# bastienjacquet/CudaDepthMapIntegration

Hardware: AMD Instinct MI355X
Metric: Gvoxel-projections/s (higher is better)
Workload: dtype f64

## Files before the change

### cudadepthmapintegration_amd/build.py

```python
from __future__ import annotations

import os
import re
import shutil
import subprocess
from concurrent.futures import ThreadPoolExecutor

_HERE = os.path.dirname(os.path.abspath(__file__))
ROOT = os.path.dirname(_HERE)
CSRC = os.path.join(_HERE, "csrc")
OBJ_DIR = os.path.join(ROOT, "build", "obj")
LIB_PATH = os.path.join(CSRC, "libdmi_hip.so")

SOURCES = ["fusion_kernels.hip", "fusion_tile.hip", "fusion_classify.hip", "coloration_kernels.hip", "grid_post.hip", "isosurface.hip", "isosurface_components.hip", "isosurface_smooth.hip", "dmi_capi.hip", "dmi_multi.hip", "host/recon_host.cpp", "host/vti_reader.cpp", "host/vtp_reader.cpp", "host/recon_cli.cpp", "host/color_cli.cpp", "host/dmi_host_capi.cpp"]
HEADERS = ["fusion_kernels.h", "fusion_device.h", "fusion_tile_acc.inc", "isosurface_table.inc", os.path.join("host", "recon_host.h"),
           os.path.join("host", "vtk_xml_data.h"), os.path.join("host", "vti_reader.h"), os.path.join("host", "vtp_reader.h"),
           os.path.join("host", "recon_cli.h"), os.path.join("host", "color_cli.h"),
           os.path.join("..", "..", "include", "dmi.h"), os.path.join("..", "..", "include", "dmi_host.h")]
CLI_MAINS = ["recon_cli_main.cpp", "color_cli_main.cpp"]

COMMON_FLAGS = ["-O3", "-std=c++17", "-fPIC", "-ffp-contract=off", "-fno-fast-math", "-Wall", "-Wno-unused-function",
                "-Wno-inline-asm", "-Wno-pass-failed"]
HIP_FLAGS = ["--offload-arch=gfx950", "-mllvm", "-disable-promote-alloca-to-vector", "-Xoffload-linker", "--discard-all"]
OPTIONAL_LLVM_FLAGS = ["-amdgpu-use-amdgpu-trackers=1"]


def _probe_llvm_flag(flag: str) -> bool:
    import tempfile

    try:
        with tempfile.TemporaryDirectory() as tmp:
            src = os.path.join(tmp, "probe.hip")
            with open(src, "w") as fh:
                fh.write("__global__ void probe() {}\n")
            r = subprocess.run([hipcc_path(), "--offload-arch=gfx950", "--cuda-device-only", "-mllvm", flag, "-c", src, "-o",
                                os.path.join(tmp, "probe.o")], capture_output=True)
            return r.returncode == 0
    except (OSError, RuntimeError):
        return False


_FLAG_CACHE = os.path.join(ROOT, "build", "llvm_flag_probe.json")


def _optional_flags() -> list:
    import json

    try:
        parts = []
        hip = os.path.realpath(hipcc_path())
        for f in (hip, os.path.realpath(os.path.join(os.path.dirname(hip), "..", "lib", "llvm", "bin", "clang"))):
            if os.path.exists(f):
                st = os.stat(f)
                parts.append("%s:%d:%d" % (f, st.st_size, int(st.st_mtime)))
        version = ";".join(parts)
    except (OSError, RuntimeError):
        return []
    try:
        with open(_FLAG_CACHE) as fh:
            rec = json.load(fh)
        if rec.get("hipcc") == version and set(rec.get("flags", {})) == set(OPTIONAL_LLVM_FLAGS):
            return [x for f in OPTIONAL_LLVM_FLAGS if rec["flags"][f] for x in ("-mllvm", f)]
    except (OSError, ValueError):
        pass
    flags = {f: _probe_llvm_flag(f) for f in OPTIONAL_LLVM_FLAGS}
    try:
        os.makedirs(os.path.dirname(_FLAG_CACHE), exist_ok=True)
        with open(_FLAG_CACHE, "w") as fh:
            json.dump({"hipcc": version, "flags": flags}, fh)
    except OSError:
        pass
    return [x for f in OPTIONAL_LLVM_FLAGS if flags[f] for x in ("-mllvm", f)]
if os.environ.get("DMI_EXP"):
    _name, _, _defs = os.environ["DMI_EXP"].partition(":")
    COMMON_FLAGS = COMMON_FLAGS + _defs.split()
    OBJ_DIR = os.path.join(ROOT, "build", "obj_exp_" + _name)
    LIB_PATH = os.path.join(CSRC, "libdmi_hip_exp_" + _name + ".so")
if os.environ.get("DMI_TUNING"):
    COMMON_FLAGS = COMMON_FLAGS + ["-DDMI_TUNING"]
    OBJ_DIR = os.path.join(ROOT, "build", "obj_tuning")
    LIB_PATH = os.path.join(CSRC, "libdmi_hip_tuning.so")


def hipcc_path() -> str:
    for cand in (shutil.which("hipcc"), "/opt/rocm/bin/hipcc"):
        if cand and os.path.exists(cand):
            return cand
    raise RuntimeError("hipcc not found: the HIP library cannot be built (no CPU fallback exists)")


HIP_FLAGS = HIP_FLAGS + _optional_flags()


def _sources():
    return [s for s in SOURCES if os.path.exists(os.path.join(CSRC, s))]


def _headers():
    return [os.path.join(CSRC, h) for h in HEADERS if os.path.exists(os.path.join(CSRC, h))]


def _obj(src: str) -> str:
    return os.path.join(OBJ_DIR, src.replace("/", "_") + ".o")


def _stale(target: str, deps) -> bool:
    if not os.path.exists(target):
        return True
    t = os.path.getmtime(target)
    return any(os.path.getmtime(d) > t for d in deps)


LIB_OVERRIDE = os.environ.get("DMI_LIB_OVERRIDE")
if LIB_OVERRIDE:
    LIB_PATH = os.path.abspath(LIB_OVERRIDE)


def source_digest(files=None) -> str:
    import hashlib

    h = hashlib.sha256()
    h.update(" ".join(COMMON_FLAGS + HIP_FLAGS).encode())
    if files is None:
        files = [os.path.join(CSRC, s) for s in _sources()] + _headers() + [os.path.join(CSRC, "host", m) for m in CLI_MAINS]
    for f in files:
        h.update(os.path.relpath(f, CSRC).encode())
        with open(f, "rb") as fh:
            h.update(fh.read())
    return h.hexdigest()


def _digest_path() -> str:
    return LIB_PATH + ".digest"


def needs_build() -> bool:
    if LIB_OVERRIDE:
        return False
    if not os.path.exists(LIB_PATH):
        return True
    if os.path.exists(_digest_path()):
        with open(_digest_path()) as fh:
            return fh.read().strip() != source_digest()
    deps = [os.path.join(CSRC, s) for s in _sources()] + _headers()
    return _stale(LIB_PATH, deps)


ACC_BASES = {8: 64, 7: 72, 6: 80, 5: 96}


def audit_accumulator_registers(asm_text: str) -> tuple[int, list[str]]:
    import re

    bad: list[str] = []
    checked = 0
    for body in re.split(r"\n(?=_ZN3dmi\S*fuse_tile_kernel\S*:)", asm_text):
        m = re.match(r"(_ZN3dmi\S*fuse_tile_kernelI\w+):", body)
        if not m:
            continue
        name = m.group(1)
        tpl = re.search(r"fuse_tile_kernelI\w\wLi(\d+)ELi(\d)ELi(\d)ELi(\d)ELi(\d)ELb([01])", name)
        tk, minw = int(tpl.group(1)), int(tpl.group(4))
        base = ACC_BASES.get(minw, 128)
        code = body[: body.find("s_endpgm")]
        in_asm = False
        scc_from_asm = False
        for line in code.splitlines():
            if "#ASMSTART" in line:
# ... 203 lines not shown
```

### cudadepthmapintegration_amd/capi.py

```python
from __future__ import annotations

import ctypes
import os
import sys
from typing import NamedTuple

import numpy as np

from . import build as _build
from .scene import GridDesc, RayPotential, Views

DMI_OK = 0
DMI_F32, DMI_F64 = 0, 1
DMI_DEPTH_AUTO, DMI_DEPTH_F32, DMI_DEPTH_F64 = 0, 1, 2
DMI_COMPONENTS_MIN_TRIANGLES, DMI_COMPONENTS_LARGEST = 0, 1

VARIANT_EXACT_DIVISION = 1
VARIANT_GENERAL_K = 2
VARIANT_FORCE_GENERAL = 16
VARIANT_NO_BRICK_CLASSES = 256
VARIANT_KEEP_BEHIND_ADDS = 1024
VARIANT_NO_INTERIOR = 2048
VARIANT_XCD_RUNS = 8192
VARIANT_ZMAJOR_SLOTS = 16384
VARIANT_PERSISTENT_ALWAYS = 32768
VARIANT_PERSISTENT_NEVER = 65536
VARIANT_NO_WINDOWS = 262144
VARIANT_WINDOWS_ALWAYS = 524288
VARIANT_COST_ORDER = 1048576
VARIANT_NO_COST_ORDER = 2097152
VARIANT_BRICK_CLASSES_ALWAYS = 131072
VARIANT_FIXED_TILE_SHAPE = 4096
VARIANT_SPATIAL_ORDER = 512
VARIANT_TILE_SHAPE = {"tk16_w5_g8_1x1": 0, "tk8_w6_g8_2x2": 32, "tk16_w5_g8_2x2": 64, "tk8_w6": 96, "tk8_w7_g8": 128, "tk16_w5_g4": 160,
                      "tk16_w6_g2": 192, "tk8_w6_g8_1x1": 224}


class GridDescC(ctypes.Structure):
    _fields_ = [("cell_dims", ctypes.c_int32 * 3), ("origin", ctypes.c_double * 3),
                ("spacing", ctypes.c_double * 3), ("grid_matrix", ctypes.c_double * 16)]


class RayPotentialC(ctypes.Structure):
    _fields_ = [("thickness", ctypes.c_double), ("rho", ctypes.c_double), ("eta", ctypes.c_double),
                ("delta", ctypes.c_double)]


class OptionsC(ctypes.Structure):
    _fields_ = [("device", ctypes.c_int32), ("grid_dtype", ctypes.c_int32), ("depth_storage", ctypes.c_int32),
                ("count_hits", ctypes.c_int32), ("kernel_variant", ctypes.c_int32), ("z_first", ctypes.c_int32),
                ("stream", ctypes.c_void_p), ("external_grid", ctypes.c_void_p)]


class TimingsC(ctypes.Structure):
    _fields_ = [("last_fuse_kernel_ms", ctypes.c_double), ("total_fuse_kernel_ms", ctypes.c_double),
                ("fuse_launches", ctypes.c_uint64), ("last_upload_ms", ctypes.c_double),
                ("last_download_ms", ctypes.c_double), ("last_cell_to_point_ms", ctypes.c_double),
                ("last_fuse_main_kernel_ms", ctypes.c_double), ("total_fuse_main_kernel_ms", ctypes.c_double)]


class InfoC(ctypes.Structure):
    _fields_ = [("n_voxels", ctypes.c_int64), ("n_views", ctypes.c_int32), ("depth_width", ctypes.c_int32),
                ("depth_height", ctypes.c_int32), ("depth_storage_in_use", ctypes.c_int32),
                ("grid_dtype", ctypes.c_int32), ("k_mode", ctypes.c_int32), ("kernel_variant", ctypes.c_int32),
                ("tiled_kernel", ctypes.c_int32), ("device_bytes", ctypes.c_uint64), ("pixels_without_depth", ctypes.c_uint64)]


class MultiOptionsC(ctypes.Structure):
    _fields_ = [("grid_dtype", ctypes.c_int32), ("depth_storage", ctypes.c_int32), ("kernel_variant", ctypes.c_int32),
                ("partition", ctypes.c_int32), ("exchange", ctypes.c_int32), ("n_slabs", ctypes.c_int32)]


class MultiInfoC(ctypes.Structure):
    _fields_ = [("world", ctypes.c_int32), ("n_local", ctypes.c_int32), ("first_rank", ctypes.c_int32),
                ("rccl_ranks", ctypes.c_int32), ("rccl_version", ctypes.c_int32), ("partition", ctypes.c_int32),
                ("exchange", ctypes.c_int32), ("n_slabs", ctypes.c_int32), ("n_voxels", ctypes.c_int64),
                ("n_views_total", ctypes.c_int64), ("n_views_local", ctypes.c_int64)]


class MultiTimingsC(ctypes.Structure):
    _fields_ = [("last_step_ms", ctypes.c_double), ("last_fuse_kernel_ms", ctypes.c_double),
                ("total_step_ms", ctypes.c_double), ("steps", ctypes.c_uint64)]


DMI_PARTITION_VIEWS, DMI_PARTITION_Z_SLABS = 0, 1
DMI_EXCHANGE_ALL_REDUCE, DMI_EXCHANGE_REDUCE_SCATTER, DMI_EXCHANGE_PEER_COPY = 0, 1, 2
DMI_UNIQUE_ID_BYTES = 128

ABI_SYMBOLS = [
    "dmi_default_options", "dmi_create", "dmi_destroy", "dmi_last_error", "dmi_add_views", "dmi_add_views_f32",
    "dmi_clear_views", "dmi_reset_grid", "dmi_upload_grid", "dmi_fuse", "dmi_fuse_range", "dmi_fuse_slab", "dmi_fuse_range_download", "dmi_synchronize",
    "dmi_download_grid_f64", "dmi_download_grid_f32", "dmi_download_hits", "dmi_grid_device_pointer",
    "dmi_get_brick_class_histogram", "dmi_get_timings", "dmi_get_info", "dmi_alloc_pinned", "dmi_free_pinned", "dmi_pcie_probe", "dmi_fp64_probe", "dmi_abi_version", "dmi_device_count",
    "dmi_color_mesh", "dmi_color_last_error", "dmi_cell_to_point", "dmi_download_point_data_f64",
    "dmi_point_data_device_pointer", "dmi_color_create", "dmi_color_destroy", "dmi_color_add_views",
    "dmi_color_clear_views", "dmi_color_process", "dmi_color_get_kernel_ms", "dmi_get_mixed_reason_histogram", "dmi_get_window_pair_count", "dmi_get_view_paths", "dmi_get_upload_kernel_ms", "dmi_sizeof_info", "dmi_sizeof_timings",
    "dmi_color_set_scratch_budget", "dmi_color_set_vertex_reorder", "dmi_color_add_views_with_depth", "dmi_color_set_depth_test",
    "dmi_iso_active_cells",
    "dmi_extract_isosurface", "dmi_download_isosurface", "dmi_get_isosurface_kernel_ms",
    "dmi_extract_isosurface_normals", "dmi_download_isosurface_normals",
    "dmi_filter_isosurface_components", "dmi_download_isosurface_regions", "dmi_get_isosurface_filter_kernel_ms",
    "dmi_get_isosurface_filter_pass_ms", "dmi_get_isosurface_filter_cas_retries",
    "dmi_smooth_isosurface", "dmi_get_isosurface_smooth_kernel_ms", "dmi_get_isosurface_smooth_pass_ms",
    "dmi_multi_default_options", "dmi_multi_view_shard", "dmi_multi_z_slab", "dmi_multi_slab_ranges", "dmi_multi_peer_chunk", "dmi_multi_create",
    "dmi_multi_get_unique_id", "dmi_multi_create_rank", "dmi_multi_destroy", "dmi_multi_last_error", "dmi_multi_add_views",
    "dmi_multi_add_views_f32", "dmi_multi_add_local_views", "dmi_multi_add_local_views_f32", "dmi_multi_clear_views", "dmi_multi_fuse", "dmi_multi_synchronize",
    "dmi_multi_download_grid_f32", "dmi_multi_download_grid_f64", "dmi_multi_get_info", "dmi_multi_get_timings",
    "dmi_multi_local_context",
]

_lib = None


class DmiError(RuntimeError):
    def __init__(self, code: int, message: str):
        super().__init__(f"dmi error {code}: {message}")
        self.code = code


def library_path() -> str:
    return _build.LIB_PATH


def load() -> ctypes.CDLL:
    global _lib
    if _lib is not None:
        return _lib
    if "torch" not in sys.modules:
        try:
            import torch
        except Exception:
            pass
    path = _build.build()
    if not os.path.exists(path):
        raise RuntimeError(f"{path} is missing: the HIP extension is required, there is no CPU fallback")
    L = ctypes.CDLL(path)
    vp, i32, dbl = ctypes.c_void_p, ctypes.c_int32, ctypes.c_double
    dp = ctypes.POINTER(ctypes.c_double)
    L.dmi_default_options.argtypes = [ctypes.POINTER(OptionsC)]
    L.dmi_default_options.restype = None
    L.dmi_create.argtypes = [ctypes.POINTER(GridDescC), ctypes.POINTER(RayPotentialC), ctypes.POINTER(OptionsC),
                             ctypes.POINTER(vp)]
    L.dmi_destroy.argtypes = [vp]
    L.dmi_destroy.restype = None
    L.dmi_last_error.argtypes = [vp]
    L.dmi_last_error.restype = ctypes.c_char_p
    L.dmi_add_views.argtypes = [vp, dp, dp, dbl, dp, dp, i32, i32, i32]
    L.dmi_add_views_f32.argtypes = [vp, ctypes.POINTER(ctypes.c_float), dp, dp, i32, i32, i32]
    L.dmi_clear_views.argtypes = [vp]
    L.dmi_reset_grid.argtypes = [vp]
    L.dmi_upload_grid.argtypes = [vp, dp]
    L.dmi_fuse.argtypes = [vp]
    L.dmi_fuse_range.argtypes = [vp, i32, i32]
    L.dmi_fuse_slab.argtypes = [vp, i32, i32]
    if hasattr(L, "dmi_fuse_range_download"):
        L.dmi_fuse_range_download.argtypes = [vp, i32, i32, vp, i32, i32]
    L.dmi_synchronize.argtypes = [vp]
    L.dmi_download_grid_f64.argtypes = [vp, dp]
    L.dmi_download_grid_f32.argtypes = [vp, ctypes.POINTER(ctypes.c_float)]
    L.dmi_download_hits.argtypes = [vp, ctypes.POINTER(ctypes.c_uint32), ctypes.POINTER(ctypes.c_uint64)]
    L.dmi_grid_device_pointer.argtypes = [vp, ctypes.POINTER(vp)]
    L.dmi_cell_to_point.argtypes = [vp]
    L.dmi_download_point_data_f64.argtypes = [vp, dp]
    L.dmi_point_data_device_pointer.argtypes = [vp, ctypes.POINTER(vp)]
    if hasattr(L, "dmi_iso_active_cells"):
        L.dmi_iso_active_cells.argtypes = [vp, ctypes.c_double, ctypes.POINTER(ctypes.c_uint64), ctypes.POINTER(ctypes.c_int64),
                                           ctypes.c_uint64]
    if hasattr(L, "dmi_extract_isosurface"):
        L.dmi_extract_isosurface.argtypes = [vp, ctypes.c_double, ctypes.POINTER(ctypes.c_uint64), ctypes.POINTER(ctypes.c_uint64)]
        L.dmi_download_isosurface.argtypes = [vp, dp, ctypes.POINTER(ctypes.c_int64)]
        L.dmi_get_isosurface_kernel_ms.argtypes = [vp, dp]
    if hasattr(L, "dmi_extract_isosurface_normals"):
        L.dmi_extract_isosurface_normals.argtypes = [vp, ctypes.c_double, ctypes.POINTER(ctypes.c_uint64), ctypes.POINTER(ctypes.c_uint64)]
        L.dmi_download_isosurface_normals.argtypes = [vp, ctypes.POINTER(ctypes.c_float)]
    if hasattr(L, "dmi_filter_isosurface_components"):
        u64p = ctypes.POINTER(ctypes.c_uint64)
        L.dmi_filter_isosurface_components.argtypes = [vp, ctypes.c_int, ctypes.c_uint64, u64p, u64p, u64p, u64p]
        L.dmi_download_isosurface_regions.argtypes = [vp, ctypes.POINTER(ctypes.c_int64), ctypes.POINTER(ctypes.c_int64)]
        L.dmi_get_isosurface_filter_kernel_ms.argtypes = [vp, dp]
        L.dmi_get_isosurface_filter_pass_ms.argtypes = [vp, dp]
        L.dmi_get_isosurface_filter_cas_retries.argtypes = [vp, u64p]
    if hasattr(L, "dmi_smooth_isosurface"):
        L.dmi_smooth_isosurface.argtypes = [vp, i32, dbl, dbl]
        L.dmi_get_isosurface_smooth_kernel_ms.argtypes = [vp, dp]
        L.dmi_get_isosurface_smooth_pass_ms.argtypes = [vp, dp]
    L.dmi_get_brick_class_histogram.argtypes = [vp, ctypes.POINTER(ctypes.c_uint64)]
    L.dmi_get_mixed_reason_histogram.argtypes = [vp, ctypes.POINTER(ctypes.c_uint64)]
    if hasattr(L, "dmi_get_window_pair_count"):
        L.dmi_get_window_pair_count.argtypes = [vp, ctypes.POINTER(ctypes.c_uint64)]
    if hasattr(L, "dmi_get_view_paths"):
        L.dmi_get_view_paths.argtypes = [vp, ctypes.POINTER(ctypes.c_uint64)]
    if hasattr(L, "dmi_get_upload_kernel_ms"):
        L.dmi_get_upload_kernel_ms.argtypes = [vp, dp, dp]
    for name in ("dmi_sizeof_info", "dmi_sizeof_timings"):
        if hasattr(L, name):
            getattr(L, name).restype = ctypes.c_size_t
    L.dmi_get_timings.argtypes = [vp, ctypes.POINTER(TimingsC)]
    L.dmi_get_info.argtypes = [vp, ctypes.POINTER(InfoC)]
    L.dmi_alloc_pinned.argtypes = [ctypes.c_size_t, ctypes.POINTER(vp)]
    L.dmi_free_pinned.argtypes = [vp]
    L.dmi_pcie_probe.argtypes = [i32, ctypes.c_size_t, dp, dp]
    L.dmi_fp64_probe.argtypes = [i32, ctypes.c_double, dp]
    u8p = ctypes.POINTER(ctypes.c_uint8)
    L.dmi_color_mesh.argtypes = [dp, ctypes.c_int64, u8p, dp, dp, i32, i32, i32, i32, u8p, u8p, ctypes.POINTER(ctypes.c_int32)]
    L.dmi_color_create.argtypes = [i32, ctypes.POINTER(vp)]
    L.dmi_color_destroy.argtypes = [vp]
    L.dmi_color_destroy.restype = None
    L.dmi_color_add_views.argtypes = [vp, u8p, dp, dp, i32, i32, i32]
    L.dmi_color_clear_views.argtypes = [vp]
    L.dmi_color_process.argtypes = [vp, dp, ctypes.c_int64, u8p, u8p, ctypes.POINTER(ctypes.c_int32)]
    L.dmi_color_get_kernel_ms.argtypes = [vp, dp]
    L.dmi_color_set_scratch_budget.argtypes = [vp, ctypes.c_uint64]
    L.dmi_color_set_vertex_reorder.argtypes = [vp, i32]
    L.dmi_color_add_views_with_depth.argtypes = [vp, u8p, dp, dp, dp, i32, i32, i32]
    L.dmi_color_set_depth_test.argtypes = [vp, i32, ctypes.c_double]
    L.dmi_color_last_error.argtypes = []
    L.dmi_color_last_error.restype = ctypes.c_char_p
    i64, i64p, i32p = ctypes.c_int64, ctypes.POINTER(ctypes.c_int64), ctypes.POINTER(ctypes.c_int32)
    L.dmi_multi_default_options.argtypes = [ctypes.POINTER(MultiOptionsC)]
    L.dmi_multi_default_options.restype = None
    L.dmi_multi_view_shard.argtypes = [i64, i32, i32, i64p, i64p]
    L.dmi_multi_z_slab.argtypes = [i32, i32, i32, i32p, i32p]
    L.dmi_multi_slab_ranges.argtypes = [i32, i32, i32p, i32p, i32]
    if hasattr(L, "dmi_multi_peer_chunk"):
        L.dmi_multi_peer_chunk.argtypes = [i64, i32, i32, i64p, i64p]
    L.dmi_multi_create.argtypes = [ctypes.POINTER(GridDescC), ctypes.POINTER(RayPotentialC), ctypes.POINTER(MultiOptionsC),
                                   i32p, i32, ctypes.POINTER(vp)]
    L.dmi_multi_get_unique_id.argtypes = [u8p]
    L.dmi_multi_create_rank.argtypes = [ctypes.POINTER(GridDescC), ctypes.POINTER(RayPotentialC), ctypes.POINTER(MultiOptionsC),
                                        i32, i32, i32, u8p, ctypes.POINTER(vp)]
    L.dmi_multi_destroy.argtypes = [vp]
    L.dmi_multi_destroy.restype = None
    L.dmi_multi_last_error.argtypes = [vp]
    L.dmi_multi_last_error.restype = ctypes.c_char_p
    L.dmi_multi_add_views.argtypes = [vp, dp, dp, dbl, dp, dp, i32, i32, i32]
    L.dmi_multi_add_views_f32.argtypes = [vp, ctypes.POINTER(ctypes.c_float), dp, dp, i32, i32, i32]
    L.dmi_multi_add_local_views.argtypes = [vp, i32, dp, dp, dbl, dp, dp, i32, i32, i32]
    L.dmi_multi_add_local_views_f32.argtypes = [vp, i32, ctypes.POINTER(ctypes.c_float), dp, dp, i32, i32, i32]
    L.dmi_multi_clear_views.argtypes = [vp]
    L.dmi_multi_fuse.argtypes = [vp]
    L.dmi_multi_synchronize.argtypes = [vp]
    L.dmi_multi_download_grid_f32.argtypes = [vp, ctypes.POINTER(ctypes.c_float), i64p, i64p]
    L.dmi_multi_download_grid_f64.argtypes = [vp, dp, i64p, i64p]
    L.dmi_multi_get_info.argtypes = [vp, ctypes.POINTER(MultiInfoC)]
    L.dmi_multi_get_timings.argtypes = [vp, ctypes.POINTER(MultiTimingsC)]
    L.dmi_multi_local_context.argtypes = [vp, i32, ctypes.POINTER(vp)]
    from . import build as _b
    for name in ABI_SYMBOLS:
        if _b.LIB_OVERRIDE and not hasattr(L, name):
            continue
        fn = getattr(L, name)
        if fn.restype is ctypes.c_int:
            fn.restype = ctypes.c_int
    _lib = L
    return L


def pinned_empty(shape, dtype) -> np.ndarray:
    L = load()
    n = int(np.prod(shape)) * np.dtype(dtype).itemsize
    p = ctypes.c_void_p()
    rc = L.dmi_alloc_pinned(n, ctypes.byref(p))
    if rc != DMI_OK:
        raise DmiError(rc, "dmi_alloc_pinned failed")
    buf = (ctypes.c_char * n).from_address(p.value)
    return np.frombuffer(buf, dtype=dtype).reshape(shape)


def pcie_probe(device: int = 0, n_bytes: int = 256 << 20) -> tuple[float, float]:
    L = load()
    a, b = ctypes.c_double(), ctypes.c_double()
    rc = L.dmi_pcie_probe(int(device), int(n_bytes), ctypes.byref(a), ctypes.byref(b))
    if rc != DMI_OK:
        raise DmiError(rc, L.dmi_last_error(None).decode())
    return float(a.value), float(b.value)


def fp64_probe(device: int = 0, milliseconds: float = 20.0) -> float:
    L = load()
    a = ctypes.c_double()
    rc = L.dmi_fp64_probe(int(device), float(milliseconds), ctypes.byref(a))
    if rc != DMI_OK:
        raise DmiError(rc, L.dmi_last_error(None).decode())
    return float(a.value)


def device_count() -> int:
    return int(load().dmi_device_count())


def _dp(a):
    return a.ctypes.data_as(ctypes.POINTER(ctypes.c_double))


class FusionContext:

    def __init__(self, grid: GridDesc, ray: RayPotential, *, device: int = 0, grid_dtype: str = "f64",
                 depth_storage: str = "auto", count_hits: bool = False, kernel_variant: int = 0,
                 stream: int | None = None, external_grid: int | None = None, z_first: int = 0):
        self._lib = load()
        self._h = ctypes.c_void_p()
        g = _grid_c(grid)
        r = RayPotentialC(float(ray.thickness), float(ray.rho), float(ray.eta), float(ray.delta))
        o = OptionsC()
        self._lib.dmi_default_options(ctypes.byref(o))
        o.device = device
        o.grid_dtype = {"f32": DMI_F32, "f64": DMI_F64}[grid_dtype]
        o.depth_storage = {"auto": DMI_DEPTH_AUTO, "f32": DMI_DEPTH_F32, "f64": DMI_DEPTH_F64}[depth_storage]
        o.count_hits = 1 if count_hits else 0
        o.kernel_variant = int(kernel_variant)
        o.z_first = int(z_first)
        o.stream = stream
        o.external_grid = external_grid
        self.grid = grid
        self.grid_dtype = grid_dtype
        self.n_voxels = grid.n_voxels
        self._mesh_counts = None
        rc = self._lib.dmi_create(ctypes.byref(g), ctypes.byref(r), ctypes.byref(o), ctypes.byref(self._h))
        if rc != DMI_OK:
            self._h = ctypes.c_void_p()
            raise DmiError(rc, self._lib.dmi_last_error(None).decode())

    def _check(self, rc: int):
        if rc != DMI_OK:
            raise DmiError(rc, self._lib.dmi_last_error(self._h).decode())

    def close(self):
        if getattr(self, "_h", None) is not None and self._h:
            self._lib.dmi_destroy(self._h)
            self._h = ctypes.c_void_p()

    def __enter__(self):
        return self

    def __exit__(self, *exc):
        self.close()

    def __del__(self):
        try:
            self.close()
# ... 84 lines not shown

    def cell_to_point(self):
        self._check(self._lib.dmi_cell_to_point(self._h))

    def download_point_data(self) -> np.ndarray:
        nx, ny, nz = (int(c) for c in self.grid.cell_dims)
        out = np.empty((nz + 1) * (ny + 1) * (nx + 1), dtype=np.float64)
        self._check(self._lib.dmi_download_point_data_f64(self._h, _dp(out)))
        return out.reshape(nz + 1, ny + 1, nx + 1)

    def iso_active_cells(self, iso: float, ids: bool = True):
        n = ctypes.c_uint64(0)
        self._check(self._lib.dmi_iso_active_cells(self._h, float(iso), ctypes.byref(n), None, 0))
        if not ids:
            return int(n.value), None
        out = np.empty(int(n.value), dtype=np.int64)
        if n.value:
            self._check(self._lib.dmi_iso_active_cells(self._h, float(iso), ctypes.byref(n),
                                                       out.ctypes.data_as(ctypes.POINTER(ctypes.c_int64)), out.size))
        return int(n.value), out

    def extract_isosurface(self, iso: float):
        nv, nt = ctypes.c_uint64(0), ctypes.c_uint64(0)
        self._mesh_counts = None
        self._check(self._lib.dmi_extract_isosurface(self._h, float(iso), ctypes.byref(nv), ctypes.byref(nt)))
        verts = np.empty((max(int(nv.value), 1), 3), dtype=np.float64)
        tris = np.empty((max(int(nt.value), 1), 3), dtype=np.int64)
        self._mesh_counts = (int(nv.value), int(nt.value), 0)
        self._check(self._lib.dmi_download_isosurface(self._h, _dp(verts), tris.ctypes.data_as(ctypes.POINTER(ctypes.c_int64))))
        return verts[:int(nv.value)], tris[:int(nt.value)]

    def extract_isosurface_with_normals(self, iso: float):
        nv, nt = ctypes.c_uint64(0), ctypes.c_uint64(0)
        self._mesh_counts = None
        self._check(self._lib.dmi_extract_isosurface_normals(self._h, float(iso), ctypes.byref(nv), ctypes.byref(nt)))
        verts = np.empty((max(int(nv.value), 1), 3), dtype=np.float64)
        tris = np.empty((max(int(nt.value), 1), 3), dtype=np.int64)
        normals = np.empty((max(int(nv.value), 1), 3), dtype=np.float32)
        self._mesh_counts = (int(nv.value), int(nt.value), 0)
        self._check(self._lib.dmi_download_isosurface(self._h, _dp(verts), tris.ctypes.data_as(ctypes.POINTER(ctypes.c_int64))))
        self._check(self._lib.dmi_download_isosurface_normals(self._h, normals.ctypes.data_as(ctypes.POINTER(ctypes.c_float))))
        return verts[:int(nv.value)], tris[:int(nt.value)], normals[:int(nv.value)]

    def filter_isosurface_components(self, mode: str = "min_triangles", min_triangles: int = 0):
        m = {"min_triangles": DMI_COMPONENTS_MIN_TRIANGLES, "largest": DMI_COMPONENTS_LARGEST}[mode]
        out = [ctypes.c_uint64(0) for _ in range(4)]
        self._check(self._lib.dmi_filter_isosurface_components(self._h, m, int(min_triangles), *[ctypes.byref(x) for x in out]))
        self._mesh_counts = (int(out[0].value), int(out[1].value), int(out[3].value))
        return tuple(int(x.value) for x in out)

    def _current_mesh_counts(self):
        c = self._mesh_counts
        if c is None:
            raise DmiError(1, "no mesh: extract_isosurface has not succeeded")
        return c

    def download_isosurface(self):
        nv, nt, _ = self._current_mesh_counts()
        verts = np.empty((max(nv, 1), 3), dtype=np.float64)
        tris = np.empty((max(nt, 1), 3), dtype=np.int64)
        self._check(self._lib.dmi_download_isosurface(self._h, _dp(verts), tris.ctypes.data_as(ctypes.POINTER(ctypes.c_int64))))
        return verts[:nv], tris[:nt]

    def download_isosurface_normals(self):
        nv, _, _ = self._current_mesh_counts()
        normals = np.empty((max(nv, 1), 3), dtype=np.float32)
        self._check(self._lib.dmi_download_isosurface_normals(self._h, normals.ctypes.data_as(ctypes.POINTER(ctypes.c_float))))
        return normals[:nv]

    def download_isosurface_regions(self):
        nv, _, nk = self._current_mesh_counts()
        rid = np.empty(max(nv, 1), dtype=np.int64)
        rsz = np.empty(max(nk, 1), dtype=np.int64)
        i64p = ctypes.POINTER(ctypes.c_int64)
        self._check(self._lib.dmi_download_isosurface_regions(self._h, rid.ctypes.data_as(i64p), rsz.ctypes.data_as(i64p)))
        return rid[:nv], rsz[:nk]

    def isosurface_filter_kernel_ms(self) -> float:
        a = ctypes.c_double(0)
        self._check(self._lib.dmi_get_isosurface_filter_kernel_ms(self._h, ctypes.byref(a)))
        return float(a.value)

    def isosurface_filter_cas_retries(self) -> int:
        a = ctypes.c_uint64(0)
        self._check(self._lib.dmi_get_isosurface_filter_cas_retries(self._h, ctypes.byref(a)))
        return int(a.value)

    def isosurface_filter_pass_ms(self) -> dict:
        a = (ctypes.c_double * 4)()
        self._check(self._lib.dmi_get_isosurface_filter_pass_ms(self._h, a))
        return dict(zip(("labels", "sizes", "scans", "compaction"), (float(x) for x in a)))

    def smooth_isosurface(self, iterations: int, lam: float = 0.5, mu: float = -0.53) -> None:
        self._check(self._lib.dmi_smooth_isosurface(self._h, int(iterations), float(lam), float(mu)))

    def isosurface_smooth_kernel_ms(self) -> float:
        a = ctypes.c_double(0)
        self._check(self._lib.dmi_get_isosurface_smooth_kernel_ms(self._h, ctypes.byref(a)))
        return float(a.value)

    def isosurface_smooth_pass_ms(self) -> dict:
        a = (ctypes.c_double * 3)()
        self._check(self._lib.dmi_get_isosurface_smooth_pass_ms(self._h, a))
        return dict(zip(("adjacency", "steps", "normals"), (float(x) for x in a)))

    def isosurface_kernel_ms(self) -> float:
        a = ctypes.c_double(0)
        self._check(self._lib.dmi_get_isosurface_kernel_ms(self._h, ctypes.byref(a)))
        return float(a.value)

    def brick_class_histogram(self) -> dict:
        h = (ctypes.c_uint64 * 4)()
        self._check(self._lib.dmi_get_brick_class_histogram(self._h, h))
        return {"mixed": int(h[0]), "free": int(h[1]), "behind": int(h[2]), "skip": int(h[3])}

    def mixed_reason_histogram(self) -> dict:
        h = (ctypes.c_uint64 * 8)()
        self._check(self._lib.dmi_get_mixed_reason_histogram(self._h, h))
        names = ["unspecified", "degenerate", "camera_plane", "image_border", "nan_depth", "sentinel_and_depth", "near_surface",
                 "free_or_no_depth"]
        return {n: int(h[i]) for i, n in enumerate(names)}

    def window_pair_count(self) -> int:
        n = ctypes.c_uint64(0)
        if not hasattr(self._lib, "dmi_get_window_pair_count"):
            return 0
        self._check(self._lib.dmi_get_window_pair_count(self._h, ctypes.byref(n)))
        return int(n.value)

    def upload_kernel_ms(self) -> tuple:
        if not hasattr(self._lib, "dmi_get_upload_kernel_ms"):
            return (0.0, 0.0)
        a, b = ctypes.c_double(0), ctypes.c_double(0)
        self._check(self._lib.dmi_get_upload_kernel_ms(self._h, ctypes.byref(a), ctypes.byref(b)))
        return (float(a.value), float(b.value))

    def timings(self) -> TimingsC:
        t = TimingsC()
        self._check(self._lib.dmi_get_timings(self._h, ctypes.byref(t)))
        return t

    def info(self) -> InfoC:
        i = InfoC()
        self._check(self._lib.dmi_get_info(self._h, ctypes.byref(i)))
        return i

    def view_paths(self) -> dict:
        names = ("general_kernel", "tiled_general_k", "tiled_fp64_selection", "tiled_tier1", "tiled_tier1_per_lane_margin", "with_window_record")
        if not hasattr(self._lib, "dmi_get_view_paths"):
            return {}
        a = (ctypes.c_uint64 * 6)()
        self._check(self._lib.dmi_get_view_paths(self._h, a))
        return {k: int(v) for k, v in zip(names, a)}


def _grid_c(grid: GridDesc) -> GridDescC:
    g = GridDescC()
    for i in range(3):
        g.cell_dims[i] = int(grid.cell_dims[i])
        g.origin[i] = float(grid.origin[i])
        g.spacing[i] = float(grid.spacing[i])
    gm = np.ascontiguousarray(grid.grid_matrix, dtype=np.float64).reshape(16)
    for i in range(16):
        g.grid_matrix[i] = gm[i]
    return g


def multi_view_shard(n: int, rank: int, world: int) -> tuple[int, int]:
    a, b = ctypes.c_int64(), ctypes.c_int64()
    if load().dmi_multi_view_shard(int(n), int(rank), int(world), ctypes.byref(a), ctypes.byref(b)) != DMI_OK:
        raise ValueError("rank/world out of range")
    return int(a.value), int(a.value + b.value)


def multi_z_slab(nz: int, rank: int, world: int) -> tuple[int, int]:
    a, b = ctypes.c_int32(), ctypes.c_int32()
    if load().dmi_multi_z_slab(int(nz), int(rank), int(world), ctypes.byref(a), ctypes.byref(b)) != DMI_OK:
        raise ValueError("rank/world out of range")
    return int(a.value), int(a.value + b.value)


def multi_peer_chunk(n: int, world: int, c: int) -> tuple[int, int]:
    a, b = ctypes.c_int64(), ctypes.c_int64()
    rc = load().dmi_multi_peer_chunk(int(n), int(world), int(c), ctypes.byref(a), ctypes.byref(b))
    if rc != DMI_OK:
        raise DmiError(rc, "dmi_multi_peer_chunk: invalid argument")
    return int(a.value), int(b.value)


def multi_slab_ranges(nz: int, n_slabs: int) -> list[tuple[int, int]]:
    a, b = (ctypes.c_int32 * 64)(), (ctypes.c_int32 * 64)()
    n = load().dmi_multi_slab_ranges(int(nz), int(n_slabs), a, b, 64)
    return [(int(a[i]), int(b[i])) for i in range(n)]


def multi_unique_id() -> bytes:
    L = load()
    buf = (ctypes.c_uint8 * DMI_UNIQUE_ID_BYTES)()
    rc = L.dmi_multi_get_unique_id(buf)
    if rc != DMI_OK:
        raise DmiError(rc, L.dmi_multi_last_error(None).decode())
    return bytes(buf)


class MultiContext:

    def __init__(self, grid: GridDesc, ray: RayPotential, *, devices=None, rank: int | None = None, world: int | None = None,
                 unique_id: bytes | None = None, device: int = 0, grid_dtype: str = "f32", depth_storage: str = "auto",
                 kernel_variant: int = 0, partition: str = "views", exchange: str = "all_reduce", n_slabs: int = 0):
        self._lib = load()
        self._h = ctypes.c_void_p()
        o = MultiOptionsC()
        self._lib.dmi_multi_default_options(ctypes.byref(o))
        o.grid_dtype = {"f32": DMI_F32, "f64": DMI_F64}[grid_dtype]
        o.depth_storage = {"auto": DMI_DEPTH_AUTO, "f32": DMI_DEPTH_F32, "f64": DMI_DEPTH_F64}[depth_storage]
        o.kernel_variant = int(kernel_variant)
        o.partition = {"views": DMI_PARTITION_VIEWS, "z_slabs": DMI_PARTITION_Z_SLABS}[partition]
        o.exchange = {"all_reduce": DMI_EXCHANGE_ALL_REDUCE, "reduce_scatter": DMI_EXCHANGE_REDUCE_SCATTER,
                      "peer_copy": DMI_EXCHANGE_PEER_COPY}[exchange]
        o.n_slabs = int(n_slabs)
        g = _grid_c(grid)
        r = RayPotentialC(float(ray.thickness), float(ray.rho), float(ray.eta), float(ray.delta))
        self.grid = grid
        self.grid_dtype = grid_dtype
        self.n_voxels = grid.n_voxels
        if devices is not None:
            d = (ctypes.c_int32 * len(devices))(*[int(x) for x in devices])
            rc = self._lib.dmi_multi_create(ctypes.byref(g), ctypes.byref(r), ctypes.byref(o), d, len(devices), ctypes.byref(self._h))
        else:
            if rank is None or world is None:
                raise ValueError("MultiContext needs devices=[...] or rank= and world=")
            idbuf = None
            if unique_id is not None:
                if len(unique_id) != DMI_UNIQUE_ID_BYTES:
                    raise ValueError("unique_id must be 128 bytes")
                idbuf = (ctypes.c_uint8 * DMI_UNIQUE_ID_BYTES).from_buffer_copy(unique_id)
            rc = self._lib.dmi_multi_create_rank(ctypes.byref(g), ctypes.byref(r), ctypes.byref(o), int(device), int(rank),
                                                 int(world), idbuf, ctypes.byref(self._h))
        if rc != DMI_OK:
            self._h = ctypes.c_void_p()
            raise DmiError(rc, self._lib.dmi_multi_last_error(None).decode())

    def _check(self, rc: int):
        if rc != DMI_OK:
            raise DmiError(rc, self._lib.dmi_multi_last_error(self._h).decode())

    def close(self):
        if getattr(self, "_h", None) is not None and self._h:
            self._lib.dmi_multi_destroy(self._h)
            self._h = ctypes.c_void_p()

    def __enter__(self):
        return self

    def __exit__(self, *exc):
        self.close()

    def __del__(self):
        try:
            self.close()
        except Exception:
            pass

    def add_views(self, views: Views, threshold: float | None = None, local_index: int | None = None):
        n, H, W = views.depth.shape
        K4 = np.ascontiguousarray(views.K4, dtype=np.float64).reshape(n, 16)
        RT4 = np.ascontiguousarray(views.RT4, dtype=np.float64).reshape(n, 16)
        L = self._lib
        if views.depth.dtype == np.float32:
            d = np.ascontiguousarray(views.depth)
            dptr = d.ctypes.data_as(ctypes.POINTER(ctypes.c_float))
            if local_index is None:
                self._check(L.dmi_multi_add_views_f32(self._h, dptr, _dp(K4), _dp(RT4), n, W, H))
            else:
                self._check(L.dmi_multi_add_local_views_f32(self._h, int(local_index), dptr, _dp(K4), _dp(RT4), n, W, H))
            return
        d = np.ascontiguousarray(views.depth, dtype=np.float64)
        bc = None
        if views.best_cost is not None and threshold is not None:
            bc = np.ascontiguousarray(views.best_cost, dtype=np.float64)
        thr = float(threshold) if threshold is not None else 0.0
        if local_index is None:
            self._check(L.dmi_multi_add_views(self._h, _dp(d), _dp(bc) if bc is not None else None, thr, _dp(K4), _dp(RT4), n, W, H))
        else:
            self._check(L.dmi_multi_add_local_views(self._h, int(local_index), _dp(d), _dp(bc) if bc is not None else None, thr,
                                                    _dp(K4), _dp(RT4), n, W, H))

    def clear_views(self):
        self._check(self._lib.dmi_multi_clear_views(self._h))

    def fuse(self):
        self._check(self._lib.dmi_multi_fuse(self._h))

    def synchronize(self):
        self._check(self._lib.dmi_multi_synchronize(self._h))

    def download_grid(self, dtype=np.float32, out: np.ndarray | None = None):
        nx, ny, nz = (int(c) for c in self.grid.cell_dims)
        if out is None:
            out = np.zeros(self.n_voxels, dtype=dtype)
        a, b = ctypes.c_int64(), ctypes.c_int64()
        if np.dtype(dtype) == np.float64:
            self._check(self._lib.dmi_multi_download_grid_f64(self._h, _dp(out), ctypes.byref(a), ctypes.byref(b)))
        else:
            self._check(self._lib.dmi_multi_download_grid_f32(self._h, out.ctypes.data_as(ctypes.POINTER(ctypes.c_float)),
                                                              ctypes.byref(a), ctypes.byref(b)))
# ... 560 lines not shown
```

### cudadepthmapintegration_amd/csrc/dmi_capi.hip

```cpp
#include "../../include/dmi.h"
#include "fusion_kernels.h"

#include <chrono>
#include <cmath>
#include <cstdio>
#include <cstdlib>
#include <cstring>
#include <exception>
#include <limits>
#include <new>
#include <string>
#include <vector>

using dmi::FuseArgs;
using dmi::FuseConfig;
using dmi::MapRec;
using dmi::TileArgs;
using dmi::TileMapRec;

namespace {

thread_local std::string g_create_error;

struct Batch {
// ... 331 lines not shown
    if (e == hipSuccess) e = hipStreamSynchronize(ctx->upload_stream);
    if (e == hipSuccess && ctx->up_start && ctx->up_stop) {
      float ms = 0.f;
      if (hipEventElapsedTime(&ms, ctx->up_start, ctx->up_stop) == hipSuccess) {
        const size_t last_cnt = (size_t)n - ((size_t)n - 1) / chunk * chunk;
        ctx->last_upload_kernel_ms = (double)ms * (double)n / (double)last_cnt;
        ctx->total_upload_kernel_ms += ctx->last_upload_kernel_ms;
      } else {
        (void)hipGetLastError();
      }
    }
    *lossy_out = counters[0];
    b.holes = counters[1];
    b.mingled_strips = counters[2];
    if (e != hipSuccess) rc = fail(ctx, DMI_ERR_DEVICE, std::string("depth upload: ") + hipGetErrorString(e));
  }
  if (rc != DMI_OK) {
    (void)hipFree(b.d_depth);
    (void)hipFree(b.d_pyramid);
    ctx->device_bytes -= npix * n * esz + pyr_bytes;
    return rc;
  }
  *out = b;
  return DMI_OK;
}


constexpr int kMaxColumn = 32;

void voxel_world(const dmi_grid_desc &g, int i, int j, int k, double w[3]) {
  const double p[3] = {g.origin[0] + (i + 0.5) * g.spacing[0], g.origin[1] + (j + 0.5) * g.spacing[1],
                       g.origin[2] + (k + 0.5) * g.spacing[2]};
  for (int r = 0; r < 3; ++r)
    w[r] = ((g.grid_matrix[4 * r] * p[0] + g.grid_matrix[4 * r + 1] * p[1]) + g.grid_matrix[4 * r + 2] * p[2]) +
           g.grid_matrix[4 * r + 3];
}

bool grid_axis_aligned(const dmi_grid_desc &g) {
  const double *m = g.grid_matrix;
  return m[1] == 0 && m[2] == 0 && m[4] == 0 && m[6] == 0 && m[8] == 0 && m[9] == 0;
}

float float_not_below(double x) {
  float f = (float)x;
  if ((double)f < x) f = std::nextafterf(f, std::numeric_limits<float>::infinity());
  return f;
}

void make_centred_rows(const dmi_context *ctx, const MapRec &r, const double P[4], const double Q[4], const double S[4],
                       double Sx, double Sy, const double M[3], double zabs, double zscale, bool general, bool aligned, TileMapRec *out,
                       dmi::WinRec *win, dmi::FootRec *foot) {
  TileMapRec &t = *out;
  std::memset(foot, 0, sizeof(*foot));
  std::memset(win, 0, sizeof(*win));
  win->e_abs = std::numeric_limits<float>::infinity();
  win->c1 = dmi::kWinC1;
  t.t1_ok = 0;
  t.t1_e1 = std::numeric_limits<float>::infinity();
  t.t1_c1 = 0.5f - 0x1p-20f;
  const double cxc = (double)(ctx->W / 2), cyc = (double)(ctx->H / 2);
  t.t1_cidx = (int32_t)((int64_t)ctx->W * (ctx->H / 2) + ctx->W / 2);
  if (general) return;
  double Pc[4], Qc[4];
  for (int c = 0; c < 4; ++c) {
    Pc[c] = P[c] - cxc * S[c];
    Qc[c] = Q[c] - cyc * S[c];
  }
  t.cpx = Pc[0]; t.cpy = Pc[1]; t.cpz = Pc[2]; t.cp0 = Pc[3];
  t.cqx = Qc[0]; t.cqy = Qc[1]; t.cqz = Qc[2]; t.cq0 = Qc[3];
  const double *g = ctx->grid.grid_matrix;
  const double sz = ctx->grid.spacing[2];
  t.cdhx = (Pc[0] * (g[2] * sz) + Pc[1] * (g[6] * sz)) + Pc[2] * (g[10] * sz);
  t.cdhy = (Qc[0] * (g[2] * sz) + Qc[1] * (g[6] * sz)) + Qc[2] * (g[10] * sz);
  const double rot = aligned ? 1.0 : 2.0;
  const double Sxc = Sx + cxc * M[2], Syc = Sy + cyc * M[2];
  const double cerr = rot * std::max(Sxc, Syc) * 0x1p-44;
  t.cerrk = cerr + 0x1p-22 * zabs * (1.0 + 0x1p-20);
  t.t1_dhx = (float)t.cdhx;
  t.t1_dhy = (float)t.cdhy;
  const double dcz = t.dhz;
  t.t1_dcz = (float)dcz;
  t.t1_dthr = (float)(dcz * (double)t.t1_c1);
  if (!(cerr < 0x1p-12 * zscale)) return;
  double czmin = std::numeric_limits<double>::infinity(), Scx = 0.0, Scy = 0.0;
  for (int c = 0; c < 8; ++c) {
    double w[3];
    voxel_world(ctx->grid, (c & 1) ? ctx->grid.cell_dims[0] - 1 : 0, (c & 2) ? ctx->grid.cell_dims[1] - 1 : 0,
                ctx->opt.z_first + ((c & 4) ? ctx->grid.cell_dims[2] - 1 : 0), w);
    czmin = std::min(czmin, ((r.rt[8] * w[0] + r.rt[9] * w[1]) + r.rt[10] * w[2]) + r.rt[11]);
    Scx = std::max(Scx, std::fabs(((Pc[0] * w[0] + Pc[1] * w[1]) + Pc[2] * w[2]) + Pc[3]));
    Scy = std::max(Scy, std::fabs(((Qc[0] * w[0] + Qc[1] * w[1]) + Qc[2] * w[2]) + Qc[3]));
  }
  czmin -= rot * 16.0 * 0x1p-52 * M[2];
  const double Sc = (std::max(Scx, Scy) + cerr) * (1.0 + 0x1p-20);
  const double D = kMaxColumn * std::max(std::fabs(t.cdhx), std::fabs(t.cdhy));
  const double Dz = kMaxColumn * std::fabs(dcz);
  const double nl = rot * 32.0 * 0x1p-53 * M[2];
  if (!std::isfinite(czmin)) return;
  const bool per_lane = !(czmin > 0.0) || !(Sc / czmin + 1.0 < 0x1p22);
  const double pmax = per_lane ? 0.0 : Sc / czmin + 1.0;
  const bool index_exact = ((int64_t)ctx->H + 2 * dmi::kValidMargin + 8) * ((int64_t)ctx->W + 2 * dmi::kValidMargin) + ctx->H +
                               2 * dmi::kValidMargin < (int64_t(1) << 24);
  double e1 = cerr + 3.0 * 0x1p-24 * Dz * pmax + 0x1p-22 * Dz + nl * (pmax + 2.0) + 0x1p-53 * std::max(Sx, Sy);
  e1 *= 1.0 + 0x1p-10;
  t.t1_erel = 0x1p-22f * (1.0f + 0x1p-10f);
  t.t1_hspan = float_not_below(D * (1.0 + 0x1p-20));
  if (!(pmax < 0x1p22) || !index_exact || !(e1 > 0x1p-100) || !(Sc < 0x1p60) || !std::isfinite(e1)) return;
  t.t1_e1 = float_not_below(e1);
  t.t1_ok = 1;
  {
    const double *sp = ctx->grid.spacing;
    double d[3][2], c[3];
    for (int ax = 0; ax < 3; ++ax) {
      const double wxs = g[ax] * sp[ax], wys = g[4 + ax] * sp[ax], wzs = g[8 + ax] * sp[ax];
      d[ax][0] = (Pc[0] * wxs + Pc[1] * wys) + Pc[2] * wzs;
      d[ax][1] = (Qc[0] * wxs + Qc[1] * wys) + Qc[2] * wzs;
      c[ax] = (S[0] * wxs + S[1] * wys) + S[2] * wzs;
    }
    const double xmax = (double)(std::max(ctx->W, ctx->H) / 2 + dmi::kValidMargin + 1);
    const double nl2 = 2.0 * nl;
    const double pwin = (dmi::kWindowRows - 0.5) * dmi::kWinCzRatio + 3.0;
    const double steps[3] = {7.0, 7.0, (double)(kMaxColumn - 1)};
    double e_step = 0.0;
    for (int xy = 0; xy < 2; ++xy) {
      double e = 0.0;
      for (int ax = 0; ax < 3; ++ax) e += steps[ax] * (std::fabs(d[ax][xy]) + xmax * std::fabs(c[ax]));
      e_step = std::max(e_step, e * 0x1p-23);
    }
    double ew = (cerr + xmax * nl2) + e_step + pwin * nl2 + 0x1p-53 * std::max(Sx, Sy);
    ew *= 1.0 + 0x1p-10;
    bool ok = std::isfinite(ew) && ew > 0x1p-100 && ew < 0x1p60;
    for (int ax = 0; ax < 3; ++ax) ok = ok && std::fabs(d[ax][0]) < 0x1p60 && std::fabs(d[ax][1]) < 0x1p60 && std::fabs(c[ax]) < 0x1p60;
    if (ok) {
      for (int xy = 0; xy < 2; ++xy) {
        win->di[xy] = (float)d[0][xy];
        win->dj[xy] = (float)d[1][xy];
        win->dk[xy] = (float)d[2][xy];
      }
      win->ci[0] = (float)c[0]; win->ci[1] = (float)(c[0] * (double)dmi::kWinC1);
      win->cj[0] = (float)c[1]; win->cj[1] = (float)(c[1] * (double)dmi::kWinC1);
      win->ck[0] = (float)c[2]; win->ck[1] = (float)(c[2] * (double)dmi::kWinC1);
      win->e_abs = float_not_below(ew);
      for (int cnr = 0; cnr < 8; ++cnr) {
        const double ni = (cnr & 1) ? 7.0 : 0.0, nj = (cnr & 2) ? 7.0 : 0.0;
        for (int v = 0; v < 2; ++v) {
          const double nk = (cnr & 4) ? (v ? 15.0 : 7.0) : 0.0;
          float *dst = v ? foot->s16[cnr] : foot->s8[cnr];
          dst[0] = (float)((ni * d[0][0] + nj * d[1][0]) + nk * d[2][0]);
          dst[1] = (float)((ni * d[0][1] + nj * d[1][1]) + nk * d[2][1]);
          dst[2] = (float)((ni * c[0] + nj * c[1]) + nk * c[2]);
        }
      }
      foot->ferr = float_not_below(cerr + xmax * nl2);
    }
  }
  if (per_lane) {
    const double B = (3.0 * 0x1p-24 * Dz + nl) * (1.0 + 0x1p-10) * (1.0 + 0x1p-10);
    if (!(B < 0x1p60) || !(B >= 0.0)) {
      t.t1_ok = 0;
      t.t1_e1 = std::numeric_limits<float>::infinity();
      return;
    }
    t.t1_b = float_not_below(B);
    t.t1_ok = 2;
  }
}

TileMapRec make_tile_rec(const dmi_context *ctx, const MapRec &r, dmi::WinRec *win, dmi::FootRec *foot, double *zscale_out) {
  TileMapRec t;
  std::memset(&t, 0, sizeof(t));
  const double *rt = r.rt, *k = r.k;
  t.rz0 = rt[8];
  t.rz1 = rt[9];
  t.rz3 = rt[11];
  const bool general = classify_k(r.k, r.rt) == dmi::K_GENERAL;
  double P[4], Q[4], S[4];
  for (int c = 0; c < 4; ++c) {
    if (general) {
      P[c] = (k[0] * rt[c] + k[1] * rt[4 + c]) + k[2] * rt[8 + c];
      Q[c] = (k[4] * rt[c] + k[5] * rt[4 + c]) + k[6] * rt[8 + c];
      S[c] = (k[8] * rt[c] + k[9] * rt[4 + c]) + k[10] * rt[8 + c];
    } else {
      P[c] = k[0] * rt[c] + k[1] * rt[4 + c] + k[2] * rt[8 + c];
      Q[c] = k[5] * rt[4 + c] + k[6] * rt[8 + c];
      S[c] = rt[8 + c];
    }
  }
  if (general) {
    P[3] += k[3];
    Q[3] += k[7];
    S[3] += k[11];
  }
  t.px = P[0]; t.py = P[1]; t.pz = P[2]; t.p0 = P[3];
  t.qx = Q[0]; t.qy = Q[1]; t.qz = Q[2]; t.q0 = Q[3];
  t.sx = S[0]; t.sy = S[1]; t.sz = S[2]; t.s0 = S[3];
  const double *g = ctx->grid.grid_matrix;
  const double sz = ctx->grid.spacing[2];
  t.dhx = (P[0] * (g[2] * sz) + P[1] * (g[6] * sz)) + P[2] * (g[10] * sz);
  t.dhy = (Q[0] * (g[2] * sz) + Q[1] * (g[6] * sz)) + Q[2] * (g[10] * sz);
  t.dhz = (S[0] * (g[2] * sz) + S[1] * (g[6] * sz)) + S[2] * (g[10] * sz);
  double wm[3];
  const bool aligned = grid_axis_aligned(ctx->grid);
  if (aligned) {
    double lo[3], hi[3];
    voxel_world(ctx->grid, 0, 0, ctx->opt.z_first, lo);
    voxel_world(ctx->grid, ctx->grid.cell_dims[0] - 1, ctx->grid.cell_dims[1] - 1,
                ctx->opt.z_first + ctx->grid.cell_dims[2] - 1 + kMaxColumn, hi);
    for (int a = 0; a < 3; ++a) wm[a] = std::max(std::fabs(lo[a]), std::fabs(hi[a]));
  } else {
    double gm[3];
    for (int a = 0; a < 3; ++a)
      gm[a] = std::fabs(ctx->grid.origin[a]) +
              (ctx->grid.cell_dims[a] + 1.0 + (a == 2 ? ctx->opt.z_first + kMaxColumn : 0)) * std::fabs(ctx->grid.spacing[a]);
    for (int a = 0; a < 3; ++a)
      wm[a] = std::fabs(g[4 * a]) * gm[0] + std::fabs(g[4 * a + 1]) * gm[1] + std::fabs(g[4 * a + 2]) * gm[2] + std::fabs(g[4 * a + 3]);
  }
  double M[3];
  for (int row = 0; row < 3; ++row)
    M[row] = std::fabs(rt[4 * row]) * wm[0] + std::fabs(rt[4 * row + 1]) * wm[1] + std::fabs(rt[4 * row + 2]) * wm[2] +
             std::fabs(rt[4 * row + 3]);
  const double Sx = std::fabs(k[0]) * M[0] + std::fabs(k[1]) * M[1] + std::fabs(k[2]) * M[2] + (general ? std::fabs(k[3]) : 0.0);
  const double Sy = (general ? std::fabs(k[4]) * M[0] : 0.0) + std::fabs(k[5]) * M[1] + std::fabs(k[6]) * M[2] +
                    (general ? std::fabs(k[7]) : 0.0);
  const double Sz = general ? std::fabs(k[8]) * M[0] + std::fabs(k[9]) * M[1] + std::fabs(k[10]) * M[2] + std::fabs(k[11]) : M[2];
  t.err = std::max(Sx, Sy) * 0x1p-44;
  t.errz = general ? Sz * 0x1p-44 : 0.0;
  t.cz_err = aligned ? 0.0 : M[2] * 0x1p-47;
  double zabs = Sz, czlo = std::numeric_limits<double>::infinity(), czhi = -czlo;
  if (!general) {
    zabs = 0.0;
    for (int c = 0; c < 8; ++c) {
      double w[3];
      voxel_world(ctx->grid, (c & 1) ? ctx->grid.cell_dims[0] - 1 : 0, (c & 2) ? ctx->grid.cell_dims[1] - 1 : 0,
                  ctx->opt.z_first + ((c & 4) ? ctx->grid.cell_dims[2] - 1 + kMaxColumn : 0), w);
      const double cz = ((rt[8] * w[0] + rt[9] * w[1]) + rt[10] * w[2]) + rt[11];
      zabs = std::max(zabs, std::fabs(cz));
      czlo = std::min(czlo, cz);
      czhi = std::max(czhi, cz);
    }
    zabs = zabs * (1.0 + 0x1p-20) + (aligned ? 1.0 : 2.0) * 32.0 * 0x1p-52 * M[2];
    if (!std::isfinite(zabs)) zabs = Sz;
  }
  double zscale = 1.0;
  if (!general && std::isfinite(czlo) && std::isfinite(czhi)) zscale = std::max(1.0, std::max(czlo, czhi / 16.0));
  t.errk = (t.err + 65536.0 * t.errz) + 0x1p-22 * zabs * (1.0 + 0x1p-20);
  t.depth = r.depth;
  make_centred_rows(ctx, r, P, Q, S, Sx, Sy, M, zabs, zscale, general, aligned, &t, win, foot);
  if (zscale_out) *zscale_out = zscale;
  return t;
}

bool tile_eligible(const dmi_context *ctx) {
  if (ctx->opt.kernel_variant & dmi::VAR_FORCE_GENERAL) return false;
  if (!ctx->finite_bounded) return false;
  if (!(ctx->ray.thickness >= 0) || !(ctx->ray.delta >= 0)) return false;
  if ((int64_t)ctx->W * ctx->H * (int64_t)(ctx->depth_f64 ? 8 : 4) >= (int64_t(1) << 31)) return false;
  return true;
}

int add_views_impl(dmi_context *ctx, const double *depth64, const float *depth32, const double *best_cost,
                   double threshold, const double *K4, const double *RT4, int32_t n, int32_t width, int32_t height) {
  if (!ctx) return DMI_ERR_INVALID_ARGUMENT;
  if ((!depth64 && !depth32) || !K4 || !RT4) return fail(ctx, DMI_ERR_INVALID_ARGUMENT, "dmi_add_views: null pointer");
  if (n <= 0) return fail(ctx, DMI_ERR_INVALID_ARGUMENT, "dmi_add_views: n must be positive");
  if (width < 1 || height < 1 || width > 32768 || height > 32768)
    return fail(ctx, DMI_ERR_INVALID_ARGUMENT, "dmi_add_views: depth-map dimensions must be in [1, 32768]");
  if (!ctx->batches.empty() && (width != ctx->W || height != ctx->H))
    return fail(ctx, DMI_ERR_INVALID_ARGUMENT, "dmi_add_views: every view of a context must share width and height");
  DMI_HIP(ctx, hipSetDevice(ctx->opt.device));
  const auto t0 = std::chrono::steady_clock::now();
  if (ctx->batches.empty()) {
    ctx->W = width;
    ctx->H = height;
    ctx->depth_f64 = ctx->opt.depth_storage == DMI_DEPTH_F64;
    ctx->k_mode = ctx->finite_bounded ? (int)dmi::K_PINHOLE : (int)dmi::K_GENERAL;
    ctx->max_tile_err = 0.0;
    ctx->pyramid = dmi::make_pyramid_desc(width, height);
  }
  const size_t npix = (size_t)width * height;

  Batch b;
  unsigned long long lossy = 0;
  int rc = upload_batch(ctx, depth64, depth32, best_cost, threshold, n, &b, &lossy);
  if (rc != DMI_OK) return rc;
  if (lossy != 0 && !ctx->depth_f64 && ctx->opt.depth_storage == DMI_DEPTH_AUTO) {
    (void)hipFree(b.d_depth);
    (void)hipFree(b.d_pyramid);
    ctx->device_bytes -= npix * n * 4 + b.aux_bytes;
    rc = promote_to_f64(ctx);
    if (rc != DMI_OK) return rc;
    rc = upload_batch(ctx, depth64, depth32, best_cost, threshold, n, &b, &lossy);
    if (rc != DMI_OK) return rc;
  }
  ctx->batches.push_back(b);
  const size_t esz = depth_elem(ctx);
  for (int32_t m = 0; m < n; ++m) {
    MapRec r;
    std::memset(&r, 0, sizeof(r));
    std::memcpy(r.rt, RT4 + 16 * (size_t)m, 12 * sizeof(double));
    std::memcpy(r.k, K4 + 16 * (size_t)m, 12 * sizeof(double));
    r.depth = static_cast<const char *>(b.d_depth) + (size_t)m * npix * esz;
    r.pyramid = b.d_pyramid + (size_t)m * ctx->pyramid.total_tiles;
    ctx->h_maps.push_back(r);
    bool finite = true;
    for (int q = 0; q < 12; ++q) finite = finite && bounded(r.k[q]) && bounded(r.rt[q]);
    const int km = classify_k(r.k, r.rt);
    if (km < ctx->k_mode) ctx->k_mode = km;
    dmi::WinRec wrec;
    dmi::FootRec frec;
    double zscale = 1.0;
    TileMapRec t = make_tile_rec(ctx, r, &wrec, &frec, &zscale);
    t.valid = reinterpret_cast<const uint8_t *>(b.d_pyramid) + b.valid_offset + (size_t)m * (size_t)dmi::valid_map_bytes(ctx->W, ctx->H);
    t.vm_c0 = ((float)(ctx->H / 2 + dmi::kValidMargin) - 3.5f) * 0.125f;
    t.vm_w8 = (float)(8 * (ctx->W + 2 * dmi::kValidMargin) - 8);
    t.vm_base = 8 * (ctx->W / 2 + dmi::kValidMargin) + ctx->H / 2 + dmi::kValidMargin;
    t.vm_bytes = (int32_t)std::min<int64_t>(dmi::valid_map_bytes(ctx->W, ctx->H), 0x7fffffff);
    t.vbits = reinterpret_cast<const uint32_t *>(reinterpret_cast<const uint8_t *>(b.d_pyramid) + b.bits_offset +
                                                 (size_t)m * (size_t)dmi::valid_bits_bytes(ctx->W, ctx->H));
    t.vb_bytes = (int32_t)std::min<int64_t>(dmi::valid_bits_bytes(ctx->W, ctx->H), 0x7fffffff);
    t.vb_rowskip = (dmi::valid_bits_tiles_x(ctx->W) - 1) * 128;
    t.vb_mx = 0x4B400000 + dmi::kValidMargin + ctx->W / 2;
    t.vb_my = 0x4B400000 + dmi::kValidMargin + ctx->H / 2;
    ctx->h_tile_maps.push_back(t);
    wrec.vbits = t.vbits;
    ctx->h_win_recs.push_back(wrec);
    ctx->h_foot_recs.push_back(frec);
    if (!(t.err <= ctx->max_tile_err)) ctx->max_tile_err = t.err;
    ctx->view_k_mode.push_back((uint8_t)km);
    ctx->view_tile_ok.push_back(finite && t.err < 0x1p-12 * zscale && 65536.0 * t.errz < 0x1p-14 && t.cerrk < 0x1p-11 * zscale ? 1 : 0);
  }
  ctx->maps_dirty = true;
  ctx->timings.last_upload_ms =
      std::chrono::duration<double, std::milli>(std::chrono::steady_clock::now() - t0).count();
  return DMI_OK;
}

constexpr int64_t kConvertChunk = int64_t(32) << 20;

int ensure_convert_stage(dmi_context *ctx) {
  if (ctx->d_convert) return DMI_OK;
  const int64_t elems = std::min<int64_t>(kConvertChunk, ctx->n_voxels);
  DMI_HIP(ctx, hipMalloc(&ctx->d_convert, (size_t)elems * 8));
  ctx->device_bytes += (uint64_t)elems * 8;
  return DMI_OK;
}

template <typename HostT>
int upload_converted(dmi_context *ctx, const HostT *src) {
  int rc = ensure_convert_stage(ctx);
  if (rc != DMI_OK) return rc;
  const size_t gsz = grid_elem(ctx);
  for (int64_t i0 = 0; i0 < ctx->n_voxels; i0 += kConvertChunk) {
    const int64_t n = std::min<int64_t>(kConvertChunk, ctx->n_voxels - i0);
    DMI_HIP(ctx, hipMemcpyAsync(ctx->d_convert, src + i0, (size_t)n * sizeof(HostT), hipMemcpyHostToDevice, ctx->stream));
    DMI_HIP(ctx, dmi::launch_convert_grid(ctx->d_convert, sizeof(HostT) == 8 ? 1 : 0, static_cast<char *>(ctx->d_grid) + (size_t)i0 * gsz, n,
                                          ctx->stream));
  }
  DMI_HIP(ctx, hipStreamSynchronize(ctx->stream));
  return DMI_OK;
}

template <typename HostT>
int download_converted(dmi_context *ctx, HostT *dst) {
  int rc = ensure_convert_stage(ctx);
  if (rc != DMI_OK) return rc;
  const size_t gsz = grid_elem(ctx);
  for (int64_t i0 = 0; i0 < ctx->n_voxels; i0 += kConvertChunk) {
    const int64_t n = std::min<int64_t>(kConvertChunk, ctx->n_voxels - i0);
    DMI_HIP(ctx, dmi::launch_convert_grid(static_cast<const char *>(ctx->d_grid) + (size_t)i0 * gsz, gsz == 8 ? 1 : 0, ctx->d_convert, n,
                                          ctx->stream));
    DMI_HIP(ctx, hipMemcpyAsync(dst + i0, ctx->d_convert, (size_t)n * sizeof(HostT), hipMemcpyDeviceToHost, ctx->stream));
  }
  DMI_HIP(ctx, hipStreamSynchronize(ctx->stream));
  return DMI_OK;
}

int flush_zero_fill(dmi_context *ctx) {
  if (ctx->zero_fill_pending) {
    DMI_HIP(ctx, hipMemsetAsync(ctx->d_grid, 0, ctx->n_voxels * grid_elem(ctx), ctx->stream));
    ctx->zero_fill_pending = false;
  }
  return DMI_OK;
}

int sync_maps(dmi_context *ctx) {
  const size_t n = ctx->h_maps.size();
  if (ctx->d_maps_capacity < n) {
    if (ctx->d_maps) (void)hipFree(ctx->d_maps);
    ctx->d_maps = nullptr;
    size_t cap = std::max<size_t>(64, n * 2);
    DMI_HIP(ctx, hipMalloc(&ctx->d_maps, cap * sizeof(MapRec)));
    if (ctx->d_tile_maps) (void)hipFree(ctx->d_tile_maps);
    ctx->d_tile_maps = nullptr;
    DMI_HIP(ctx, hipMalloc(&ctx->d_tile_maps, cap * sizeof(TileMapRec)));
    if (ctx->d_win_recs) (void)hipFree(ctx->d_win_recs);
    ctx->d_win_recs = nullptr;
    DMI_HIP(ctx, hipMalloc(&ctx->d_win_recs, cap * sizeof(dmi::WinRec)));
    if (ctx->d_foot_recs) (void)hipFree(ctx->d_foot_recs);
    ctx->d_foot_recs = nullptr;
    DMI_HIP(ctx, hipMalloc(&ctx->d_foot_recs, cap * sizeof(dmi::FootRec)));
    ctx->device_bytes += (cap - ctx->d_maps_capacity) * (sizeof(MapRec) + sizeof(TileMapRec) + sizeof(dmi::WinRec) + sizeof(dmi::FootRec));
    ctx->d_maps_capacity = cap;
    ctx->maps_dirty = true;
// ... 442 lines not shown
  a.delta = ctx->ray.delta;
  a.rho_pos = ctx->ray.rho * 1.0;
  a.rho_neg = ctx->ray.rho * -1.0;
  a.rho_zero = ctx->ray.rho * 0.0;
  a.slope = ctx->ray.rho / ctx->ray.thickness;
  a.free_space = -ctx->ray.eta * ctx->ray.rho;
  a.maps = ctx->d_maps;
  a.grid = ctx->d_grid;
  a.voxel_hits = ctx->d_voxel_hits;
  a.map_hits = ctx->d_map_hits;

  FuseConfig cfg;
  cfg.depth_is_f64 = ctx->depth_f64 ? 1 : 0;
  cfg.grid_is_f64 = ctx->opt.grid_dtype == DMI_F64 ? 1 : 0;
  cfg.k_mode = run_k_mode;
  cfg.count_hits = ctx->opt.count_hits ? 1 : 0;
  cfg.variant = ctx->opt.kernel_variant;

  cfg.use_tile = tiled ? 1 : 0;
  cfg.general_k = tiled && general_k ? 1 : 0;
  bool tall_by_holes = false, many_borders = false;
  {
    unsigned long long mingled = 0, strips = 0, without = 0;
    for (const Batch &bt : ctx->batches) {
      mingled += bt.mingled_strips;
      without += bt.holes;
      strips += (unsigned long long)bt.n * (unsigned long long)ctx->W * (unsigned long long)(ctx->H / 8);
    }
    const bool scattered = without <= 6 * mingled;
    cfg.holes = scattered && mingled * 160 > strips ? 1 : 0;
    tall_by_holes = scattered && mingled * 80 > strips;
    many_borders = mingled * 25 > strips;
    tall_by_holes = tall_by_holes || many_borders;
  }
  bool mostly_empty = false;
  if (!cfg.holes) {
    unsigned long long without = 0, pixels = 0;
    for (const Batch &bt : ctx->batches) {
      without += bt.holes;
      pixels += (unsigned long long)bt.n * (unsigned long long)ctx->W * (unsigned long long)ctx->H;
    }
    mostly_empty = without * 4 >= pixels && pixels > 0;
  }
  if (cfg.use_tile && !(cfg.variant & (dmi::VAR_TILE_SHAPE_MASK | dmi::VAR_FIXED_TILE_SHAPE))) {
    const int64_t bricks16 = (int64_t)((a.nx + 15) / 16) * ((a.ny + 15) / 16) * ((a.nz + 15) / 16);
    if (bricks16 <= 32768 && !(tall_by_holes && bricks16 >= 4096) && !(mostly_empty && bricks16 >= 13824))
      cfg.variant |= 7 << dmi::VAR_TILE_SHAPE_SHIFT;
  }

  TileArgs t;
  std::memset(&t, 0, sizeof(t));
  if (cfg.use_tile) {
    const dmi::TileShape sh = dmi::tile_shape(cfg.variant, ctx->depth_f64, !grid_axis_aligned(ctx->grid), cfg.general_k != 0);
    t.nx = a.nx; t.ny = a.ny; t.nz = a.nz; t.W = a.W; t.H = a.H;
    t.first_map = first; t.n_maps = count; t.init_from_grid = a.init_from_grid;
    t.kpad = (a.nz + sh.tk - 1) / sh.tk * sh.tk;
    t.bricks_x = (a.nx + 8 * sh.wx - 1) / (8 * sh.wx);
    t.bricks_y = (a.ny + 8 * sh.wy - 1) / (8 * sh.wy);
    t.bricks_z = t.kpad / sh.tk;
    t.super_x = (t.bricks_x + 3) / 4;
    t.super_y = (t.bricks_y + 3) / 4;
    t.super_z = (t.bricks_z + 1) / 2;
    if (!whole_grid) {
      t.sbz_first = z_first / (2 * sh.tk);
      t.super_z = (z_first + z_count + 2 * sh.tk - 1) / (2 * sh.tk) - t.sbz_first;
    }
    if (t.bricks_x > 2047 || t.bricks_y > 2047 || t.bricks_z > 1023)
      return fail(ctx, DMI_ERR_INVALID_ARGUMENT, "dmi_fuse: more bricks along an axis than the tiled kernel's order entries hold");
    t.slot_base = t.sbz_first * t.super_x * t.super_y * 32;
    t.slot_count = t.super_x * t.super_y * t.super_z * 32;
    rc = slot_permutation(ctx, t.super_x, t.super_y, t.super_z, (cfg.variant & dmi::VAR_ZMAJOR_SLOTS) != 0, &t.sb_perm);
    if (rc != DMI_OK) return rc;
    t.xcd_run_wg = 32 * std::max(1, t.super_x * t.super_y);
    if (((int64_t)t.super_x * t.super_y * t.super_z * 32 + 16 * (int64_t)t.xcd_run_wg + 64) > (int64_t)0x7fffffff)
      return fail(ctx, DMI_ERR_INVALID_ARGUMENT, "dmi_fuse: grid too large for one launch");
    t.depth_bytes = (int32_t)((int64_t)a.W * a.H * (ctx->depth_f64 ? 8 : 4));
    t.kz0 = a.kz0;
#ifdef DMI_TUNING
    if (std::getenv("DMI_DEBUG_NO_DEPTH_LOADS")) t.depth_bytes = 0;
#endif
    t.ox = a.ox; t.oy = a.oy; t.oz = a.oz; t.sx = a.sx; t.sy = a.sy; t.sz = a.sz;
    std::memcpy(t.g, a.g, sizeof(t.g));
    t.thick = a.thick; t.delta = a.delta; t.rho_pos = a.rho_pos; t.rho_neg = a.rho_neg;
    t.slope = a.slope; t.free_space = a.free_space;
    t.tile_maps = ctx->d_tile_maps;
    t.grid = a.grid; t.voxel_hits = a.voxel_hits; t.map_hits = a.map_hits;
    t.rotated = grid_axis_aligned(ctx->grid) ? 0 : 1;
    t.flags = ((cfg.variant & dmi::VAR_NO_INTERIOR) ? dmi::TILE_FLAG_NO_INTERIOR : 0) |
              ((cfg.variant & dmi::VAR_XCD_RUNS) ? dmi::TILE_FLAG_XCD_RUNS : 0);
    t.maps = ctx->d_maps;
    const size_t table_doubles = std::max<size_t>((size_t)n_views, 4) * (size_t)t.kpad;
    const size_t need = table_doubles + (size_t)dmi::kFreeSumsMax + 1;
    if (ctx->cz_table_capacity < need) {
      if (ctx->d_cz_table) {
        DMI_HIP(ctx, hipStreamSynchronize(ctx->stream));
        (void)hipFree(ctx->d_cz_table);
        ctx->device_bytes -= ctx->cz_table_capacity * 8;
        ctx->d_cz_table = nullptr;
        ctx->cz_table_capacity = 0;
      }
      const size_t grown = need * 2;
      DMI_HIP(ctx, hipMalloc(&ctx->d_cz_table, grown * 8));
      ctx->cz_table_capacity = grown;
      ctx->device_bytes += grown * 8;
    }
    t.cz_table = ctx->d_cz_table;
    if (!ctx->d_queue_heads) DMI_HIP(ctx, hipMalloc(&ctx->d_queue_heads, 128 * sizeof(int32_t)));
    t.queue_heads = ctx->d_queue_heads;
    if (!a.init_from_grid && !ctx->opt.count_hits && count <= dmi::kFreeSumsMax) t.free_sums = ctx->d_cz_table + table_doubles;
    t.wbricks_x = (a.nx + 7) / 8;
    t.wbricks_y = (a.ny + 7) / 8;
    if (!(cfg.variant & (dmi::VAR_NO_BRICK_CLASSES | dmi::VAR_BRICK_CLASSES_ALWAYS)) &&
        (int64_t)t.wbricks_x * t.wbricks_y * (int64_t)t.bricks_z <= dmi::kNoClassesMaxBricks && count < dmi::kNoClassesMaxViews)
      cfg.variant |= dmi::VAR_NO_BRICK_CLASSES;
    t.class_pitch = 64;
    while (t.class_pitch < n_views) t.class_pitch *= 2;
    if (cfg.variant & dmi::VAR_NO_BRICK_CLASSES) {
      if (ctx->zero_row_capacity < (size_t)t.class_pitch) {
        if (ctx->d_zero_row) {
          DMI_HIP(ctx, hipStreamSynchronize(ctx->stream));
          (void)hipFree(ctx->d_zero_row);
          ctx->d_zero_row = nullptr;
        }
        DMI_HIP(ctx, hipMalloc(&ctx->d_zero_row, (size_t)t.class_pitch));
        DMI_HIP(ctx, hipMemsetAsync(ctx->d_zero_row, dmi::BRICK_MIXED, (size_t)t.class_pitch, ctx->stream));
        ctx->zero_row_capacity = (size_t)t.class_pitch;
      }
      t.classes = ctx->d_zero_row;
      t.class_pitch = 0;
    } else {
      const size_t fine_bytes = ((size_t)t.wbricks_x * t.wbricks_y * t.bricks_z * (size_t)t.class_pitch + 255) / 256 * 256;
      const size_t coarse_end = (fine_bytes + (size_t)dmi::coarse_class_bytes(t, sh.tk) + 255) / 256 * 256;
      bool any_tier1 = false;
      for (int32_t m = first; m < first + count && !any_tier1; ++m) any_tier1 = std::isfinite(ctx->h_win_recs[(size_t)m].e_abs);
      const bool zero_free = (!a.init_from_grid || ctx->grid_free_of_negative_zero) && !ctx->opt.count_hits && !(cfg.variant & dmi::VAR_KEEP_BEHIND_ADDS);
      const bool windows = DMI_TIER1 != 0 && !cfg.general_k && !cfg.count_hits && !(cfg.variant & (dmi::VAR_NO_WINDOWS | dmi::VAR_NO_INTERIOR)) &&
                           (cfg.holes || many_borders || (cfg.variant & dmi::VAR_WINDOWS_ALWAYS)) && any_tier1 && zero_free && !ctx->depth_f64;
      const size_t cbytes = coarse_end + (windows ? fine_bytes * sizeof(dmi::WinPair) : 0);
      ctx->coarse_offset = fine_bytes;
      if (ctx->classes_capacity < cbytes) {
        if (ctx->d_classes) {
          DMI_HIP(ctx, hipStreamSynchronize(ctx->stream));
          (void)hipFree(ctx->d_classes);
          ctx->device_bytes -= ctx->classes_capacity;
          ctx->d_classes = nullptr;
          ctx->classes_capacity = 0;
        }
        DMI_HIP(ctx, hipMalloc(&ctx->d_classes, cbytes));
        DMI_HIP(ctx, hipMemsetAsync(ctx->d_classes, dmi::BRICK_SKIP, cbytes, ctx->stream));
        ctx->classes_capacity = cbytes;
        ctx->device_bytes += cbytes;
      }
      t.classes = ctx->d_classes;
      if (windows) {
        t.win_origin = reinterpret_cast<dmi::WinPair *>(ctx->d_classes + coarse_end);
        t.win_delta = (int64_t)reinterpret_cast<intptr_t>(t.win_origin) - 16 * (int64_t)reinterpret_cast<intptr_t>(t.classes);
        t.win_recs = ctx->d_win_recs;
        t.foot_recs = ctx->d_foot_recs;
        t.vb_bytes = (int32_t)std::min<int64_t>(dmi::valid_bits_bytes(ctx->W, ctx->H), 0x7fffffff);
        t.vb_rowskip = (dmi::valid_bits_tiles_x(ctx->W) - 1) * 128;
        t.win_cx = dmi::kValidMargin + ctx->W / 2;
        t.win_cy = dmi::kValidMargin + ctx->H / 2;
      }
      if (!(cfg.variant & dmi::VAR_SPATIAL_ORDER)) {
        const size_t n_slots = (size_t)t.super_x * t.super_y * t.super_z * 32;
        if (ctx->order_capacity < n_slots) {
          if (ctx->d_order) {
            DMI_HIP(ctx, hipStreamSynchronize(ctx->stream));
            (void)hipFree(ctx->d_order);
            (void)hipFree(ctx->d_order_level);
            ctx->device_bytes -= ctx->order_capacity * 5 + 4;
            ctx->d_order = nullptr;
            ctx->d_order_level = nullptr;
            ctx->order_capacity = 0;
          }
          DMI_HIP(ctx, hipMalloc(&ctx->d_order, (n_slots + 1) * sizeof(int32_t)));
          DMI_HIP(ctx, hipMalloc(&ctx->d_order_level, dmi::order_scratch_bytes(n_slots)));
          ctx->order_capacity = n_slots;
          ctx->device_bytes += n_slots * 5 + 4;
        }
        t.order = ctx->d_order + 1;
        t.n_order = ctx->d_order;
        t.order_levels = reinterpret_cast<const int32_t *>(ctx->d_order_level + (n_slots + 15) / 16 * 16);
        t.xcd_run_wg = 32 * (4 / (sh.wx * sh.wy));
        const bool cost_order = sh.wx * sh.wy == 1 && !(cfg.variant & dmi::VAR_NO_COST_ORDER) &&
                                ((cfg.variant & dmi::VAR_COST_ORDER) || n_slots <= (size_t)dmi::kCostOrderMaxSlots);
        if (cost_order) {
          t.flags |= dmi::TILE_FLAG_COST_ORDER | dmi::TILE_FLAG_XCD_RUNS;
          t.xcd_run_wg = 16;
        }
      }
    }
    if ((!a.init_from_grid || ctx->grid_free_of_negative_zero) && !ctx->opt.count_hits && !(cfg.variant & dmi::VAR_KEEP_BEHIND_ADDS))
      t.behind_mask = 0x0101010101010101ull;
#ifdef DMI_TUNING
    if (std::getenv("DMI_DEBUG_WG_TIMES")) {
      const size_t per_round = 8 * (size_t)t.xcd_run_wg;
      const size_t blocks = ((size_t)t.super_x * t.super_y * t.super_z * 32 + 32 + per_round - 1) / per_round * per_round;
      if (ctx->wg_times_blocks < blocks) {
        if (ctx->d_wg_times) {
          DMI_HIP(ctx, hipStreamSynchronize(ctx->stream));
          (void)hipFree(ctx->d_wg_times);
        }
        DMI_HIP(ctx, hipMalloc(&ctx->d_wg_times, blocks * 3 * sizeof(unsigned long long)));
        ctx->wg_times_blocks = blocks;
      }
      DMI_HIP(ctx, hipMemsetAsync(ctx->d_wg_times, 0, blocks * 3 * sizeof(unsigned long long), ctx->stream));
      t.wg_times = ctx->d_wg_times;
      t.wg_times_n = (int64_t)blocks;
    }
    if (const char *e = std::getenv("DMI_DEBUG_PAIRS")) {
      if (!std::strcmp(e, "nowin")) t.flags |= dmi::TILE_FLAG_DBG_SKIP_WINDOW_PAIRS;
      if (!std::strcmp(e, "onlywin")) t.flags |= dmi::TILE_FLAG_DBG_ONLY_WINDOW_PAIRS;
      if (!std::strcmp(e, "nowinloads")) t.flags |= dmi::TILE_FLAG_DBG_NO_WINDOW_LOADS;
    }
    if (const char *e = std::getenv("DMI_XCD_RUN_WG")) {
      t.xcd_run_wg = std::max(1, std::atoi(e));
      if (((int64_t)t.super_x * t.super_y * t.super_z * 32 + 8 * (int64_t)t.xcd_run_wg) > (int64_t)0x7fffffff)
        return fail(ctx, DMI_ERR_INVALID_ARGUMENT, "dmi_fuse: DMI_XCD_RUN_WG makes the launch too large");
    }
#endif
    if (!ctx->d_fuse_args) DMI_HIP(ctx, hipMalloc(&ctx->d_fuse_args, sizeof(FuseArgs)));
    DMI_HIP(ctx, hipMemcpyAsync(ctx->d_fuse_args, &a, sizeof(FuseArgs), hipMemcpyHostToDevice, ctx->stream));
    t.full = ctx->d_fuse_args;
  }

  EventPair ev;
  if (!ctx->pool.empty()) {
    ev = ctx->pool.back();
    ctx->pool.pop_back();
  } else {
    DMI_HIP(ctx, hipEventCreate(&ev.start));
    DMI_HIP(ctx, hipEventCreate(&ev.stop));
    DMI_HIP(ctx, hipEventCreate(&ev.mid));
  }
  ev.has_mid = cfg.use_tile != 0 && !(cfg.variant & dmi::VAR_NO_BRICK_CLASSES);
  DMI_HIP(ctx, hipEventRecord(ev.start, ctx->stream));
  hipError_t e = cfg.use_tile ? dmi::launch_fuse_tiled(t, ctx->d_maps, cfg, ctx->pyramid, ctx->d_order_level,
                                                         ctx->d_classes ? ctx->d_classes + ctx->coarse_offset : nullptr,
                                                         ev.has_mid ? ev.mid : nullptr, ctx->stream) : dmi::launch_fuse(a, cfg, ctx->stream);
  if (e != hipSuccess) {
    ctx->pool.push_back(ev);
    (void)hipGetLastError();
    return fail(ctx, DMI_ERR_DEVICE, std::string("fusion kernel launch: ") + hipGetErrorString(e));
  }
  ctx->last_fuse_tiled = cfg.use_tile != 0;
  ctx->last_fuse_classes = cfg.use_tile != 0 && !(cfg.variant & dmi::VAR_NO_BRICK_CLASSES);
  ctx->last_class_bricks = (int64_t)t.wbricks_x * t.wbricks_y * t.bricks_z;
  ctx->last_bricks_z = t.bricks_z;
  ctx->last_tk = t.bricks_z > 0 ? t.kpad / t.bricks_z : 0;
  ctx->last_win_origin = t.win_origin;
  ctx->last_class_pitch = t.class_pitch;
  ctx->last_first = first;
  ctx->last_count = count;
  DMI_HIP(ctx, hipEventRecord(ev.stop, ctx->stream));
  ctx->pending.push_back(ev);
  for (int32_t z = z_first; z < z_first + z_count; ++z) ctx->layer_is_zero[(size_t)z] = 0;
  ctx->zero_fill_pending = false;
  ctx->points_valid = false;
  if (ctx->pending.size() >= 256) return drain_events(ctx);
  return DMI_OK;
}

}

int dmi_fuse(dmi_context *ctx) {
  return guarded(ctx, "dmi_fuse", [&]() -> int {
  if (!ctx) return DMI_ERR_INVALID_ARGUMENT;
  return dmi_fuse_range(ctx, 0, (int32_t)ctx->h_maps.size());
  });
}

int dmi_synchronize(dmi_context *ctx) {
  return guarded(ctx, "dmi_synchronize", [&]() -> int {
  if (!ctx) return DMI_ERR_INVALID_ARGUMENT;
  DMI_HIP(ctx, hipSetDevice(ctx->opt.device));
  DMI_HIP(ctx, hipStreamSynchronize(ctx->stream));
  return drain_events(ctx);
  });
}

int dmi_download_grid_f64(dmi_context *ctx, double *out) {
  return guarded(ctx, "dmi_download_grid_f64", [&]() -> int {
  if (!ctx || !out) return fail(ctx, DMI_ERR_INVALID_ARGUMENT, "dmi_download_grid_f64: null argument");
  DMI_HIP(ctx, hipSetDevice(ctx->opt.device));
  { int rc_ = flush_zero_fill(ctx); if (rc_ != DMI_OK) return rc_; }
  const auto t0 = std::chrono::steady_clock::now();
  if (ctx->opt.grid_dtype == DMI_F64) {
    DMI_HIP(ctx, hipMemcpyAsync(out, ctx->d_grid, ctx->n_voxels * 8, hipMemcpyDeviceToHost, ctx->stream));
    DMI_HIP(ctx, hipStreamSynchronize(ctx->stream));
  } else {
    int rc_ = download_converted<double>(ctx, out);
    if (rc_ != DMI_OK) return rc_;
  }
  ctx->timings.last_download_ms =
      std::chrono::duration<double, std::milli>(std::chrono::steady_clock::now() - t0).count();
  return drain_events(ctx);
  });
}

int dmi_download_grid_f32(dmi_context *ctx, float *out) {
  return guarded(ctx, "dmi_download_grid_f32", [&]() -> int {
  if (!ctx || !out) return fail(ctx, DMI_ERR_INVALID_ARGUMENT, "dmi_download_grid_f32: null argument");
  DMI_HIP(ctx, hipSetDevice(ctx->opt.device));
  { int rc_ = flush_zero_fill(ctx); if (rc_ != DMI_OK) return rc_; }
  const auto t0 = std::chrono::steady_clock::now();
  if (ctx->opt.grid_dtype == DMI_F32) {
    DMI_HIP(ctx, hipMemcpyAsync(out, ctx->d_grid, ctx->n_voxels * 4, hipMemcpyDeviceToHost, ctx->stream));
    DMI_HIP(ctx, hipStreamSynchronize(ctx->stream));
  } else {
    int rc_ = download_converted<float>(ctx, out);
// ... 913 lines not shown
```

### cudadepthmapintegration_amd/csrc/fusion_classify.hip

```cpp
#include <algorithm>
#include <cstring>

#include <stdlib.h>

#include "fusion_kernels.h"
#include "fusion_device.h"

namespace dmi {

namespace {

template <typename T>
__device__ __forceinline__ T cload(const T *p) {
  return *reinterpret_cast<const T __attribute__((address_space(4))) *>(reinterpret_cast<uintptr_t>(p));
}

__device__ __forceinline__ float float_below(double d) {
  float f = (float)d;
  if ((double)f > d) f = nextafterf(f, -__builtin_inff());
  return f;
}
__device__ __forceinline__ float float_above(double d) {
  float f = (float)d;
  if ((double)f < d) f = nextafterf(f, __builtin_inff());
  return f;
}

struct TileAcc {
  float dmin = __builtin_inff(), dmax = -__builtin_inff();
  uint32_t flags = 0;
  __device__ __forceinline__ void add_value(double d) {
    if (d != d) {
      flags |= TILE_HAS_NAN;
    } else if (d == -1.0) {
      flags |= TILE_HAS_SENTINEL;
    } else {
      flags |= TILE_HAS_VALID;
      dmin = fminf(dmin, float_below(d));
      dmax = fmaxf(dmax, float_above(d));
    }
  }
  __device__ __forceinline__ void add_tile(const DepthTile &t) {
    flags |= t.flags;
    dmin = fminf(dmin, t.dmin);
    dmax = fmaxf(dmax, t.dmax);
  }
  __device__ __forceinline__ DepthTile tile() const { return DepthTile{dmin, dmax, flags, 0u}; }
  __device__ __forceinline__ DepthTile base_tile() const {
    return DepthTile{dmin, dmax, flags | ((flags & TILE_HAS_SENTINEL) ? 0u : (uint32_t)TILE_PART_HOLE_FREE) |
                                     ((flags & TILE_HAS_VALID) ? 0u : (uint32_t)TILE_PART_NO_VALID), 0u};
  }
};

template <typename InT, typename OutT>
__global__ __launch_bounds__(512) void upload_views_kernel(const InT *__restrict__ in, const double *__restrict__ best_cost, double thr,
                                                           OutT *__restrict__ out, int W, int H, PyramidDesc P,
                                                           DepthTile *__restrict__ pyr, uint8_t *__restrict__ valid,
                                                           uint32_t *__restrict__ bits, unsigned long long *__restrict__ counters) {
  __shared__ unsigned long long masks[8][8];
  __shared__ float part_min[8][64], part_max[8][64];
  __shared__ uint32_t part_flags[8][64];
  __shared__ unsigned int block_counts[2];
  const int lane = threadIdx.x & 63, w = threadIdx.x >> 6;
  const int64_t m = blockIdx.z;
  const int Wp = W + 2 * kValidMargin;
  const int tiles_x = valid_bits_tiles_x(W), tiles_y = valid_bits_tiles_y(H);
  const int tile_rows = (H + 2 * kValidMargin + 7) / 8;
  const int Y = blockIdx.y * 8 + w, y = Y - kValidMargin;
  const bool row_inside = y >= 0 && y < H;
  const int64_t npix = (int64_t)W * H;
  const InT *src = in + m * npix + (int64_t)(H - 1 - y) * W;
  const double *cost = best_cost ? best_cost + m * npix + (int64_t)(H - 1 - y) * W : nullptr;
  OutT *dst = out + m * npix + (int64_t)y * W;
  if (threadIdx.x < 2) block_counts[threadIdx.x] = 0;
  unsigned int lossy = 0;
  InT held[8];
  double held_cost[8];
#pragma unroll
  for (int k = 0; k < 8; ++k) held[k] = (InT)0, held_cost[k] = 0.0;
  if (row_inside) {
#pragma unroll
    for (int k = 0; k < 8; ++k) {
      const int x = min(max(blockIdx.x * 512 + 64 * k + lane - kValidMargin, 0), W - 1);
      held[k] = src[x];
      if (cost != nullptr) held_cost[k] = cost[x];
    }
  }
#pragma unroll
  for (int k = 0; k < 8; ++k) {
    const int X = blockIdx.x * 512 + 64 * k + lane, x = X - kValidMargin;
    const bool inside = row_inside && x >= 0 && x < W;
    bool has = false;
    TileAcc acc;
    if (inside) {
      double d = (double)held[k];
      if (cost != nullptr && held_cost[k] > thr) d = -1.0;
      const OutT o = (OutT)d;
      if (sizeof(OutT) == 4 && sizeof(InT) == 8) {
        const double back = (double)o;
        lossy += (__double_as_longlong(back) != __double_as_longlong(d)) && !(d != d);
      }
      dst[x] = o;
      has = !(o == (OutT)-1);
      acc.add_value((double)o);
    }
    const unsigned long long mask = __builtin_amdgcn_ballot_w64(has);
    if (lane == 0) masks[w][k] = mask;
    const int tx = X >> 5;
    if ((lane & 31) == 0 && tx < tiles_x && Y < tiles_y * 32)
      bits[m * (valid_bits_bytes(W, H) / 4) + ((int64_t)(Y >> 5) * tiles_x + tx) * 32 + (Y & 31)] = (uint32_t)(mask >> (lane & 32));
    float dmin = acc.dmin, dmax = acc.dmax;
    uint32_t flags = acc.flags;
#pragma unroll
    for (int off = 1; off < 8; off <<= 1) {
      dmin = fminf(dmin, __shfl_xor(dmin, off, 64));
      dmax = fmaxf(dmax, __shfl_xor(dmax, off, 64));
      flags |= (uint32_t)__shfl_xor((int)flags, off, 64);
    }
    if ((lane & 7) == 0) {
      part_min[w][k * 8 + (lane >> 3)] = dmin;
      part_max[w][k * 8 + (lane >> 3)] = dmax;
      part_flags[w][k * 8 + (lane >> 3)] = flags;
    }
  }
  if (sizeof(OutT) == 4 && sizeof(InT) == 8) {
    for (int off = 32; off > 0; off >>= 1) lossy += __shfl_xor((int)lossy, off, 64);
    if (lane == 0 && lossy != 0) atomicAdd(counters, (unsigned long long)lossy);
  }
  __syncthreads();
  const int t = threadIdx.x;
  if (t < 64) {
    const int ptx = blockIdx.x * 64 + t - kValidMargin / 8, pty = (int)blockIdx.y - kValidMargin / 8;
    if (ptx >= 0 && ptx < P.width[0] && pty >= 0 && pty < P.height[0]) {
      TileAcc a;
#pragma unroll
      for (int r = 0; r < 8; ++r) {
        a.dmin = fminf(a.dmin, part_min[r][t]);
        a.dmax = fmaxf(a.dmax, part_max[r][t]);
        a.flags |= part_flags[r][t];
      }
      pyr[m * P.total_tiles + P.offset[0] + pty * P.width[0] + ptx] = a.base_tile();
    }
  }
  {
    const int X = blockIdx.x * 512 + t, x = X - kValidMargin;
    unsigned long long bytes = 0;
    int have = 0;
#pragma unroll
    for (int r = 0; r < 8; ++r) {
      const bool has = (masks[r][t >> 6] >> (t & 63)) & 1ull;
      bytes |= (unsigned long long)(has ? kValidByte : 0) << (8 * r);
      have += has ? 1 : 0;
    }
    if (X < Wp && (int)blockIdx.y < tile_rows) *reinterpret_cast<unsigned long long *>(valid + m * valid_map_bytes(W, H) + ((int64_t)blockIdx.y * Wp + X) * 8) = bytes;
    const int y0 = (int)blockIdx.y * 8 - kValidMargin;
    const int rows_inside = max(0, min(H, y0 + 8) - max(0, y0));
    const bool col_inside = x >= 0 && x < W;
    const int holes = col_inside ? rows_inside - have : 0;
    const bool mingled = col_inside && rows_inside == 8 && holes > 0 && holes < 8;
    int hsum = holes;
    for (int off = 32; off > 0; off >>= 1) hsum += __shfl_xor(hsum, off, 64);
    const int msum = __builtin_popcountll(__builtin_amdgcn_ballot_w64(mingled));
    if (lane == 0) {
      if (hsum) atomicAdd(&block_counts[0], (unsigned int)hsum);
      if (msum) atomicAdd(&block_counts[1], (unsigned int)msum);
    }
  }
  __syncthreads();
  if (t < 2 && block_counts[t] != 0) atomicAdd(counters + 1 + t, (unsigned long long)block_counts[t]);
}

__global__ __launch_bounds__(1024) void pyramid_levels_kernel(PyramidDesc P, DepthTile *pyr) {
  DepthTile *view = pyr + (int64_t)blockIdx.x * P.total_tiles;
  for (int level = 1; level < P.n_levels; ++level) {
    const int w = P.width[level], tiles = w * P.height[level];
    const DepthTile *child = view + P.offset[level - 1];
    const int cw = P.width[level - 1], ch = P.height[level - 1];
    for (int t = threadIdx.x; t < tiles; t += blockDim.x) {
      const int ty = t / w, tx = t - ty * w;
      TileAcc acc;
      for (int y = 2 * ty; y < 2 * ty + 2 && y < ch; ++y)
        for (int x = 2 * tx; x < 2 * tx + 2 && x < cw; ++x) acc.add_tile(child[y * cw + x]);
      view[P.offset[level] + t] = acc.tile();
    }
    __syncthreads();
  }
}

template <int kQueryTiles>
__device__ __forceinline__ int query_level(const PyramidDesc &P, int extent) {
  int li = 0;
  while (li + 1 < P.n_levels && ((extent - 1) >> (kPyramidMinLevel + li)) + 2 > kQueryTiles) ++li;
  return li;
}

template <int kQueryTiles>
__device__ __forceinline__ TileAcc pyramid_query(const DepthTile *__restrict__ pyr, const PyramidDesc &P, int x0, int x1,
                                                 int y0, int y1) {
  const int li = query_level<kQueryTiles>(P, max(x1 - x0, y1 - y0) + 1);
  const int L = kPyramidMinLevel + li;
  TileAcc acc;
  const int tx0 = x0 >> L, tx1 = x1 >> L, ty0 = y0 >> L, ty1 = y1 >> L;
  for (int ty = ty0; ty <= ty1; ++ty)
    for (int tx = tx0; tx <= tx1; ++tx) acc.add_tile(pyr[P.offset[li] + ty * P.width[li] + tx]);
  return acc;
}

struct BoxFootprint {
  uint8_t cls;
  bool query;
  bool partial;
  bool in_margin;
  int x0, x1, y0, y1;
  int rx0, rx1, ry0, ry1;
  double czmin, czmax;
};

template <bool ROT, bool GK>
__device__ __forceinline__ BoxFootprint box_footprint_k(const TileArgs &a, const MapRec *__restrict__ mr,
                                                      const TileMapRec *__restrict__ tr, int i0, int i1, int j0, int j1, int k0,
                                                      int k1) {
  BoxFootprint fp;
  fp.query = false;
  fp.partial = false;
  fp.in_margin = false;
  fp.x0 = fp.x1 = fp.y0 = fp.y1 = 0;
  fp.rx0 = fp.rx1 = fp.ry0 = fp.ry1 = 0;
  double czmin = __builtin_inf(), czmax = -__builtin_inf();
  double umin = __builtin_inf(), umax = -__builtin_inf(), vmin = __builtin_inf(), vmax = -__builtin_inf();
  constexpr bool genk = GK;
  double hzmin = __builtin_inf(), hzmax = -__builtin_inf();
  bool bad = false;
  const double r23 = mr->rt[11];
  if constexpr (ROT) {
#pragma unroll
    for (int c = 0; c < 8; ++c) {
      const int i = (c & 1) ? i1 : i0, j = (c & 2) ? j1 : j0, k = (c & 4) ? k1 : k0;
      const double gx = a.ox + (i + 0.5) * a.sx;
      const double gy = a.oy + (j + 0.5) * a.sy;
      const double gz = a.oz + ((k + a.kz0) + 0.5) * a.sz;
      const double wx = row4(a.g + 0, gx, gy, gz), wy = row4(a.g + 4, gx, gy, gz), wz = row4(a.g + 8, gx, gy, gz);
      const double cz = row4(mr->rt + 8, wx, wy, wz);
      const double hx = __builtin_fma(tr->px, wx, __builtin_fma(tr->py, wy, __builtin_fma(tr->pz, wz, tr->p0)));
      const double hy = __builtin_fma(tr->qx, wx, __builtin_fma(tr->qy, wy, __builtin_fma(tr->qz, wz, tr->q0)));
      const double hz = genk ? __builtin_fma(tr->sx, wx, __builtin_fma(tr->sy, wy, __builtin_fma(tr->sz, wz, tr->s0))) : cz;
      double r = __builtin_amdgcn_rcp(hz);
      r = __builtin_fma(r, __builtin_fma(-hz, r, 1.0), r);
      const double u = hx * r, v = hy * r;
      bad = bad || !(cz == cz);
      if (genk) {
        bad = bad || !(hz == hz);
        hzmin = fmin(hzmin, hz);
        hzmax = fmax(hzmax, hz);
      }
      czmin = fmin(czmin, cz);
      czmax = fmax(czmax, cz);
      umin = fmin(umin, u);
      umax = fmax(umax, u);
      vmin = fmin(vmin, v);
      vmax = fmax(vmax, v);
    }
    czmin -= 2.0 * tr->cz_err;
    czmax += 2.0 * tr->cz_err;
  } else {
  double wxs[2], wys[2], wzs[2];
  for (int c = 0; c < 2; ++c) {
    const int i = c ? i1 : i0, j = c ? j1 : j0, k = c ? k1 : k0;
    const double gx = a.ox + (i + 0.5) * a.sx;
    const double gy = a.oy + (j + 0.5) * a.sy;
    const double gz = a.oz + ((k + a.kz0) + 0.5) * a.sz;
    wxs[c] = row4(a.g + 0, gx, gy, gz);
    wys[c] = row4(a.g + 4, gx, gy, gz);
    wzs[c] = row4(a.g + 8, gx, gy, gz);
  }
  const double r20 = mr->rt[8], r21 = mr->rt[9], r22 = mr->rt[10];
  const double zx[2] = {r20 * wxs[0], r20 * wxs[1]}, zy[2] = {r21 * wys[0], r21 * wys[1]}, zz[2] = {r22 * wzs[0], r22 * wzs[1]};
  const double ux[2] = {tr->px * wxs[0], tr->px * wxs[1]};
  const double uy[2] = {__builtin_fma(tr->py, wys[0], tr->p0), __builtin_fma(tr->py, wys[1], tr->p0)};
  const double uz[2] = {tr->pz * wzs[0], tr->pz * wzs[1]};
  const double vx[2] = {tr->qx * wxs[0], tr->qx * wxs[1]};
  const double vy[2] = {__builtin_fma(tr->qy, wys[0], tr->q0), __builtin_fma(tr->qy, wys[1], tr->q0)};
  const double vz[2] = {tr->qz * wzs[0], tr->qz * wzs[1]};
  double sxw[2] = {0.0, 0.0}, syw[2] = {0.0, 0.0}, szw[2] = {0.0, 0.0};
  if (genk) {
    sxw[0] = tr->sx * wxs[0], sxw[1] = tr->sx * wxs[1];
    syw[0] = __builtin_fma(tr->sy, wys[0], tr->s0), syw[1] = __builtin_fma(tr->sy, wys[1], tr->s0);
    szw[0] = tr->sz * wzs[0], szw[1] = tr->sz * wzs[1];
  }
#pragma unroll
  for (int c = 0; c < 8; ++c) {
    const int cx = c & 1, cy = (c >> 1) & 1, ck = c >> 2;
    const double cz = ((zx[cx] + zy[cy]) + zz[ck]) + r23;
    const double hx = (ux[cx] + uy[cy]) + uz[ck];
    const double hy = (vx[cx] + vy[cy]) + vz[ck];
    const double hz = genk ? (sxw[cx] + syw[cy]) + szw[ck] : cz;
    double r = __builtin_amdgcn_rcp(hz);
    r = __builtin_fma(r, __builtin_fma(-hz, r, 1.0), r);
    const double u = hx * r, v = hy * r;
    bad = bad || !(cz == cz);
    if (genk) {
      bad = bad || !(hz == hz);
      hzmin = fmin(hzmin, hz);
      hzmax = fmax(hzmax, hz);
    }
    czmin = fmin(czmin, cz);
    czmax = fmax(czmax, cz);
    umin = fmin(umin, u);
    umax = fmax(umax, u);
    vmin = fmin(vmin, v);
    vmax = fmax(vmax, v);
  }
  }
  uint8_t cls = BRICK_MIXED | (MIXED_DEGENERATE << 2);
  const double errz2 = 2.0 * tr->errz;
  const double err = genk ? tr->err + 65536.0 * tr->errz : tr->err;
  const double dmin = genk ? hzmin - errz2 : czmin, dmax = genk ? hzmax + errz2 : czmax;
  const double ulimit = genk ? 65536.0 : 0x1p30;
  if (!bad) {
    cls = BRICK_MIXED | (MIXED_CAMERA_PLANE << 2);
    if (dmax < 0.0) {
      cls = BRICK_SKIP;
    } else if (dmin > 4.0 * err && dmin > 0.0 && umin == umin && umax == umax && vmin == vmin && vmax == vmax &&
               fabs(umin) < ulimit && fabs(umax) < ulimit && fabs(vmin) < ulimit && fabs(vmax) < ulimit) {
      double rmin = __builtin_amdgcn_rcp(dmin);
      rmin = __builtin_fma(rmin, __builtin_fma(-dmin, rmin, 1.0), rmin);
      const double e = 2.0 * err * rmin * (1.0 + 0x1p-30) + 0x1p-20;
      const int x0 = (int)ceil(umin - 0.5 - e), x1 = (int)floor(umax + 0.5 + e);
      const int y0 = (int)ceil(vmin - 0.5 - e), y1 = (int)floor(vmax + 0.5 + e);
      cls = BRICK_MIXED | (MIXED_IMAGE_BORDER << 2);
      fp.rx0 = x0;
      fp.rx1 = x1;
      fp.ry0 = y0;
      fp.ry1 = y1;
      if (x1 < 0 || y1 < 0 || x0 >= a.W || y0 >= a.H) {
        cls = BRICK_SKIP;
      } else if (x0 >= 0 && y0 >= 0 && x1 < a.W && y1 < a.H) {
        fp.query = true;
        fp.x0 = x0;
        fp.x1 = x1;
        fp.y0 = y0;
        fp.y1 = y1;
      } else {
        fp.partial = true;
        fp.in_margin = x0 >= -kValidMargin && y0 >= -kValidMargin && x1 < a.W + kValidMargin && y1 < a.H + kValidMargin;
        fp.x0 = max(x0, 0);
        fp.x1 = min(x1, a.W - 1);
        fp.y0 = max(y0, 0);
        fp.y1 = min(y1, a.H - 1);
      }
    }
  }
  fp.cls = cls;
  fp.czmin = czmin;
  fp.czmax = czmax;
  return fp;
}

template <bool ROT, bool GK>
__device__ __forceinline__ BoxFootprint box_footprint(const TileArgs &a, const MapRec *__restrict__ mr,
                                                      const TileMapRec *__restrict__ tr, int i0, int i1, int j0, int j1, int k0,
                                                      int k1) {
  if constexpr (GK) {
    if (tr->errz != 0.0) return box_footprint_k<ROT, true>(a, mr, tr, i0, i1, j0, j1, k0, k1);
  }
  return box_footprint_k<ROT, false>(a, mr, tr, i0, i1, j0, j1, k0, k1);
}

__device__ __forceinline__ uint8_t class_from_bounds(const TileArgs &a, const TileAcc &d, double czmin, double czmax) {
  if (d.flags & TILE_HAS_NAN) return BRICK_MIXED | (MIXED_NAN_DEPTH << 2);
  if (!(d.flags & TILE_HAS_VALID)) return BRICK_SKIP;
  const bool holes = (d.flags & TILE_HAS_SENTINEL) != 0;
  if ((czmax - (double)d.dmin) < -a.delta) {
    if (!holes) return BRICK_FREE;
    const bool free_column_exact = a.behind_mask != 0 || __builtin_signbit(a.free_space);
    return free_column_exact ? (uint8_t)(BRICK_MIXED | (MIXED_FREE_OR_NODEPTH << 2)) : (uint8_t)(BRICK_MIXED | (MIXED_SENTINEL_AND_DEPTH << 2));
  }
  if ((czmin - (double)d.dmax) > a.delta) {
    if (!holes) return BRICK_BEHIND;
    return a.behind_mask ? (uint8_t)BRICK_SKIP : (uint8_t)(BRICK_MIXED | (MIXED_SENTINEL_AND_DEPTH << 2));
  }
  return BRICK_MIXED | ((holes ? MIXED_SENTINEL_AND_DEPTH : MIXED_NEAR_SURFACE) << 2);
}

template <bool GK>
__device__ __forceinline__ uint8_t border_class(const TileArgs &a, const BoxFootprint &fp, const TileAcc &d) {
  const uint8_t c = class_from_bounds(a, d, fp.czmin, fp.czmax);
  if (c == BRICK_SKIP || (c == BRICK_BEHIND && a.behind_mask)) return BRICK_SKIP;
  const bool map_serves = DMI_TIER1 != 0 && !GK && fp.in_margin && a.behind_mask != 0;
  if (map_serves && (c == BRICK_FREE || c == (uint8_t)(BRICK_MIXED | (MIXED_FREE_OR_NODEPTH << 2))))
    return BRICK_MIXED | (MIXED_FREE_OR_NODEPTH << 2);
  return BRICK_MIXED | (MIXED_IMAGE_BORDER << 2);
}

template <int kQueryTiles, bool ROT, bool GK>
__device__ __forceinline__ uint8_t classify_box(const TileArgs &a, const MapRec *__restrict__ mr,
                                                const TileMapRec *__restrict__ tr, const PyramidDesc &P, int i0, int i1,
                                                int j0, int j1, int k0, int k1) {
  const BoxFootprint fp = box_footprint<ROT, GK>(a, mr, tr, i0, i1, j0, j1, k0, k1);
  if (fp.partial) return border_class<GK>(a, fp, pyramid_query<kQueryTiles>(mr->pyramid, P, fp.x0, fp.x1, fp.y0, fp.y1));
  if (!fp.query) return fp.cls;
  return class_from_bounds(a, pyramid_query<kQueryTiles>(mr->pyramid, P, fp.x0, fp.x1, fp.y0, fp.y1), fp.czmin, fp.czmax);
}

constexpr int kCostLevels = 64;

template <bool ROT, bool GK>
__global__ __launch_bounds__(256) void classify_coarse_kernel(const TileArgs a, const MapRec *__restrict__ maps,
                                                              const PyramidDesc P, int tk, uint8_t *__restrict__ classes,
                                                              uint8_t *__restrict__ coarse) {
  fill_launch_tables(a, maps, ((int64_t)blockIdx.y * gridDim.x + blockIdx.x) * 256 + threadIdx.y * 64 + threadIdx.x,
                     (int64_t)gridDim.x * gridDim.y * 256);
  if ((a.flags & TILE_FLAG_COST_ORDER) && blockIdx.x == 0 && blockIdx.y == 0 && threadIdx.y == 0)
    for (int q = threadIdx.x; q < 2 * kCostLevels; q += 64) const_cast<int32_t *>(a.order_levels)[q] = 0;
  const int bz_first = 2 * a.sbz_first;
  const int bz_count = min(2 * a.super_z, a.bricks_z - bz_first);
  const int per_z = 32 / tk;
  const int cx_n = (a.wbricks_x + 3) / 4, cy_n = (a.wbricks_y + 3) / 4, cz_n = (bz_count + per_z - 1) / per_z;
  const int local = blockIdx.x * 4 + threadIdx.y;
  const int mm = blockIdx.y * 64 + threadIdx.x;
  if (local >= cx_n * cy_n * cz_n || mm >= a.n_maps) return;
  const int m = a.first_map + mm;
  const int cbx = local % cx_n;
  const int ct = local / cx_n;
  const int cby = ct % cy_n, cbz = ct / cy_n + bz_first / per_z;
  const int bz0 = cbz * per_z;
  const BoxFootprint fp = box_footprint<ROT, GK>(a, maps + m, a.tile_maps + m, cbx * 32, cbx * 32 + 31, cby * 32, cby * 32 + 31,
                                                 bz0 * tk, bz0 * tk + 31);
  uint8_t cls = fp.cls;
  bool speckled = false;
  if (fp.query) {
    const TileAcc d = pyramid_query<5>(maps[m].pyramid, P, fp.x0, fp.x1, fp.y0, fp.y1);
    cls = class_from_bounds(a, d, fp.czmin, fp.czmax);
    speckled = !(d.flags & (TILE_PART_HOLE_FREE | TILE_PART_NO_VALID));
  } else if (fp.partial) {
    cls = border_class<GK>(a, fp, pyramid_query<5>(maps[m].pyramid, P, fp.x0, fp.x1, fp.y0, fp.y1));
  }
  const bool inherit_mixed = cls == (uint8_t)(BRICK_MIXED | (MIXED_FREE_OR_NODEPTH << 2)) && speckled;
  coarse[(int64_t)((cbz * cy_n + cby) * cx_n + cbx) * a.class_pitch + m] = inherit_mixed ? (uint8_t)(cls | COARSE_CHILDREN_WRITTEN) : cls;
  if ((cls & 3) == BRICK_MIXED && !inherit_mixed) return;
  for (int dz = 0; dz < per_z; ++dz) {
    const int bz = bz0 + dz;
    if (bz >= bz_first + bz_count) break;
    for (int dy = 0; dy < 4; ++dy) {
      const int by = cby * 4 + dy;
      if (by >= a.wbricks_y) break;
      for (int dx = 0; dx < 4; ++dx) {
        const int bx = cbx * 4 + dx;
        if (bx >= a.wbricks_x) break;
        classes[(int64_t)((bz * a.wbricks_y + by) * a.wbricks_x + bx) * a.class_pitch + m] = cls;
      }
    }
  }
}

constexpr int kWindow = 16;

template <int kQueryTiles, int kChildren, bool ROT, bool GK>
__global__ __launch_bounds__(256) void classify_kernel(const TileArgs a, const MapRec *__restrict__ maps,
                                                       const PyramidDesc P, int tk, uint8_t *__restrict__ classes,
                                                       const uint8_t *__restrict__ coarse, int group_views) {
  constexpr int children = kChildren;
  constexpr int views_per_wave = 64 / children;
  constexpr int per_z = children / 16;
  __shared__ float2 window_mm[4 * views_per_wave][kWindow * kWindow];
  __shared__ uint8_t window_fl[4 * views_per_wave][kWindow * kWindow];
  const int bz_first = 2 * a.sbz_first;
  const int bz_count = min(2 * a.super_z, a.bricks_z - bz_first);
  const int cx_n = (a.wbricks_x + 3) / 4, cy_n = (a.wbricks_y + 3) / 4;
  const int lane = threadIdx.x & 63, wave = __builtin_amdgcn_readfirstlane(threadIdx.x >> 6);
  const int local = blockIdx.x;
  const int cbx = local % cx_n;
  const int ct = local / cx_n;
  const int cby = ct % cy_n, cbz = ct / cy_n + bz_first / per_z;
  const int chunk0 = blockIdx.y * group_views;
  const uint8_t *__restrict__ crow = coarse + (int64_t)((cbz * cy_n + cby) * cx_n + cbx) * a.class_pitch + a.first_map + chunk0;
  const unsigned long long unproven = __builtin_amdgcn_ballot_w64(
      lane < group_views && chunk0 + lane < a.n_maps && (crow[lane] & (3 | COARSE_CHILDREN_WRITTEN)) == BRICK_MIXED);
  if (unproven == 0) return;
  unsigned long long items = views_per_wave == 1 ? unproven & (0x1111111111111111ull << wave)
                                                 : (unproven | (unproven >> 1)) & (0x0101010101010101ull << (2 * wave));
  const int child = lane % children;
  const int bx = cbx * 4 + (child & 3), by = cby * 4 + ((child >> 2) & 3), bz = cbz * per_z + (child >> 4);
  const bool in_grid = bx < a.wbricks_x && by < a.wbricks_y && bz < bz_first + bz_count;
  uint8_t *__restrict__ out = classes + (int64_t)((bz * a.wbricks_y + by) * a.wbricks_x + bx) * a.class_pitch;
  while (items) {
    const int first = __builtin_ctzll(items);
    items &= items - 1;
    const int rel = first + lane / children;
    const int mm = chunk0 + rel;
    const int m = a.first_map + min(mm, a.n_maps - 1);
    const bool mine = in_grid && ((unproven >> rel) & 1ull);
    const MapRec *__restrict__ mr = maps + m;
    BoxFootprint fp;
    fp.query = false;
    fp.partial = false;
    fp.in_margin = false;
    fp.cls = BRICK_SKIP;
    MapRec mr_u;
    TileMapRec tr_u;
    if constexpr (views_per_wave == 1) {
      const int mu = __builtin_amdgcn_readfirstlane(m);
      const MapRec *src = maps + mu;
      const TileMapRec *tsrc = a.tile_maps + mu;
#pragma unroll
      for (int q = 8; q < 12; ++q) mr_u.rt[q] = cload(&src->rt[q]);
      mr_u.pyramid = cload(&src->pyramid);
      tr_u.px = cload(&tsrc->px); tr_u.py = cload(&tsrc->py); tr_u.pz = cload(&tsrc->pz); tr_u.p0 = cload(&tsrc->p0);
      tr_u.qx = cload(&tsrc->qx); tr_u.qy = cload(&tsrc->qy); tr_u.qz = cload(&tsrc->qz); tr_u.q0 = cload(&tsrc->q0);
      tr_u.err = cload(&tsrc->err);
      tr_u.cz_err = cload(&tsrc->cz_err);
      tr_u.errz = cload(&tsrc->errz);
      if constexpr (GK) {
        tr_u.sx = cload(&tsrc->sx); tr_u.sy = cload(&tsrc->sy); tr_u.sz = cload(&tsrc->sz); tr_u.s0 = cload(&tsrc->s0);
      }
      mr = &mr_u;
      if (mine) {
        fp = box_footprint<ROT, GK>(a, &mr_u, &tr_u, bx * 8, bx * 8 + 7, by * 8, by * 8 + 7, bz * tk, bz * tk + tk - 1);
      }
    } else {
      if (mine) fp = box_footprint<ROT, GK>(a, mr, a.tile_maps + m, bx * 8, bx * 8 + 7, by * 8, by * 8 + 7, bz * tk, bz * tk + tk - 1);
    }
    const bool query = mine && (fp.query || fp.partial);
    uint8_t cls = fp.cls;
    const int li = query ? query_level<kQueryTiles>(P, max(fp.x1 - fp.x0, fp.y1 - fp.y0) + 1) : 0x7fff;
    bool from_window = false;
    {
      float2 *__restrict__ win_mm = window_mm[wave * views_per_wave + lane / children];
      uint8_t *__restrict__ win_fl = window_fl[wave * views_per_wave + lane / children];
      int li_w = li;
      for (int off = children >> 1; off > 0; off >>= 1) li_w = min(li_w, __shfl_xor(li_w, off, 64));
      if (li_w != 0x7fff) {
        const int L = kPyramidMinLevel + li_w;
        const bool at_level = query && li == li_w;
        int tx0 = at_level ? fp.x0 >> L : 0x7fffffff, ty0 = at_level ? fp.y0 >> L : 0x7fffffff;
        int tx1 = at_level ? fp.x1 >> L : -1, ty1 = at_level ? fp.y1 >> L : -1;
        int wx0 = tx0, wy0 = ty0, wx1 = tx1, wy1 = ty1;
        for (int off = children >> 1; off > 0; off >>= 1) {
          wx0 = min(wx0, __shfl_xor(wx0, off, 64));
          wy0 = min(wy0, __shfl_xor(wy0, off, 64));
          wx1 = max(wx1, __shfl_xor(wx1, off, 64));
          wy1 = max(wy1, __shfl_xor(wy1, off, 64));
        }
        if (wx1 - wx0 < kWindow && wy1 - wy0 < kWindow) {
          const DepthTile *__restrict__ level = mr->pyramid + P.offset[li_w];
          const int pitch = P.width[li_w];
          const int ww = wx1 - wx0 + 1, wh = wy1 - wy0 + 1;
          const int tx = child & 15;
          for (int ty = child >> 4; ty < wh; ty += children / 16)
            if (tx < ww) {
              const DepthTile t = level[(wy0 + ty) * pitch + wx0 + tx];
              win_mm[ty * kWindow + tx] = make_float2(t.dmin, t.dmax);
              win_fl[ty * kWindow + tx] = (uint8_t)t.flags;
            }
          __builtin_amdgcn_fence(__ATOMIC_RELEASE, "wavefront");
          __builtin_amdgcn_wave_barrier();
          __builtin_amdgcn_fence(__ATOMIC_ACQUIRE, "wavefront");
          if (at_level) {
            TileAcc d;
            for (int ty = ty0; ty <= ty1; ++ty)
              for (int tx = tx0; tx <= tx1; ++tx) {
                const int w = (ty - wy0) * kWindow + (tx - wx0);
                const float2 mm = win_mm[w];
                d.add_tile(DepthTile{mm.x, mm.y, (uint32_t)win_fl[w], 0u});
              }
            cls = fp.partial ? border_class<GK>(a, fp, d) : class_from_bounds(a, d, fp.czmin, fp.czmax);
            from_window = true;
          }
          __builtin_amdgcn_fence(__ATOMIC_RELEASE, "wavefront");
          __builtin_amdgcn_wave_barrier();
        }
      }
    }
    if (query && !from_window) {
      const TileAcc d = pyramid_query<kQueryTiles>(mr->pyramid, P, fp.x0, fp.x1, fp.y0, fp.y1);
      cls = fp.partial ? border_class<GK>(a, fp, d) : class_from_bounds(a, d, fp.czmin, fp.czmax);
    }
    if (mine) out[m] = cls;
  }
}

constexpr int kOriginViews = 8;
constexpr uint32_t kNotWanted = 0xfffffffeu;
template <bool ROT>
__global__ __launch_bounds__(256) void window_origin_kernel(const TileArgs a, const MapRec *__restrict__ maps, int tk,
                                                            uint8_t *__restrict__ classes, WinPair *__restrict__ origins,
                                                            int group_views) {
  __shared__ WinPair tile[kOriginViews][256 + 1];
  __shared__ int64_t rows[256];
  const int bz_first = 2 * a.sbz_first;
  const int bz_count = min(2 * a.super_z, a.bricks_z - bz_first);
  const int64_t n_bricks = (int64_t)a.wbricks_x * a.wbricks_y * bz_count;
  const int lane = threadIdx.x & 63;
  const int64_t local = (int64_t)blockIdx.x * 256 + threadIdx.x;
  const bool exists = local < n_bricks;
  const int bx = (int)(local % a.wbricks_x);
  const int64_t t = local / a.wbricks_x;
  const int by = (int)(t % a.wbricks_y), bz = (int)(t / a.wbricks_y) + bz_first;
  const int64_t row = (((int64_t)bz * a.wbricks_y + by) * a.wbricks_x + bx) * a.class_pitch;
  const bool eligible = exists && bz * tk + tk <= a.nz;
  (void)lane;
  double wxa, wya, wza;
  {
    const double gx = a.ox + (bx * 8 + 0.5) * a.sx;
    const double gy = a.oy + (by * 8 + 0.5) * a.sy;
    const double gz = a.oz + ((bz * tk + a.kz0) + 0.5) * a.sz;
    wxa = row4(a.g + 0, gx, gy, gz), wya = row4(a.g + 4, gx, gy, gz), wza = row4(a.g + 8, gx, gy, gz);
  }
  const int m_begin = a.first_map, m_end = a.first_map + a.n_maps;
  const int g_lo = (m_begin & ~3) + blockIdx.y * group_views;
  rows[threadIdx.x] = row;
  uint32_t held[kOriginViews / 4];
#pragma unroll
  for (int g = 0; g < kOriginViews / 4; ++g) {
    const int m4 = g_lo + 4 * g;
    held[g] = (eligible && 4 * g < group_views && m4 < m_end) ? *reinterpret_cast<const uint32_t *>(classes + row + m4) : 0u;
#pragma unroll
    for (int q = 0; q < 4; ++q) tile[4 * g + q][threadIdx.x].origin = kNotWanted;
  }
#pragma unroll
  for (int g = 0; g < kOriginViews / 4; ++g) {
    const int m4 = g_lo + 4 * g;
    if (4 * g >= group_views || m4 >= m_end) break;
    const uint32_t c4 = held[g];
#pragma unroll 1
    for (int q = 0; q < 4; ++q) {
      const int m = m4 + q;
      const uint8_t c = (uint8_t)(c4 >> (8 * q));
      const bool want = eligible && m >= m_begin && m < m_end && (c & 0x1f) == (uint8_t)(BRICK_MIXED | (MIXED_FREE_OR_NODEPTH << 2));
      if (__builtin_amdgcn_ballot_w64(want) == 0) continue;
      WinPair wp;
      wp.origin = kNotWanted;
      wp.ax = wp.ay = wp.acz = 0.f;
      if (cload(&a.win_recs[m].e_abs) < __builtin_inff()) {
        const MapRec *src = maps + m;
        const TileMapRec *tsrc = a.tile_maps + m;
        const FootRec *fr = a.foot_recs + m;
        const float(*scp)[4] = tk == 16 ? fr->s16 : fr->s8;
        if (want) {
          const double cza = ((cload(&src->rt[8]) * wxa + cload(&src->rt[9]) * wya) + cload(&src->rt[10]) * wza) + cload(&src->rt[11]);
          const double hxa = __builtin_fma(cload(&tsrc->cpx), wxa, __builtin_fma(cload(&tsrc->cpy), wya, __builtin_fma(cload(&tsrc->cpz), wza, cload(&tsrc->cp0))));
          const double hya = __builtin_fma(cload(&tsrc->cqx), wxa, __builtin_fma(cload(&tsrc->cqy), wya, __builtin_fma(cload(&tsrc->cqz), wza, cload(&tsrc->cq0))));
          const float hx0 = (float)hxa, hy0 = (float)hya, z0 = (float)cza;
          float umin = __builtin_inff(), umax = -__builtin_inff(), vmin = __builtin_inff(), vmax = -__builtin_inff();
          float zmin = __builtin_inff(), zmax = -__builtin_inff();
#pragma unroll
          for (int cnr = 0; cnr < 8; ++cnr) {
            const float z = z0 + cload(&scp[cnr][2]);
            const float r = __builtin_amdgcn_rcpf(z);
            const float u = (hx0 + cload(&scp[cnr][0])) * r, v = (hy0 + cload(&scp[cnr][1])) * r;
            umin = __builtin_fminf(umin, u), umax = __builtin_fmaxf(umax, u);
            vmin = __builtin_fminf(vmin, v), vmax = __builtin_fmaxf(vmax, v);
            zmin = __builtin_fminf(zmin, z), zmax = __builtin_fmaxf(zmax, z);
          }
          const float umag = __builtin_fmaxf(__builtin_fmaxf(__builtin_fabsf(umin), __builtin_fabsf(umax)), __builtin_fmaxf(__builtin_fabsf(vmin), __builtin_fabsf(vmax)));
          const float e = 2.0f * cload(&fr->ferr) * __builtin_amdgcn_rcpf(zmin) * (1.0f + 0x1p-20f) + (0x1p-19f * umag + 0x1p-12f);
          const bool sane = zmin > 0.0f && zmax <= (float)(kWinCzRatio * (1.0 - 0x1p-20)) * zmin && umin > -65536.0f && umax < 65536.0f &&
                            vmin > -65536.0f && vmax < 65536.0f && e < 0.25f;
          if (sane) {
            const int cxc = a.W / 2, cyc = a.H / 2;
            const int x0 = (int)__builtin_ceilf(umin - 0.5f - e) + cxc, x1 = (int)__builtin_floorf(umax + 0.5f + e) + cxc;
            const int y0 = (int)__builtin_ceilf(vmin - 0.5f - e) + cyc, y1 = (int)__builtin_floorf(vmax + 0.5f + e) + cyc;
            if (x0 >= -kValidMargin && y0 >= -kValidMargin && x1 < a.W + kValidMargin && y1 < a.H + kValidMargin &&
                x1 - x0 < kWindowCols && y1 - y0 < kWindowRows) {
              wp.origin = (uint32_t)(x0 + kValidMargin) | ((uint32_t)(y0 + kValidMargin) << 16);
              wp.ax = (float)(hxa - (double)(x0 - cxc) * cza);
              wp.ay = (float)(hya - (double)(y0 - cyc) * cza);
              wp.acz = z0;
            }
          }
        }
      }
      if (want) {
        if (wp.origin != kNotWanted)
          tile[4 * g + q][threadIdx.x] = wp;
        else
          classes[row + m] = (uint8_t)(c | CLASS_NO_WINDOW);
      }
    }
  }
  __syncthreads();
  const int v = threadIdx.x & (kOriginViews - 1);
  const int m = g_lo + v;
  if (v < group_views && m < m_end) {
#pragma unroll
    for (int it = 0; it < 8; ++it) {
      const int b = (threadIdx.x >> 3) + 32 * it;
      const WinPair wp = tile[v][b];
      if (wp.origin != kNotWanted) origins[rows[b] + m] = wp;
    }
  }
}


__device__ __forceinline__ bool slot_to_brick(const TileArgs &a, int slot, int &bx, int &by, int &bz) {
  const int within = slot & 31;
  const int code = a.sb_perm[(slot - a.slot_base) >> 5];
  const int sbx = code & 1023, sby = (code >> 10) & 1023, sbz = (code >> 20) + a.sbz_first;
  bx = sbx * 4 + (within & 3);
  by = sby * 4 + ((within >> 2) & 3);
  bz = sbz * 2 + (within >> 4);
  return bx < a.bricks_x && by < a.bricks_y && bz < a.bricks_z;
}

constexpr int kWorkLevels = 4;

__global__ __launch_bounds__(256) void brick_work_kernel(const TileArgs a, int wx, int wy, int n_slots,
                                                         uint8_t *__restrict__ level) {
  const int lane = threadIdx.x & 63;
  const int slot = blockIdx.x * 4 + (threadIdx.x >> 6);
  if (slot >= n_slots) return;
  int bx, by, bz;
  if (!slot_to_brick(a, slot + a.slot_base, bx, by, bz)) {
    if (lane == 0) level[slot] = 255;
    return;
  }
  int mixed = 0, total = 0;
  for (int v = 0; v < wy; ++v)
    for (int u = 0; u < wx; ++u) {
      const int wbx = bx * wx + u, wby = by * wy + v;
// ... 412 lines not shown
```

### cudadepthmapintegration_amd/csrc/fusion_kernels.h

```cpp
#pragma once

#include <hip/hip_runtime.h>
#include <stddef.h>
#include <stdint.h>
#include <string.h>

struct dmi_context;

namespace dmi {

int grid_pointer_for_sums(::dmi_context *ctx, void **ptr);

struct alignas(16) DepthTile {
  float dmin, dmax;
  uint32_t flags;
  uint32_t pad;
};
enum TileFlags : uint32_t { TILE_HAS_SENTINEL = 1, TILE_HAS_VALID = 2, TILE_HAS_NAN = 4, TILE_PART_HOLE_FREE = 8, TILE_PART_NO_VALID = 16 };
constexpr int64_t kNoClassesMaxBricks = 1024;
constexpr int kNoClassesMaxViews = 48;
constexpr uint8_t COARSE_CHILDREN_WRITTEN = 0x80;

constexpr int kPyramidMinLevel = 3;
constexpr int kPyramidMaxLevels = 13;

struct PyramidDesc {
  int32_t n_levels;
  int32_t total_tiles;
  int32_t width[kPyramidMaxLevels];
  int32_t height[kPyramidMaxLevels];
  int32_t offset[kPyramidMaxLevels];
};

struct alignas(16) MapRec {
  double rt[12];
  double k[12];
  const void *depth;
  const DepthTile *pyramid;
};
static_assert(sizeof(MapRec) == 208, "MapRec layout");

struct alignas(16) TileMapRec {
  double rz0, rz1, rz3;
  double px, py, pz, p0;
  double qx, qy, qz, q0;
  double dhx, dhy;
  double err;
  const void *depth;
  double cz_err;
  double errk;
  double sx, sy, sz, s0, dhz, errz;
  double cpx, cpy, cpz, cp0, cqx, cqy, cqz, cq0;
  double cdhx, cdhy, cerrk;
  float t1_dhx, t1_dhy, t1_dcz, t1_dthr;
  float t1_e1, t1_c1;
  float t1_erel, t1_hspan;
  int32_t t1_cidx;
  int32_t t1_ok;
  const uint8_t *valid;
  float vm_c0, vm_w8;
  int32_t vm_base, vm_bytes;
  const uint32_t *vbits;
  int32_t vb_bytes;
  int32_t vb_rowskip;
  int32_t vb_mx, vb_my;
  float t1_b;
  int32_t vb_pad;
};
#ifndef DMI_TIER1
#define DMI_TIER1 1
#endif
constexpr int kValidMargin = 32;
constexpr unsigned kValidByte = 10;
__host__ __device__ inline int64_t valid_map_bytes(int W, int H) {
  return (int64_t)((H + 2 * kValidMargin + 7) / 8) * (W + 2 * kValidMargin) * 8;
}
__host__ __device__ inline int valid_bits_tiles_x(int W) { return (W + 2 * kValidMargin + 31) / 32 + 1; }
__host__ __device__ inline int valid_bits_tiles_y(int H) { return (H + 2 * kValidMargin + 31) / 32; }
__host__ __device__ inline int64_t valid_bits_bytes(int W, int H) { return (int64_t)valid_bits_tiles_x(W) * valid_bits_tiles_y(H) * 128; }
constexpr int kWindowCols = 32, kWindowRows = 64;
constexpr uint8_t CLASS_NO_WINDOW = 0x20;
static_assert(sizeof(TileMapRec) == 368, "TileMapRec layout");

struct alignas(64) WinRec {
  const uint32_t *vbits;
  float di[2], dj[2], dk[2];
  float ci[2], cj[2], ck[2];
  float e_abs;
  float c1;
};
static_assert(sizeof(WinRec) == 64, "WinRec is one cache line");
struct alignas(64) FootRec {
  float s8[8][4];
  float s16[8][4];
  float ferr, pad[15];
};
static_assert(sizeof(FootRec) == 320, "FootRec layout");
constexpr float kWinC1 = 0.5f - 0x1p-14f;
constexpr double kWinCzRatio = 1.25;
struct alignas(16) WinPair {
  uint32_t origin;
  float ax, ay, acz;
};
static_assert(sizeof(WinPair) == 16, "WinPair layout");

enum KMode : int {
  K_GENERAL = 0,
  K_PINHOLE_SKEW = 1,
  K_PINHOLE = 2
};

struct FuseArgs {
  int32_t nx, ny, nz;
  int32_t W, H;
  int32_t first_map, n_maps;
  int32_t init_from_grid;
  int32_t kz0, pad1;
  int32_t k_first, k_count;
  double ox, oy, oz;
  double sx, sy, sz;
  double g[12];
  double thick, delta;
  double rho_pos, rho_neg, rho_zero;
  double slope;
  double free_space;
  const MapRec *maps;
  void *grid;
  uint32_t *voxel_hits;
  unsigned long long *map_hits;
};

struct TileArgs {
  int32_t nx, ny, nz, W, H, first_map, n_maps, init_from_grid;
  int32_t kpad;
  int32_t bricks_x, bricks_y, bricks_z;
  int32_t super_x, super_y, super_z;
  int32_t sbz_first, pad3;
  int32_t slot_base, slot_count;
  int32_t depth_bytes;
  int32_t kz0, pad1;
  double ox, oy, oz, sx, sy, sz;
  double g[12];
  double thick, delta, rho_pos, rho_neg, slope, free_space;
  const TileMapRec *tile_maps;
  const double *cz_table;
  void *grid;
  uint32_t *voxel_hits;
  unsigned long long *map_hits;
  const FuseArgs *full;
  const uint8_t *classes;
  int32_t class_pitch;
  int32_t wbricks_x, wbricks_y;
  int32_t xcd_run_wg;
  const int32_t *order;
  const int32_t *n_order;
  unsigned long long behind_mask;
  int32_t rotated;
  int32_t flags;
  const MapRec *maps;
  const int32_t *order_levels;
  const double *free_sums;
  const int32_t *sb_perm;
  unsigned long long *wg_times;
  int64_t wg_times_n;
  int32_t *queue_heads;
  WinPair *win_origin;
  int64_t win_delta;
  const WinRec *win_recs;
  const FootRec *foot_recs;
  int32_t vb_bytes, vb_rowskip;
  int32_t win_cx, win_cy;
};
constexpr int kFreeSumsMax = 4096;
__host__ __device__ inline int32_t pack_brick(int bx, int by, int bz) { return (int32_t)((uint32_t)bx | ((uint32_t)by << 11) | ((uint32_t)bz << 22)); }
static_assert(offsetof(TileArgs, nx) == 0 && offsetof(TileArgs, nz) == 8 && offsetof(TileArgs, kpad) == 32 &&
                  offsetof(TileArgs, bricks_x) == 36 && offsetof(TileArgs, bricks_z) == 44 && offsetof(TileArgs, sbz_first) == 60,
              "TileArgs head layout");
enum TileKernelFlags : int32_t {
  TILE_FLAG_NO_INTERIOR = 1,
  TILE_FLAG_XCD_RUNS = 2,
  TILE_FLAG_COST_ORDER = 4,
  TILE_FLAG_DBG_SKIP_WINDOW_PAIRS = 256,
  TILE_FLAG_DBG_ONLY_WINDOW_PAIRS = 512,
  TILE_FLAG_DBG_NO_WINDOW_LOADS = 1024
};

enum BrickClass : uint8_t {
  BRICK_MIXED = 0,
  BRICK_FREE = 1,
  BRICK_BEHIND = 2,
  BRICK_SKIP = 3
};

enum MixedReason : uint8_t {
  MIXED_UNSPECIFIED = 0,
  MIXED_DEGENERATE = 1,
  MIXED_CAMERA_PLANE = 2,
  MIXED_IMAGE_BORDER = 3,
  MIXED_NAN_DEPTH = 4,
  MIXED_SENTINEL_AND_DEPTH = 5,
  MIXED_NEAR_SURFACE = 6,
  MIXED_FREE_OR_NODEPTH = 7
};

struct FuseConfig {
  int depth_is_f64;
  int grid_is_f64;
  int k_mode;
  int count_hits;
  int variant;
  int use_tile;
  int general_k;
  int holes;
};

enum VariantBits : int {
  VAR_EXACT_DIVISION = 1,
  VAR_GENERAL_K = 2,
  VAR_BLOCK_SHAPE_MASK = 12,
  VAR_FORCE_GENERAL = 16,
  VAR_TILE_SHAPE_MASK = 0xE0,
  VAR_TILE_SHAPE_SHIFT = 5,
  VAR_NO_BRICK_CLASSES = 256,
  VAR_SPATIAL_ORDER = 512,
  VAR_FIXED_TILE_SHAPE = 4096,
  VAR_KEEP_BEHIND_ADDS = 1024,
  VAR_NO_INTERIOR = 2048,
  VAR_XCD_RUNS = 8192,
  VAR_ZMAJOR_SLOTS = 16384,
  VAR_PERSISTENT_ALWAYS = 32768,
  VAR_PERSISTENT_NEVER = 65536,
  VAR_BRICK_CLASSES_ALWAYS = 131072,
  VAR_NO_WINDOWS = 262144,
  VAR_WINDOWS_ALWAYS = 524288,
  VAR_COST_ORDER = 1048576,
  VAR_NO_COST_ORDER = 2097152
};

constexpr int kMaxColumnHeight = 16;
struct TileShape {
  int tk, wx, wy;
};
TileShape tile_shape(int variant, bool depth_is_f64, bool rotated, bool general_k);

hipError_t launch_fuse(const FuseArgs &args, const FuseConfig &cfg, hipStream_t stream);

hipError_t launch_fuse_tiled(const TileArgs &args, const MapRec *maps_dev, const FuseConfig &cfg, const PyramidDesc &pyramid,
                             uint8_t *order_scratch, uint8_t *coarse_classes, hipEvent_t before_main_kernel,
// ... 93 lines not shown
```

### include/dmi.h

```cpp
#ifndef DMI_H_
#define DMI_H_

#include <stddef.h>
#include <stdint.h>

#ifdef __cplusplus
extern "C" {
#endif

#define DMI_ABI_VERSION 5

typedef struct dmi_context dmi_context;

typedef enum dmi_status {
  DMI_OK = 0,
  DMI_ERR_INVALID_ARGUMENT = 1,
  DMI_ERR_DEVICE = 2,
  DMI_ERR_OUT_OF_MEMORY = 3,
  DMI_ERR_STATE = 4
} dmi_status;

typedef enum dmi_dtype { DMI_F32 = 0, DMI_F64 = 1 } dmi_dtype;

typedef enum dmi_depth_storage { DMI_DEPTH_AUTO = 0, DMI_DEPTH_F32 = 1, DMI_DEPTH_F64 = 2 } dmi_depth_storage;

typedef struct dmi_grid_desc {
  int32_t cell_dims[3];
  double origin[3];
  double spacing[3];
  double grid_matrix[16];
} dmi_grid_desc;

typedef struct dmi_ray_potential {
  double thickness;
  double rho;
  double eta;
  double delta;
} dmi_ray_potential;

typedef struct dmi_options {
  int32_t device;
  int32_t grid_dtype;
  int32_t depth_storage;
  int32_t count_hits;
  int32_t kernel_variant;
  int32_t z_first;
  void *stream;
  void *external_grid;
} dmi_options;

typedef struct dmi_timings {
  double last_fuse_kernel_ms;
  double total_fuse_kernel_ms;
  uint64_t fuse_launches;
  double last_upload_ms;
  double last_download_ms;
  double last_cell_to_point_ms;
  double last_fuse_main_kernel_ms;
  double total_fuse_main_kernel_ms;
} dmi_timings;

typedef struct dmi_info {
  int64_t n_voxels;
  int32_t n_views;
  int32_t depth_width;
  int32_t depth_height;
  int32_t depth_storage_in_use;
  int32_t grid_dtype;
  int32_t k_mode;
  int32_t kernel_variant;
  int32_t tiled_kernel;
  uint64_t device_bytes;
  uint64_t pixels_without_depth;
} dmi_info;

void dmi_default_options(dmi_options *opt);

int dmi_create(const dmi_grid_desc *grid, const dmi_ray_potential *ray, const dmi_options *opt, dmi_context **out);

void dmi_destroy(dmi_context *ctx);

const char *dmi_last_error(const dmi_context *ctx);

int dmi_add_views(dmi_context *ctx, const double *depth, const double *best_cost, double threshold, const double *K4,
                  const double *RT4, int32_t n, int32_t width, int32_t height);

int dmi_add_views_f32(dmi_context *ctx, const float *depth, const double *K4, const double *RT4, int32_t n,
                      int32_t width, int32_t height);

int dmi_clear_views(dmi_context *ctx);

int dmi_reset_grid(dmi_context *ctx);

int dmi_upload_grid(dmi_context *ctx, const double *grid);

int dmi_fuse(dmi_context *ctx);

int dmi_fuse_range(dmi_context *ctx, int32_t first, int32_t count);

#define DMI_SLAB_ALIGNMENT 32
int dmi_fuse_slab(dmi_context *ctx, int32_t z_first, int32_t z_count);

int dmi_synchronize(dmi_context *ctx);

int dmi_download_grid_f64(dmi_context *ctx, double *out);
int dmi_download_grid_f32(dmi_context *ctx, float *out);

int dmi_fuse_range_download(dmi_context *ctx, int32_t first, int32_t count, void *out, int32_t out_dtype, int32_t n_slabs);

int dmi_download_hits(dmi_context *ctx, uint32_t *voxel_hits, uint64_t *map_hits);

int dmi_grid_device_pointer(dmi_context *ctx, void **ptr);

int dmi_cell_to_point(dmi_context *ctx);
int dmi_download_point_data_f64(dmi_context *ctx, double *out);
int dmi_point_data_device_pointer(dmi_context *ctx, void **ptr);

int dmi_iso_active_cells(dmi_context *ctx, double iso, uint64_t *count, int64_t *cell_ids, uint64_t capacity);

int dmi_extract_isosurface(dmi_context *ctx, double iso, uint64_t *n_vertices, uint64_t *n_triangles);
int dmi_download_isosurface(dmi_context *ctx, double *vertices, int64_t *triangles);
int dmi_extract_isosurface_normals(dmi_context *ctx, double iso, uint64_t *n_vertices, uint64_t *n_triangles);
int dmi_download_isosurface_normals(dmi_context *ctx, float *normals);
int dmi_get_isosurface_kernel_ms(dmi_context *ctx, double *last);

enum { DMI_COMPONENTS_MIN_TRIANGLES = 0, DMI_COMPONENTS_LARGEST = 1 };
int dmi_filter_isosurface_components(dmi_context *ctx, int mode, uint64_t min_triangles, uint64_t *n_vertices, uint64_t *n_triangles,
                                     uint64_t *n_components, uint64_t *n_components_kept);
int dmi_download_isosurface_regions(dmi_context *ctx, int64_t *region_id, int64_t *region_size);
int dmi_get_isosurface_filter_kernel_ms(dmi_context *ctx, double *last);
int dmi_get_isosurface_filter_pass_ms(dmi_context *ctx, double out[4]);
int dmi_get_isosurface_filter_cas_retries(dmi_context *ctx, uint64_t *last);

int dmi_smooth_isosurface(dmi_context *ctx, int32_t iterations, double lambda, double mu);
int dmi_get_isosurface_smooth_kernel_ms(dmi_context *ctx, double *last);
int dmi_get_isosurface_smooth_pass_ms(dmi_context *ctx, double out[3]);

int dmi_get_brick_class_histogram(dmi_context *ctx, uint64_t out[4]);

int dmi_get_mixed_reason_histogram(dmi_context *ctx, uint64_t out[8]);

int dmi_get_window_pair_count(dmi_context *ctx, uint64_t *out);

int dmi_get_view_paths(dmi_context *ctx, uint64_t out[6]);

int dmi_get_timings(dmi_context *ctx, dmi_timings *out);
int dmi_get_info(dmi_context *ctx, dmi_info *out);
size_t dmi_sizeof_info(void);
size_t dmi_sizeof_timings(void);

int dmi_get_upload_kernel_ms(dmi_context *ctx, double *last, double *total);

int dmi_alloc_pinned(size_t bytes, void **out);
int dmi_free_pinned(void *ptr);
int dmi_pcie_probe(int32_t device, size_t bytes, double *h2d_GBps, double *d2h_GBps);
int dmi_fp64_probe(int32_t device, double milliseconds, double *tflops);

int dmi_color_mesh(const double *points, int64_t n_points, const uint8_t *colors, const double *K4, const double *RT4,
                   int32_t n_views, int32_t width, int32_t height, int32_t device, uint8_t *mean, uint8_t *median,
                   int32_t *count);
const char *dmi_color_last_error(void);

typedef struct dmi_color_context dmi_color_context;
int dmi_color_create(int32_t device, dmi_color_context **out);
void dmi_color_destroy(dmi_color_context *ctx);
int dmi_color_add_views(dmi_color_context *ctx, const uint8_t *colors, const double *K4, const double *RT4, int32_t n,
                        int32_t width, int32_t height);
int dmi_color_clear_views(dmi_color_context *ctx);
int dmi_color_process(dmi_color_context *ctx, const double *points, int64_t n_points, uint8_t *mean, uint8_t *median,
                      int32_t *count);
int dmi_color_set_scratch_budget(dmi_color_context *ctx, uint64_t bytes);
int dmi_color_set_vertex_reorder(dmi_color_context *ctx, int32_t enable);
int dmi_color_get_kernel_ms(dmi_color_context *ctx, double *out);
int dmi_color_add_views_with_depth(dmi_color_context *ctx, const uint8_t *colors, const double *depths, const double *K4,
                                   const double *RT4, int32_t n, int32_t width, int32_t height);
int dmi_color_set_depth_test(dmi_color_context *ctx, int32_t enable, double tolerance);

typedef struct dmi_multi_context dmi_multi_context;

typedef enum dmi_partition { DMI_PARTITION_VIEWS = 0, DMI_PARTITION_Z_SLABS = 1 } dmi_partition;
typedef enum dmi_exchange { DMI_EXCHANGE_ALL_REDUCE = 0, DMI_EXCHANGE_REDUCE_SCATTER = 1, DMI_EXCHANGE_PEER_COPY = 2 } dmi_exchange;

#define DMI_UNIQUE_ID_BYTES 128

typedef struct dmi_multi_options {
  int32_t grid_dtype;
  int32_t depth_storage;
  int32_t kernel_variant;
  int32_t partition;
  int32_t exchange;
  int32_t n_slabs;
} dmi_multi_options;

typedef struct dmi_multi_info {
  int32_t world;
  int32_t n_local;
  int32_t first_rank;
  int32_t rccl_ranks;
  int32_t rccl_version;
  int32_t partition, exchange, n_slabs;
  int64_t n_voxels;
  int64_t n_views_total;
  int64_t n_views_local;
} dmi_multi_info;

typedef struct dmi_multi_timings {
  double last_step_ms;
  double last_fuse_kernel_ms;
  double total_step_ms;
  uint64_t steps;
} dmi_multi_timings;

void dmi_multi_default_options(dmi_multi_options *opt);

int dmi_multi_view_shard(int64_t n, int32_t rank, int32_t world, int64_t *first, int64_t *count);
#define DMI_Z_SLAB_ALIGNMENT 16
int dmi_multi_z_slab(int32_t nz, int32_t rank, int32_t world, int32_t *z_first, int32_t *z_count);
int dmi_multi_peer_chunk(int64_t n, int32_t world, int32_t c, int64_t *first, int64_t *count);
int dmi_multi_slab_ranges(int32_t nz, int32_t n_slabs, int32_t *z_first, int32_t *z_count, int32_t max_slabs);

int dmi_multi_create(const dmi_grid_desc *grid, const dmi_ray_potential *ray, const dmi_multi_options *opt,
                     const int32_t *devices, int32_t n, dmi_multi_context **out);
int dmi_multi_get_unique_id(uint8_t id[DMI_UNIQUE_ID_BYTES]);
int dmi_multi_create_rank(const dmi_grid_desc *grid, const dmi_ray_potential *ray, const dmi_multi_options *opt,
                          int32_t device, int32_t rank, int32_t world, const uint8_t id[DMI_UNIQUE_ID_BYTES],
                          dmi_multi_context **out);
void dmi_multi_destroy(dmi_multi_context *ctx);
const char *dmi_multi_last_error(const dmi_multi_context *ctx);

int dmi_multi_add_views(dmi_multi_context *ctx, const double *depth, const double *best_cost, double threshold,
                        const double *K4, const double *RT4, int32_t n, int32_t width, int32_t height);
int dmi_multi_add_views_f32(dmi_multi_context *ctx, const float *depth, const double *K4, const double *RT4, int32_t n,
                            int32_t width, int32_t height);
int dmi_multi_add_local_views(dmi_multi_context *ctx, int32_t local_index, const double *depth, const double *best_cost,
                              double threshold, const double *K4, const double *RT4, int32_t n, int32_t width, int32_t height);
int dmi_multi_add_local_views_f32(dmi_multi_context *ctx, int32_t local_index, const float *depth, const double *K4,
                                  const double *RT4, int32_t n, int32_t width, int32_t height);
int dmi_multi_clear_views(dmi_multi_context *ctx);

int dmi_multi_fuse(dmi_multi_context *ctx);
int dmi_multi_synchronize(dmi_multi_context *ctx);

int dmi_multi_download_grid_f32(dmi_multi_context *ctx, float *out, int64_t *owned_first, int64_t *owned_count);
int dmi_multi_download_grid_f64(dmi_multi_context *ctx, double *out, int64_t *owned_first, int64_t *owned_count);

int dmi_multi_get_info(dmi_multi_context *ctx, dmi_multi_info *out);
int dmi_multi_get_timings(dmi_multi_context *ctx, dmi_multi_timings *out);
int dmi_multi_local_context(dmi_multi_context *ctx, int32_t local_index, dmi_context **out);

int dmi_abi_version(void);
int dmi_device_count(void);

#ifdef __cplusplus
}
#endif

#endif
```

Before: 2916.

## Compute brick footprints in fp32 from precomputed corner offsets with fp64 fallback

After: 2862. 1.8% lower.

```diff
diff --git a/cudadepthmapintegration_amd/build.py b/cudadepthmapintegration_amd/build.py
--- a/cudadepthmapintegration_amd/build.py
+++ b/cudadepthmapintegration_amd/build.py
@@ -12,8 +12,8 @@
 OBJ_DIR = os.path.join(ROOT, "build", "obj")
 LIB_PATH = os.path.join(CSRC, "libdmi_hip.so")
 
-SOURCES = ["fusion_kernels.hip", "fusion_tile.hip", "fusion_classify.hip", "coloration_kernels.hip", "grid_post.hip", "isosurface.hip", "isosurface_components.hip", "isosurface_smooth.hip", "dmi_capi.hip", "dmi_multi.hip", "host/recon_host.cpp", "host/vti_reader.cpp", "host/vtp_reader.cpp", "host/recon_cli.cpp", "host/color_cli.cpp", "host/dmi_host_capi.cpp"]
-HEADERS = ["fusion_kernels.h", "fusion_device.h", "fusion_tile_acc.inc", "isosurface_table.inc", os.path.join("host", "recon_host.h"),
+SOURCES = ["fusion_kernels.hip", "fusion_tile.hip", "fusion_classify.hip", "footprint_check.hip", "coloration_kernels.hip", "grid_post.hip", "isosurface.hip", "isosurface_components.hip", "isosurface_smooth.hip", "dmi_capi.hip", "dmi_multi.hip", "host/recon_host.cpp", "host/vti_reader.cpp", "host/vtp_reader.cpp", "host/recon_cli.cpp", "host/color_cli.cpp", "host/dmi_host_capi.cpp"]
+HEADERS = ["fusion_kernels.h", "fusion_device.h", "fusion_footprint.h", "fusion_tile_acc.inc", "isosurface_table.inc", os.path.join("host", "recon_host.h"),
            os.path.join("host", "vtk_xml_data.h"), os.path.join("host", "vti_reader.h"), os.path.join("host", "vtp_reader.h"),
            os.path.join("host", "recon_cli.h"), os.path.join("host", "color_cli.h"),
            os.path.join("..", "..", "include", "dmi.h"), os.path.join("..", "..", "include", "dmi_host.h")]
diff --git a/cudadepthmapintegration_amd/capi.py b/cudadepthmapintegration_amd/capi.py
--- a/cudadepthmapintegration_amd/capi.py
+++ b/cudadepthmapintegration_amd/capi.py
@@ -107,6 +107,7 @@
     "dmi_multi_add_views_f32", "dmi_multi_add_local_views", "dmi_multi_add_local_views_f32", "dmi_multi_clear_views", "dmi_multi_fuse", "dmi_multi_synchronize",
     "dmi_multi_download_grid_f32", "dmi_multi_download_grid_f64", "dmi_multi_get_info", "dmi_multi_get_timings",
     "dmi_multi_local_context",
+    "dmi_check_brick_footprints",
 ]
 
 _lib = None
@@ -186,6 +187,9 @@
         L.dmi_get_isosurface_smooth_pass_ms.argtypes = [vp, dp]
     L.dmi_get_brick_class_histogram.argtypes = [vp, ctypes.POINTER(ctypes.c_uint64)]
     L.dmi_get_mixed_reason_histogram.argtypes = [vp, ctypes.POINTER(ctypes.c_uint64)]
+    if hasattr(L, "dmi_check_brick_footprints"):
+        L.dmi_check_brick_footprints.argtypes = [ctypes.POINTER(GridDescC), i32, i32, i32, dp, dp, i32, ctypes.c_uint64, ctypes.c_uint64,
+                                                 ctypes.POINTER(ctypes.c_uint64)]
     if hasattr(L, "dmi_get_window_pair_count"):
         L.dmi_get_window_pair_count.argtypes = [vp, ctypes.POINTER(ctypes.c_uint64)]
     if hasattr(L, "dmi_get_view_paths"):
@@ -576,6 +580,22 @@
         a = (ctypes.c_uint64 * 6)()
         self._check(self._lib.dmi_get_view_paths(self._h, a))
         return {k: int(v) for k, v in zip(names, a)}
+
+
+def check_brick_footprints(grid: GridDesc, width: int, height: int, K4: np.ndarray, RT4: np.ndarray, column: int = 16,
+                           samples: int = 100000, seed: int = 1) -> dict:
+    L = load()
+    K = np.ascontiguousarray(K4, dtype=np.float64).reshape(-1, 16)
+    RT = np.ascontiguousarray(RT4, dtype=np.float64).reshape(-1, 16)
+    assert K.shape == RT.shape
+    counts = (ctypes.c_uint64 * 4)()
+    dp = ctypes.POINTER(ctypes.c_double)
+    g = _grid_c(grid)
+    rc = L.dmi_check_brick_footprints(ctypes.byref(g), int(width), int(height), int(K.shape[0]), K.ctypes.data_as(dp),
+                                      RT.ctypes.data_as(dp), int(column), int(samples), int(seed), counts)
+    if rc != 0:
+        raise DmiError(rc, "dmi_check_brick_footprints: invalid argument (a general K has no fp32 footprint)")
+    return {"fp32": int(counts[0]), "violations": int(counts[1]), "larger": int(counts[2]), "fp64": int(counts[3])}
 
 
 def _grid_c(grid: GridDesc) -> GridDescC:
diff --git a/cudadepthmapintegration_amd/csrc/dmi_capi.hip b/cudadepthmapintegration_amd/csrc/dmi_capi.hip
--- a/cudadepthmapintegration_amd/csrc/dmi_capi.hip
+++ b/cudadepthmapintegration_amd/csrc/dmi_capi.hip
@@ -507,6 +507,7 @@
         }
       }
       foot->ferr = float_not_below(cerr + xmax * nl2);
+      foot->ferr_far = float_not_below(cerr + 65536.0 * nl2);
     }
   }
   if (per_lane) {
@@ -604,6 +605,26 @@
   if (zscale_out) *zscale_out = zscale;
   return t;
 }
+
+}
+
+namespace dmi {
+bool host_view_records(const dmi_grid_desc &grid, int32_t W, int32_t H, const double *K4, const double *RT4, MapRec *mr,
+                       TileMapRec *tr, FootRec *foot) {
+  dmi_context ctx;
+  ctx.grid = grid;
+  ctx.W = W;
+  ctx.H = H;
+  std::memset(mr, 0, sizeof(*mr));
+  std::memcpy(mr->rt, RT4, 12 * sizeof(double));
+  std::memcpy(mr->k, K4, 12 * sizeof(double));
+  WinRec win;
+  *tr = make_tile_rec(&ctx, *mr, &win, foot, nullptr);
+  return classify_k(mr->k, mr->rt) != K_GENERAL;
+}
+}
+
+namespace {
 
 bool tile_eligible(const dmi_context *ctx) {
   if (ctx->opt.kernel_variant & dmi::VAR_FORCE_GENERAL) return false;
@@ -1352,11 +1373,11 @@
         ctx->device_bytes += cbytes;
       }
       t.classes = ctx->d_classes;
+      t.foot_recs = ctx->d_foot_recs;
       if (windows) {
         t.win_origin = reinterpret_cast<dmi::WinPair *>(ctx->d_classes + coarse_end);
         t.win_delta = (int64_t)reinterpret_cast<intptr_t>(t.win_origin) - 16 * (int64_t)reinterpret_cast<intptr_t>(t.classes);
         t.win_recs = ctx->d_win_recs;
-        t.foot_recs = ctx->d_foot_recs;
         t.vb_bytes = (int32_t)std::min<int64_t>(dmi::valid_bits_bytes(ctx->W, ctx->H), 0x7fffffff);
         t.vb_rowskip = (dmi::valid_bits_tiles_x(ctx->W) - 1) * 128;
         t.win_cx = dmi::kValidMargin + ctx->W / 2;
diff --git a/cudadepthmapintegration_amd/csrc/footprint_check.hip b/cudadepthmapintegration_amd/csrc/footprint_check.hip
--- /dev/null
+++ b/cudadepthmapintegration_amd/csrc/footprint_check.hip
@@ -0,0 +1,82 @@
+#include <cstring>
+#include <vector>
+
+#include "../../include/dmi.h"
+#include "fusion_footprint.h"
+
+namespace dmi {
+bool host_view_records(const dmi_grid_desc &grid, int32_t W, int32_t H, const double *K4, const double *RT4, MapRec *mr,
+                       TileMapRec *tr, FootRec *foot);
+
+namespace {
+
+struct SplitMix64 {
+  uint64_t s;
+  uint64_t next() {
+    uint64_t z = (s += 0x9e3779b97f4a7c15ull);
+    z = (z ^ (z >> 30)) * 0xbf58476d1ce4e5b9ull;
+    z = (z ^ (z >> 27)) * 0x94d049bb133111ebull;
+    return z ^ (z >> 31);
+  }
+};
+
+template <bool ROT>
+void check_pairs(const TileArgs &a, const std::vector<MapRec> &maps, const std::vector<TileMapRec> &recs,
+                 const std::vector<FootRec> &foots, int tk, uint64_t samples, uint64_t seed, uint64_t *counts) {
+  SplitMix64 rng{seed};
+  const int nbx = (a.nx + 7) / 8, nby = (a.ny + 7) / 8, nbz = (a.nz + tk - 1) / tk;
+  for (uint64_t n = 0; n < samples; ++n) {
+    const size_t m = (size_t)(rng.next() % maps.size());
+    const int bx = (int)(rng.next() % (uint64_t)nbx), by = (int)(rng.next() % (uint64_t)nby), bz = (int)(rng.next() % (uint64_t)nbz);
+    const int i0 = bx * 8, j0 = by * 8, k0 = bz * tk;
+    BoxFootprint f32;
+    const bool served = brick_footprint_f32<ROT>(a, &maps[m], &recs[m], tk == 16 ? foots[m].s16 : foots[m].s8, foots[m].ferr_far, i0,
+                                                 i0 + 7, j0, j0 + 7, k0, k0 + tk - 1, f32);
+    if (!served) {
+      ++counts[3];
+      continue;
+    }
+    ++counts[0];
+    const BoxFootprint f64 = box_footprint_k<ROT, false>(a, &maps[m], &recs[m], i0, i0 + 7, j0, j0 + 7, k0, k0 + tk - 1);
+    const bool has_rect = f64.query || f64.partial || (f64.cls == BRICK_SKIP && f64.czmax >= 0.0);
+    const bool inside = has_rect && f32.rx0 <= f64.rx0 && f32.rx1 >= f64.rx1 && f32.ry0 <= f64.ry0 && f32.ry1 >= f64.ry1;
+    const bool same_z = f32.czmin == f64.czmin && f32.czmax == f64.czmax;
+    if (!inside || !same_z) ++counts[1];
+    if (inside && (f32.rx0 < f64.rx0 || f32.rx1 > f64.rx1 || f32.ry0 < f64.ry0 || f32.ry1 > f64.ry1)) ++counts[2];
+  }
+}
+
+}
+}
+
+extern "C" int dmi_check_brick_footprints(const dmi_grid_desc *grid, int32_t width, int32_t height, int32_t n_views, const double *K4,
+                                          const double *RT4, int32_t column, uint64_t samples, uint64_t seed, uint64_t *counts) {
+  if (!grid || !K4 || !RT4 || !counts || n_views <= 0 || width <= 0 || height <= 0 || (column != 8 && column != 16))
+    return DMI_ERR_INVALID_ARGUMENT;
+  try {
+    std::vector<dmi::MapRec> maps((size_t)n_views);
+    std::vector<dmi::TileMapRec> recs((size_t)n_views);
+    std::vector<dmi::FootRec> foots((size_t)n_views);
+    for (int32_t m = 0; m < n_views; ++m)
+      if (!dmi::host_view_records(*grid, width, height, K4 + 16 * (size_t)m, RT4 + 16 * (size_t)m, &maps[(size_t)m], &recs[(size_t)m],
+                                  &foots[(size_t)m]))
+        return DMI_ERR_INVALID_ARGUMENT;
+    dmi::TileArgs a;
+    std::memset(&a, 0, sizeof(a));
+    a.nx = grid->cell_dims[0]; a.ny = grid->cell_dims[1]; a.nz = grid->cell_dims[2];
+    a.W = width; a.H = height;
+    a.ox = grid->origin[0]; a.oy = grid->origin[1]; a.oz = grid->origin[2];
+    a.sx = grid->spacing[0]; a.sy = grid->spacing[1]; a.sz = grid->spacing[2];
+    std::memcpy(a.g, grid->grid_matrix, sizeof(a.g));
+    const double *g = grid->grid_matrix;
+    const bool aligned = g[1] == 0 && g[2] == 0 && g[4] == 0 && g[6] == 0 && g[8] == 0 && g[9] == 0;
+    for (int q = 0; q < 4; ++q) counts[q] = 0;
+    if (aligned)
+      dmi::check_pairs<false>(a, maps, recs, foots, column, samples, seed, counts);
+    else
+      dmi::check_pairs<true>(a, maps, recs, foots, column, samples, seed, counts);
+  } catch (...) {
+    return DMI_ERR_OUT_OF_MEMORY;
+  }
+  return DMI_OK;
+}
diff --git a/cudadepthmapintegration_amd/csrc/fusion_classify.hip b/cudadepthmapintegration_amd/csrc/fusion_classify.hip
--- a/cudadepthmapintegration_amd/csrc/fusion_classify.hip
+++ b/cudadepthmapintegration_amd/csrc/fusion_classify.hip
@@ -5,6 +5,7 @@
 
 #include "fusion_kernels.h"
 #include "fusion_device.h"
+#include "fusion_footprint.h"
 
 namespace dmi {
 
@@ -24,6 +25,27 @@
   float f = (float)d;
   if ((double)f < d) f = nextafterf(f, __builtin_inff());
   return f;
+}
+
+__device__ __forceinline__ uint16_t half_bits(_Float16 h) { return __builtin_bit_cast(uint16_t, h); }
+__device__ __forceinline__ float half_value(uint16_t b) { return (float)__builtin_bit_cast(_Float16, b); }
+__device__ __forceinline__ uint16_t half_next_down(uint16_t b) {
+  if (b == 0xfc00u) return b;
+  if ((b & 0x7fffu) == 0) return 0x8001u;
+  return (b & 0x8000u) ? (uint16_t)(b + 1) : (uint16_t)(b - 1);
+}
+__device__ __forceinline__ uint16_t half_next_up(uint16_t b) {
+  if (b == 0x7c00u) return b;
+  if ((b & 0x7fffu) == 0) return 0x0001u;
+  return (b & 0x8000u) ? (uint16_t)(b - 1) : (uint16_t)(b + 1);
+}
+__device__ __forceinline__ uint16_t half_below(float f) {
+  const uint16_t b = half_bits((_Float16)f);
+  return half_value(b) > f ? half_next_down(b) : b;
+}
+__device__ __forceinline__ uint16_t half_above(float f) {
+  const uint16_t b = half_bits((_Float16)f);
+  return half_value(b) < f ? half_next_up(b) : b;
 }
 
 struct TileAcc {
@@ -206,156 +228,6 @@
   return acc;
 }
 
-struct BoxFootprint {
-  uint8_t cls;
-  bool query;
-  bool partial;
-  bool in_margin;
-  int x0, x1, y0, y1;
-  int rx0, rx1, ry0, ry1;
-  double czmin, czmax;
-};
-
-template <bool ROT, bool GK>
-__device__ __forceinline__ BoxFootprint box_footprint_k(const TileArgs &a, const MapRec *__restrict__ mr,
-                                                      const TileMapRec *__restrict__ tr, int i0, int i1, int j0, int j1, int k0,
-                                                      int k1) {
-  BoxFootprint fp;
-  fp.query = false;
-  fp.partial = false;
-  fp.in_margin = false;
-  fp.x0 = fp.x1 = fp.y0 = fp.y1 = 0;
-  fp.rx0 = fp.rx1 = fp.ry0 = fp.ry1 = 0;
-  double czmin = __builtin_inf(), czmax = -__builtin_inf();
-  double umin = __builtin_inf(), umax = -__builtin_inf(), vmin = __builtin_inf(), vmax = -__builtin_inf();
-  constexpr bool genk = GK;
-  double hzmin = __builtin_inf(), hzmax = -__builtin_inf();
-  bool bad = false;
-  const double r23 = mr->rt[11];
-  if constexpr (ROT) {
-#pragma unroll
-    for (int c = 0; c < 8; ++c) {
-      const int i = (c & 1) ? i1 : i0, j = (c & 2) ? j1 : j0, k = (c & 4) ? k1 : k0;
-      const double gx = a.ox + (i + 0.5) * a.sx;
-      const double gy = a.oy + (j + 0.5) * a.sy;
-      const double gz = a.oz + ((k + a.kz0) + 0.5) * a.sz;
-      const double wx = row4(a.g + 0, gx, gy, gz), wy = row4(a.g + 4, gx, gy, gz), wz = row4(a.g + 8, gx, gy, gz);
-      const double cz = row4(mr->rt + 8, wx, wy, wz);
-      const double hx = __builtin_fma(tr->px, wx, __builtin_fma(tr->py, wy, __builtin_fma(tr->pz, wz, tr->p0)));
-      const double hy = __builtin_fma(tr->qx, wx, __builtin_fma(tr->qy, wy, __builtin_fma(tr->qz, wz, tr->q0)));
-      const double hz = genk ? __builtin_fma(tr->sx, wx, __builtin_fma(tr->sy, wy, __builtin_fma(tr->sz, wz, tr->s0))) : cz;
-      double r = __builtin_amdgcn_rcp(hz);
-      r = __builtin_fma(r, __builtin_fma(-hz, r, 1.0), r);
-      const double u = hx * r, v = hy * r;
-      bad = bad || !(cz == cz);
-      if (genk) {
-        bad = bad || !(hz == hz);
-        hzmin = fmin(hzmin, hz);
-        hzmax = fmax(hzmax, hz);
-      }
-      czmin = fmin(czmin, cz);
-      czmax = fmax(czmax, cz);
-      umin = fmin(umin, u);
-      umax = fmax(umax, u);
-      vmin = fmin(vmin, v);
-      vmax = fmax(vmax, v);
-    }
-    czmin -= 2.0 * tr->cz_err;
-    czmax += 2.0 * tr->cz_err;
-  } else {
-  double wxs[2], wys[2], wzs[2];
-  for (int c = 0; c < 2; ++c) {
-    const int i = c ? i1 : i0, j = c ? j1 : j0, k = c ? k1 : k0;
-    const double gx = a.ox + (i + 0.5) * a.sx;
-    const double gy = a.oy + (j + 0.5) * a.sy;
-    const double gz = a.oz + ((k + a.kz0) + 0.5) * a.sz;
-    wxs[c] = row4(a.g + 0, gx, gy, gz);
-    wys[c] = row4(a.g + 4, gx, gy, gz);
-    wzs[c] = row4(a.g + 8, gx, gy, gz);
-  }
-  const double r20 = mr->rt[8], r21 = mr->rt[9], r22 = mr->rt[10];
-  const double zx[2] = {r20 * wxs[0], r20 * wxs[1]}, zy[2] = {r21 * wys[0], r21 * wys[1]}, zz[2] = {r22 * wzs[0], r22 * wzs[1]};
-  const double ux[2] = {tr->px * wxs[0], tr->px * wxs[1]};
-  const double uy[2] = {__builtin_fma(tr->py, wys[0], tr->p0), __builtin_fma(tr->py, wys[1], tr->p0)};
-  const double uz[2] = {tr->pz * wzs[0], tr->pz * wzs[1]};
-  const double vx[2] = {tr->qx * wxs[0], tr->qx * wxs[1]};
-  const double vy[2] = {__builtin_fma(tr->qy, wys[0], tr->q0), __builtin_fma(tr->qy, wys[1], tr->q0)};
-  const double vz[2] = {tr->qz * wzs[0], tr->qz * wzs[1]};
-  double sxw[2] = {0.0, 0.0}, syw[2] = {0.0, 0.0}, szw[2] = {0.0, 0.0};
-  if (genk) {
-    sxw[0] = tr->sx * wxs[0], sxw[1] = tr->sx * wxs[1];
-    syw[0] = __builtin_fma(tr->sy, wys[0], tr->s0), syw[1] = __builtin_fma(tr->sy, wys[1], tr->s0);
-    szw[0] = tr->sz * wzs[0], szw[1] = tr->sz * wzs[1];
-  }
-#pragma unroll
-  for (int c = 0; c < 8; ++c) {
-    const int cx = c & 1, cy = (c >> 1) & 1, ck = c >> 2;
-    const double cz = ((zx[cx] + zy[cy]) + zz[ck]) + r23;
-    const double hx = (ux[cx] + uy[cy]) + uz[ck];
-    const double hy = (vx[cx] + vy[cy]) + vz[ck];
-    const double hz = genk ? (sxw[cx] + syw[cy]) + szw[ck] : cz;
-    double r = __builtin_amdgcn_rcp(hz);
-    r = __builtin_fma(r, __builtin_fma(-hz, r, 1.0), r);
-    const double u = hx * r, v = hy * r;
-    bad = bad || !(cz == cz);
-    if (genk) {
-      bad = bad || !(hz == hz);
-      hzmin = fmin(hzmin, hz);
-      hzmax = fmax(hzmax, hz);
-    }
-    czmin = fmin(czmin, cz);
-    czmax = fmax(czmax, cz);
-    umin = fmin(umin, u);
-    umax = fmax(umax, u);
-    vmin = fmin(vmin, v);
-    vmax = fmax(vmax, v);
-  }
-  }
-  uint8_t cls = BRICK_MIXED | (MIXED_DEGENERATE << 2);
-  const double errz2 = 2.0 * tr->errz;
-  const double err = genk ? tr->err + 65536.0 * tr->errz : tr->err;
-  const double dmin = genk ? hzmin - errz2 : czmin, dmax = genk ? hzmax + errz2 : czmax;
-  const double ulimit = genk ? 65536.0 : 0x1p30;
-  if (!bad) {
-    cls = BRICK_MIXED | (MIXED_CAMERA_PLANE << 2);
-    if (dmax < 0.0) {
-      cls = BRICK_SKIP;
-    } else if (dmin > 4.0 * err && dmin > 0.0 && umin == umin && umax == umax && vmin == vmin && vmax == vmax &&
-               fabs(umin) < ulimit && fabs(umax) < ulimit && fabs(vmin) < ulimit && fabs(vmax) < ulimit) {
-      double rmin = __builtin_amdgcn_rcp(dmin);
-      rmin = __builtin_fma(rmin, __builtin_fma(-dmin, rmin, 1.0), rmin);
-      const double e = 2.0 * err * rmin * (1.0 + 0x1p-30) + 0x1p-20;
-      const int x0 = (int)ceil(umin - 0.5 - e), x1 = (int)floor(umax + 0.5 + e);
-      const int y0 = (int)ceil(vmin - 0.5 - e), y1 = (int)floor(vmax + 0.5 + e);
-      cls = BRICK_MIXED | (MIXED_IMAGE_BORDER << 2);
-      fp.rx0 = x0;
-      fp.rx1 = x1;
-      fp.ry0 = y0;
-      fp.ry1 = y1;
-      if (x1 < 0 || y1 < 0 || x0 >= a.W || y0 >= a.H) {
-        cls = BRICK_SKIP;
-      } else if (x0 >= 0 && y0 >= 0 && x1 < a.W && y1 < a.H) {
-        fp.query = true;
-        fp.x0 = x0;
-        fp.x1 = x1;
-        fp.y0 = y0;
-        fp.y1 = y1;
-      } else {
-        fp.partial = true;
-        fp.in_margin = x0 >= -kValidMargin && y0 >= -kValidMargin && x1 < a.W + kValidMargin && y1 < a.H + kValidMargin;
-        fp.x0 = max(x0, 0);
-        fp.x1 = min(x1, a.W - 1);
-        fp.y0 = max(y0, 0);
-        fp.y1 = min(y1, a.H - 1);
-      }
-    }
-  }
-  fp.cls = cls;
-  fp.czmin = czmin;
-  fp.czmax = czmax;
-  return fp;
-}
-
 template <bool ROT, bool GK>
 __device__ __forceinline__ BoxFootprint box_footprint(const TileArgs &a, const MapRec *__restrict__ mr,
                                                       const TileMapRec *__restrict__ tr, int i0, int i1, int j0, int j1, int k0,
@@ -366,16 +238,18 @@
   return box_footprint_k<ROT, false>(a, mr, tr, i0, i1, j0, j1, k0, k1);
 }
 
+__device__ __forceinline__ bool bounds_far_behind(const TileArgs &a, float dmin, double czmax) { return (czmax - (double)dmin) < -a.delta; }
+__device__ __forceinline__ bool bounds_far_in_front(const TileArgs &a, float dmax, double czmin) { return (czmin - (double)dmax) > a.delta; }
 __device__ __forceinline__ uint8_t class_from_bounds(const TileArgs &a, const TileAcc &d, double czmin, double czmax) {
   if (d.flags & TILE_HAS_NAN) return BRICK_MIXED | (MIXED_NAN_DEPTH << 2);
   if (!(d.flags & TILE_HAS_VALID)) return BRICK_SKIP;
   const bool holes = (d.flags & TILE_HAS_SENTINEL) != 0;
-  if ((czmax - (double)d.dmin) < -a.delta) {
+  if (bounds_far_behind(a, d.dmin, czmax)) {
     if (!holes) return BRICK_FREE;
     const bool free_column_exact = a.behind_mask != 0 || __builtin_signbit(a.free_space);
     return free_column_exact ? (uint8_t)(BRICK_MIXED | (MIXED_FREE_OR_NODEPTH << 2)) : (uint8_t)(BRICK_MIXED | (MIXED_SENTINEL_AND_DEPTH << 2));
   }
-  if ((czmin - (double)d.dmax) > a.delta) {
+  if (bounds_far_in_front(a, d.dmax, czmin)) {
     if (!holes) return BRICK_BEHIND;
     return a.behind_mask ? (uint8_t)BRICK_SKIP : (uint8_t)(BRICK_MIXED | (MIXED_SENTINEL_AND_DEPTH << 2));
   }
@@ -390,6 +264,21 @@
   if (map_serves && (c == BRICK_FREE || c == (uint8_t)(BRICK_MIXED | (MIXED_FREE_OR_NODEPTH << 2))))
     return BRICK_MIXED | (MIXED_FREE_OR_NODEPTH << 2);
   return BRICK_MIXED | (MIXED_IMAGE_BORDER << 2);
+}
+
+template <bool ROT, bool GK>
+__device__ __forceinline__ BoxFootprint brick_footprint(const TileArgs &a, const MapRec *__restrict__ mr,
+                                                        const TileMapRec *__restrict__ tr, int m, int tk, int bx, int by, int bz) {
+  if constexpr (!GK) {
+    if (a.foot_recs != nullptr) {
+      const FootRec *__restrict__ fr = a.foot_recs + m;
+      BoxFootprint fp;
+      if (brick_footprint_f32<ROT>(a, mr, tr, tk == 16 ? fr->s16 : fr->s8, fr->ferr_far, bx * 8, bx * 8 + 7, by * 8, by * 8 + 7,
+                                   bz * tk, bz * tk + tk - 1, fp))
+        return fp;
+    }
+  }
+  return box_footprint<ROT, GK>(a, mr, tr, bx * 8, bx * 8 + 7, by * 8, by * 8 + 7, bz * tk, bz * tk + tk - 1);
 }
 
 template <int kQueryTiles, bool ROT, bool GK>
@@ -462,7 +351,7 @@
   constexpr int children = kChildren;
   constexpr int views_per_wave = 64 / children;
   constexpr int per_z = children / 16;
-  __shared__ float2 window_mm[4 * views_per_wave][kWindow * kWindow];
+  __shared__ uint32_t window_mm[4 * views_per_wave][kWindow * kWindow];
   __shared__ uint8_t window_fl[4 * views_per_wave][kWindow * kWindow];
   const int bz_first = 2 * a.sbz_first;
   const int bz_count = min(2 * a.super_z, a.bricks_z - bz_first);
@@ -514,18 +403,20 @@
         tr_u.sx = cload(&tsrc->sx); tr_u.sy = cload(&tsrc->sy); tr_u.sz = cload(&tsrc->sz); tr_u.s0 = cload(&tsrc->s0);
       }
       mr = &mr_u;
-      if (mine) {
-        fp = box_footprint<ROT, GK>(a, &mr_u, &tr_u, bx * 8, bx * 8 + 7, by * 8, by * 8 + 7, bz * tk, bz * tk + tk - 1);
+      if constexpr (!GK) {
+        tr_u.cpx = cload(&tsrc->cpx); tr_u.cpy = cload(&tsrc->cpy); tr_u.cpz = cload(&tsrc->cpz); tr_u.cp0 = cload(&tsrc->cp0);
+        tr_u.cqx = cload(&tsrc->cqx); tr_u.cqy = cload(&tsrc->cqy); tr_u.cqz = cload(&tsrc->cqz); tr_u.cq0 = cload(&tsrc->cq0);
       }
+      if (mine) fp = brick_footprint<ROT, GK>(a, &mr_u, &tr_u, mu, tk, bx, by, bz);
     } else {
-      if (mine) fp = box_footprint<ROT, GK>(a, mr, a.tile_maps + m, bx * 8, bx * 8 + 7, by * 8, by * 8 + 7, bz * tk, bz * tk + tk - 1);
+      if (mine) fp = brick_footprint<ROT, GK>(a, mr, a.tile_maps + m, m, tk, bx, by, bz);
     }
     const bool query = mine && (fp.query || fp.partial);
     uint8_t cls = fp.cls;
     const int li = query ? query_level<kQueryTiles>(P, max(fp.x1 - fp.x0, fp.y1 - fp.y0) + 1) : 0x7fff;
     bool from_window = false;
     {
-      float2 *__restrict__ win_mm = window_mm[wave * views_per_wave + lane / children];
+      uint32_t *__restrict__ win_mm = window_mm[wave * views_per_wave + lane / children];
       uint8_t *__restrict__ win_fl = window_fl[wave * views_per_wave + lane / children];
       int li_w = li;
       for (int off = children >> 1; off > 0; off >>= 1) li_w = min(li_w, __shfl_xor(li_w, off, 64));
@@ -549,7 +440,7 @@
           for (int ty = child >> 4; ty < wh; ty += children / 16)
             if (tx < ww) {
               const DepthTile t = level[(wy0 + ty) * pitch + wx0 + tx];
-              win_mm[ty * kWindow + tx] = make_float2(t.dmin, t.dmax);
+              win_mm[ty * kWindow + tx] = (uint32_t)half_below(t.dmin) | ((uint32_t)half_above(t.dmax) << 16);
               win_fl[ty * kWindow + tx] = (uint8_t)t.flags;
             }
           __builtin_amdgcn_fence(__ATOMIC_RELEASE, "wavefront");
@@ -560,11 +451,20 @@
             for (int ty = ty0; ty <= ty1; ++ty)
               for (int tx = tx0; tx <= tx1; ++tx) {
                 const int w = (ty - wy0) * kWindow + (tx - wx0);
-                const float2 mm = win_mm[w];
-                d.add_tile(DepthTile{mm.x, mm.y, (uint32_t)win_fl[w], 0u});
+                const uint32_t mm = win_mm[w];
+                d.add_tile(DepthTile{half_value((uint16_t)mm), half_value((uint16_t)(mm >> 16)), (uint32_t)win_fl[w], 0u});
               }
-            cls = fp.partial ? border_class<GK>(a, fp, d) : class_from_bounds(a, d, fp.czmin, fp.czmax);
-            from_window = true;
+            bool settled = true;
+            if ((d.flags & TILE_HAS_VALID) && !(d.flags & TILE_HAS_NAN)) {
+              const float dmin_in = half_value(half_next_up(half_bits((_Float16)d.dmin)));
+              const float dmax_in = half_value(half_next_down(half_bits((_Float16)d.dmax)));
+              settled = bounds_far_behind(a, d.dmin, fp.czmax) == bounds_far_behind(a, dmin_in, fp.czmax) &&
+                        bounds_far_in_front(a, d.dmax, fp.czmin) == bounds_far_in_front(a, dmax_in, fp.czmin);
+            }
+            if (settled) {
+              cls = fp.partial ? border_class<GK>(a, fp, d) : class_from_bounds(a, d, fp.czmin, fp.czmax);
+              from_window = true;
+            }
           }
           __builtin_amdgcn_fence(__ATOMIC_RELEASE, "wavefront");
           __builtin_amdgcn_wave_barrier();
diff --git a/cudadepthmapintegration_amd/csrc/fusion_footprint.h b/cudadepthmapintegration_amd/csrc/fusion_footprint.h
--- /dev/null
+++ b/cudadepthmapintegration_amd/csrc/fusion_footprint.h
@@ -0,0 +1,268 @@
+#pragma once
+#include <cmath>
+#include <cstdint>
+
+#include "fusion_kernels.h"
+
+#define DMI_FP_HD __host__ __device__ __forceinline__
+
+namespace dmi {
+
+DMI_FP_HD double fp_row4(const double *__restrict__ m, double x, double y, double z) {
+  return ((m[0] * x + m[1] * y) + m[2] * z) + m[3];
+}
+DMI_FP_HD double fp_rcp64(double x) {
+#if defined(__HIP_DEVICE_COMPILE__)
+  double r = __builtin_amdgcn_rcp(x);
+  return __builtin_fma(r, __builtin_fma(-x, r, 1.0), r);
+#else
+  return 1.0 / x;
+#endif
+}
+DMI_FP_HD float fp_rcp32(float x) {
+#if defined(__HIP_DEVICE_COMPILE__)
+  return __builtin_amdgcn_rcpf(x);
+#else
+  return 1.0f / x;
+#endif
+}
+DMI_FP_HD int fp_imin(int a, int b) { return a < b ? a : b; }
+DMI_FP_HD int fp_imax(int a, int b) { return a > b ? a : b; }
+
+struct BoxFootprint {
+  uint8_t cls;
+  bool query;
+  bool partial;
+  bool in_margin;
+  int x0, x1, y0, y1;
+  int rx0, rx1, ry0, ry1;
+  double czmin, czmax;
+};
+
+DMI_FP_HD void footprint_against_image(const TileArgs &a, int x0, int x1, int y0, int y1, BoxFootprint &fp) {
+  fp.cls = BRICK_MIXED | (MIXED_IMAGE_BORDER << 2);
+  fp.rx0 = x0;
+  fp.rx1 = x1;
+  fp.ry0 = y0;
+  fp.ry1 = y1;
+  if (x1 < 0 || y1 < 0 || x0 >= a.W || y0 >= a.H) {
+    fp.cls = BRICK_SKIP;
+  } else if (x0 >= 0 && y0 >= 0 && x1 < a.W && y1 < a.H) {
+    fp.query = true;
+    fp.x0 = x0;
+    fp.x1 = x1;
+    fp.y0 = y0;
+    fp.y1 = y1;
+  } else {
+    fp.partial = true;
+    fp.in_margin = x0 >= -kValidMargin && y0 >= -kValidMargin && x1 < a.W + kValidMargin && y1 < a.H + kValidMargin;
+    fp.x0 = fp_imax(x0, 0);
+    fp.x1 = fp_imin(x1, a.W - 1);
+    fp.y0 = fp_imax(y0, 0);
+    fp.y1 = fp_imin(y1, a.H - 1);
+  }
+}
+
+template <bool ROT, bool GK>
+DMI_FP_HD BoxFootprint box_footprint_k(const TileArgs &a, const MapRec *__restrict__ mr, const TileMapRec *__restrict__ tr, int i0,
+                                       int i1, int j0, int j1, int k0, int k1) {
+  BoxFootprint fp;
+  fp.query = false;
+  fp.partial = false;
+  fp.in_margin = false;
+  fp.x0 = fp.x1 = fp.y0 = fp.y1 = 0;
+  fp.rx0 = fp.rx1 = fp.ry0 = fp.ry1 = 0;
+  double czmin = __builtin_inf(), czmax = -__builtin_inf();
+  double umin = __builtin_inf(), umax = -__builtin_inf(), vmin = __builtin_inf(), vmax = -__builtin_inf();
+  constexpr bool genk = GK;
+  double hzmin = __builtin_inf(), hzmax = -__builtin_inf();
+  bool bad = false;
+  const double r23 = mr->rt[11];
+  if constexpr (ROT) {
+#pragma unroll
+    for (int c = 0; c < 8; ++c) {
+      const int i = (c & 1) ? i1 : i0, j = (c & 2) ? j1 : j0, k = (c & 4) ? k1 : k0;
+      const double gx = a.ox + (i + 0.5) * a.sx;
+      const double gy = a.oy + (j + 0.5) * a.sy;
+      const double gz = a.oz + ((k + a.kz0) + 0.5) * a.sz;
+      const double wx = fp_row4(a.g + 0, gx, gy, gz), wy = fp_row4(a.g + 4, gx, gy, gz), wz = fp_row4(a.g + 8, gx, gy, gz);
+      const double cz = fp_row4(mr->rt + 8, wx, wy, wz);
+      const double hx = __builtin_fma(tr->px, wx, __builtin_fma(tr->py, wy, __builtin_fma(tr->pz, wz, tr->p0)));
+      const double hy = __builtin_fma(tr->qx, wx, __builtin_fma(tr->qy, wy, __builtin_fma(tr->qz, wz, tr->q0)));
+      const double hz = genk ? __builtin_fma(tr->sx, wx, __builtin_fma(tr->sy, wy, __builtin_fma(tr->sz, wz, tr->s0))) : cz;
+      const double r = fp_rcp64(hz);
+      const double u = hx * r, v = hy * r;
+      bad = bad || !(cz == cz);
+      if (genk) {
+        bad = bad || !(hz == hz);
+        hzmin = fmin(hzmin, hz);
+        hzmax = fmax(hzmax, hz);
+      }
+      czmin = fmin(czmin, cz);
+      czmax = fmax(czmax, cz);
+      umin = fmin(umin, u);
+      umax = fmax(umax, u);
+      vmin = fmin(vmin, v);
+      vmax = fmax(vmax, v);
+    }
+    czmin -= 2.0 * tr->cz_err;
+    czmax += 2.0 * tr->cz_err;
+  } else {
+  double wxs[2], wys[2], wzs[2];
+  for (int c = 0; c < 2; ++c) {
+    const int i = c ? i1 : i0, j = c ? j1 : j0, k = c ? k1 : k0;
+    const double gx = a.ox + (i + 0.5) * a.sx;
+    const double gy = a.oy + (j + 0.5) * a.sy;
+    const double gz = a.oz + ((k + a.kz0) + 0.5) * a.sz;
+    wxs[c] = fp_row4(a.g + 0, gx, gy, gz);
+    wys[c] = fp_row4(a.g + 4, gx, gy, gz);
+    wzs[c] = fp_row4(a.g + 8, gx, gy, gz);
+  }
+  const double r20 = mr->rt[8], r21 = mr->rt[9], r22 = mr->rt[10];
+  const double zx[2] = {r20 * wxs[0], r20 * wxs[1]}, zy[2] = {r21 * wys[0], r21 * wys[1]}, zz[2] = {r22 * wzs[0], r22 * wzs[1]};
+  const double ux[2] = {tr->px * wxs[0], tr->px * wxs[1]};
+  const double uy[2] = {__builtin_fma(tr->py, wys[0], tr->p0), __builtin_fma(tr->py, wys[1], tr->p0)};
+  const double uz[2] = {tr->pz * wzs[0], tr->pz * wzs[1]};
+  const double vx[2] = {tr->qx * wxs[0], tr->qx * wxs[1]};
+  const double vy[2] = {__builtin_fma(tr->qy, wys[0], tr->q0), __builtin_fma(tr->qy, wys[1], tr->q0)};
+  const double vz[2] = {tr->qz * wzs[0], tr->qz * wzs[1]};
+  double sxw[2] = {0.0, 0.0}, syw[2] = {0.0, 0.0}, szw[2] = {0.0, 0.0};
+  if (genk) {
+    sxw[0] = tr->sx * wxs[0], sxw[1] = tr->sx * wxs[1];
+    syw[0] = __builtin_fma(tr->sy, wys[0], tr->s0), syw[1] = __builtin_fma(tr->sy, wys[1], tr->s0);
+    szw[0] = tr->sz * wzs[0], szw[1] = tr->sz * wzs[1];
+  }
+#pragma unroll
+  for (int c = 0; c < 8; ++c) {
+    const int cx = c & 1, cy = (c >> 1) & 1, ck = c >> 2;
+    const double cz = ((zx[cx] + zy[cy]) + zz[ck]) + r23;
+    const double hx = (ux[cx] + uy[cy]) + uz[ck];
+    const double hy = (vx[cx] + vy[cy]) + vz[ck];
+    const double hz = genk ? (sxw[cx] + syw[cy]) + szw[ck] : cz;
+    const double r = fp_rcp64(hz);
+    const double u = hx * r, v = hy * r;
+    bad = bad || !(cz == cz);
+    if (genk) {
+      bad = bad || !(hz == hz);
+      hzmin = fmin(hzmin, hz);
+      hzmax = fmax(hzmax, hz);
+    }
+    czmin = fmin(czmin, cz);
+    czmax = fmax(czmax, cz);
+    umin = fmin(umin, u);
+    umax = fmax(umax, u);
+    vmin = fmin(vmin, v);
+    vmax = fmax(vmax, v);
+  }
+  }
+  uint8_t cls = BRICK_MIXED | (MIXED_DEGENERATE << 2);
+  const double errz2 = 2.0 * tr->errz;
+  const double err = genk ? tr->err + 65536.0 * tr->errz : tr->err;
+  const double dmin = genk ? hzmin - errz2 : czmin, dmax = genk ? hzmax + errz2 : czmax;
+  const double ulimit = genk ? 65536.0 : 0x1p30;
+  if (!bad) {
+    cls = BRICK_MIXED | (MIXED_CAMERA_PLANE << 2);
+    if (dmax < 0.0) {
+      cls = BRICK_SKIP;
+    } else if (dmin > 4.0 * err && dmin > 0.0 && umin == umin && umax == umax && vmin == vmin && vmax == vmax &&
+               fabs(umin) < ulimit && fabs(umax) < ulimit && fabs(vmin) < ulimit && fabs(vmax) < ulimit) {
+      const double rmin = fp_rcp64(dmin);
+      const double e = 2.0 * err * rmin * (1.0 + 0x1p-30) + 0x1p-20;
+      const int x0 = (int)ceil(umin - 0.5 - e), x1 = (int)floor(umax + 0.5 + e);
+      const int y0 = (int)ceil(vmin - 0.5 - e), y1 = (int)floor(vmax + 0.5 + e);
+      fp.cls = cls;
+      footprint_against_image(a, x0, x1, y0, y1, fp);
+      cls = fp.cls;
+    }
+  }
+  fp.cls = cls;
+  fp.czmin = czmin;
+  fp.czmax = czmax;
+  return fp;
+}
+
+template <bool ROT>
+DMI_FP_HD bool brick_footprint_f32(const TileArgs &a, const MapRec *__restrict__ mr, const TileMapRec *__restrict__ tr,
+                                   const float (*__restrict__ scp)[4], float ferr_far, int i0, int i1, int j0, int j1, int k0,
+                                   int k1, BoxFootprint &fp) {
+  fp.query = false;
+  fp.partial = false;
+  fp.in_margin = false;
+  fp.x0 = fp.x1 = fp.y0 = fp.y1 = 0;
+  fp.rx0 = fp.rx1 = fp.ry0 = fp.ry1 = 0;
+  if (!(ferr_far > 0.0f)) return false;
+  double czmin = __builtin_inf(), czmax = -__builtin_inf();
+  double wxa, wya, wza, cza;
+  bool bad = false;
+  if constexpr (ROT) {
+    wxa = wya = wza = cza = 0.0;
+#pragma unroll
+    for (int c = 0; c < 8; ++c) {
+      const int i = (c & 1) ? i1 : i0, j = (c & 2) ? j1 : j0, k = (c & 4) ? k1 : k0;
+      const double gx = a.ox + (i + 0.5) * a.sx;
+      const double gy = a.oy + (j + 0.5) * a.sy;
+      const double gz = a.oz + ((k + a.kz0) + 0.5) * a.sz;
+      const double wx = fp_row4(a.g + 0, gx, gy, gz), wy = fp_row4(a.g + 4, gx, gy, gz), wz = fp_row4(a.g + 8, gx, gy, gz);
+      const double cz = fp_row4(mr->rt + 8, wx, wy, wz);
+      if (c == 0) wxa = wx, wya = wy, wza = wz, cza = cz;
+      bad = bad || !(cz == cz);
+      czmin = fmin(czmin, cz);
+      czmax = fmax(czmax, cz);
+    }
+    czmin -= 2.0 * tr->cz_err;
+    czmax += 2.0 * tr->cz_err;
+  } else {
+    double wxs[2], wys[2], wzs[2];
+    for (int c = 0; c < 2; ++c) {
+      const int i = c ? i1 : i0, j = c ? j1 : j0, k = c ? k1 : k0;
+      const double gx = a.ox + (i + 0.5) * a.sx;
+      const double gy = a.oy + (j + 0.5) * a.sy;
+      const double gz = a.oz + ((k + a.kz0) + 0.5) * a.sz;
+      wxs[c] = fp_row4(a.g + 0, gx, gy, gz);
+      wys[c] = fp_row4(a.g + 4, gx, gy, gz);
+      wzs[c] = fp_row4(a.g + 8, gx, gy, gz);
+    }
+    const double r20 = mr->rt[8], r21 = mr->rt[9], r22 = mr->rt[10], r23 = mr->rt[11];
+    const double zx[2] = {r20 * wxs[0], r20 * wxs[1]}, zy[2] = {r21 * wys[0], r21 * wys[1]}, zz[2] = {r22 * wzs[0], r22 * wzs[1]};
+    cza = 0.0;
+#pragma unroll
+    for (int c = 0; c < 8; ++c) {
+      const double cz = ((zx[c & 1] + zy[(c >> 1) & 1]) + zz[c >> 2]) + r23;
+      if (c == 0) cza = cz;
+      bad = bad || !(cz == cz);
+      czmin = fmin(czmin, cz);
+      czmax = fmax(czmax, cz);
+    }
+    wxa = wxs[0], wya = wys[0], wza = wzs[0];
+  }
+  if (bad || !(czmin > 4.0 * tr->err) || !(czmin > 0.0)) return false;
+  const double hxa = __builtin_fma(tr->cpx, wxa, __builtin_fma(tr->cpy, wya, __builtin_fma(tr->cpz, wza, tr->cp0)));
+  const double hya = __builtin_fma(tr->cqx, wxa, __builtin_fma(tr->cqy, wya, __builtin_fma(tr->cqz, wza, tr->cq0)));
+  const float hx0 = (float)hxa, hy0 = (float)hya, z0 = (float)cza;
+  float umin = __builtin_inff(), umax = -__builtin_inff(), vmin = __builtin_inff(), vmax = -__builtin_inff();
+  float zmin = __builtin_inff(), zmax = -__builtin_inff();
+#pragma unroll
+  for (int cnr = 0; cnr < 8; ++cnr) {
+    const float z = z0 + scp[cnr][2];
+    const float r = fp_rcp32(z);
+    const float u = (hx0 + scp[cnr][0]) * r, v = (hy0 + scp[cnr][1]) * r;
+    umin = __builtin_fminf(umin, u), umax = __builtin_fmaxf(umax, u);
+    vmin = __builtin_fminf(vmin, v), vmax = __builtin_fmaxf(vmax, v);
+    zmin = __builtin_fminf(zmin, z), zmax = __builtin_fmaxf(zmax, z);
+  }
+  const float umag = __builtin_fmaxf(__builtin_fmaxf(__builtin_fabsf(umin), __builtin_fabsf(umax)),
+                                     __builtin_fmaxf(__builtin_fabsf(vmin), __builtin_fabsf(vmax)));
+  const float e = 2.0f * ferr_far * fp_rcp32(zmin) * (1.0f + 0x1p-20f) + (0x1p-19f * umag + 0x1p-12f);
+  const bool sane = zmin > 0.0f && zmax <= (float)(kWinCzRatio * (1.0 - 0x1p-20)) * zmin && umin > -65536.0f && umax < 65536.0f &&
+                    vmin > -65536.0f && vmax < 65536.0f && e < 0.25f;
+  if (!sane) return false;
+  const int cxc = a.W / 2, cyc = a.H / 2;
+  const int x0 = (int)__builtin_ceilf(umin - 0.5f - e) + cxc, x1 = (int)__builtin_floorf(umax + 0.5f + e) + cxc;
+  const int y0 = (int)__builtin_ceilf(vmin - 0.5f - e) + cyc, y1 = (int)__builtin_floorf(vmax + 0.5f + e) + cyc;
+  footprint_against_image(a, x0, x1, y0, y1, fp);
+  fp.czmin = czmin;
+  fp.czmax = czmax;
+  return true;
+}
+
+}
diff --git a/cudadepthmapintegration_amd/csrc/fusion_kernels.h b/cudadepthmapintegration_amd/csrc/fusion_kernels.h
--- a/cudadepthmapintegration_amd/csrc/fusion_kernels.h
+++ b/cudadepthmapintegration_amd/csrc/fusion_kernels.h
@@ -93,7 +93,7 @@
 struct alignas(64) FootRec {
   float s8[8][4];
   float s16[8][4];
-  float ferr, pad[15];
+  float ferr, ferr_far, pad[14];
 };
 static_assert(sizeof(FootRec) == 320, "FootRec layout");
 constexpr float kWinC1 = 0.5f - 0x1p-14f;
diff --git a/include/dmi.h b/include/dmi.h
--- a/include/dmi.h
+++ b/include/dmi.h
@@ -141,6 +141,8 @@
 int dmi_get_mixed_reason_histogram(dmi_context *ctx, uint64_t out[8]);
 
 int dmi_get_window_pair_count(dmi_context *ctx, uint64_t *out);
+int dmi_check_brick_footprints(const dmi_grid_desc *grid, int32_t width, int32_t height, int32_t n_views, const double *K4,
+                               const double *RT4, int32_t column, uint64_t samples, uint64_t seed, uint64_t *counts);
 
 int dmi_get_view_paths(dmi_context *ctx, uint64_t out[6]);
 
```
